# JeroendenBoef/GraphPOPE

Measured on AMD Instinct MI355X. Metric: POPE embeddings/sec (nodes x anchors) + SAGE nodes/sec, Flickr 256 anchors, higher is better.
Workload: dtype u64; 1 GPU; configs[1]: flickr-shaped geodesic-stochastic, N=89250 E=899756 F=500, 256 anchors PER GPU (np.random seed 42); inputs resident in HBM (edge_index, x) -> [N, F+K] f32 in HBM on every rank; anchors_total=256, anchors_per_rank=256, parallelism=single GPU

## Files before the change

### graphpope_amd/_lib.py

```python
from __future__ import annotations

import ctypes
import os
from ctypes import c_char_p, c_double, c_float, c_int, c_int32, c_int64, c_size_t, c_uint64, c_void_p, POINTER

_HERE = os.path.dirname(os.path.abspath(__file__))
LIB_PATH = os.path.join(_HERE, "libgraphpope_hip.so")

OK, ERR_INVALID, ERR_HIP, ERR_INDEX, ERR_HOP_OVERFLOW, ERR_WORKSPACE, ERR_NO_DEVICE, ERR_UNSORTED = 0, -1, -2, -3, -4, -5, -6, -7
METRIC = {"distance": 0, "similarity": 1, "euclidean": 2}
KNOB_LIVE_MODE, KNOB_FINALIZE_VARIANT, KNOB_FINALIZE_BLOCKS = 0, 1, 2
KNOB_PAIRWISE_KERNEL, KNOB_COPY_BATCHES, KNOB_FAIL_HOST_REGISTER = 4, 5, 7
KNOB_SAGE_FORWARD_OVERLAP = 14
KNOB_GEMM_TILE16_BUFFERS = 18
KNOB_PREPARE_MERGE = 19
KNOB_STREAMK_XCD = 20
KNOB_FORWARD_WHOLE_TILES = 21
KNOB_LEVEL1_APPLY = 22

SIGNATURES = {
    "pope_last_error": (c_char_p, []),
    "pope_version": (c_char_p, []),
    "pope_require_device": (c_int, [POINTER(c_int32)]),
    "pope_debug_set": (c_int, [c_int32, c_int32]),
    "pope_host_copy_2d": (c_int, [c_void_p, c_int64, c_void_p, c_int64, c_int64, c_int64, c_int32]),
    "pope_copy_2d_to_host": (c_int, [c_void_p, c_int64, c_void_p, c_int64, c_int64, c_int64, c_void_p]),
    "pope_assemble_host_result": (c_int, [c_void_p, c_int64, c_int64, c_void_p, c_int64, c_int64, c_void_p, c_int64, c_int64, c_int32,
                                          c_int32, c_void_p]),
    "pope_assemble_begin": (c_void_p, [c_void_p, c_int64, c_int64, c_void_p, c_int64, c_int64, c_int32, c_int32]),
    "pope_assemble_finish": (c_int, [c_void_p, c_void_p, c_int64, c_int64, c_void_p]),
    "pope_assemble_abort": (None, [c_void_p]),
    "pope_assemble_prepare": (None, [c_int32]),
    "pope_assemble_ring_ready": (c_int32, []),
    "pope_assemble_finish_codes": (c_int, [c_void_p, c_void_p, c_int64, c_int32, c_void_p, c_void_p]),
    "pope_geodesic_hop_codes": (c_int, [c_void_p, c_int32, c_int32, c_int64, c_int32, c_void_p, c_int64, c_void_p, c_void_p]),
    "pope_host_pin": (c_int, [c_void_p, c_size_t]),
    "pope_host_unpin": (c_int, [c_void_p]),
    "pope_copy_to_device": (c_int, [c_void_p, c_void_p, c_size_t, c_void_p]),
    "pope_csr_scratch_bytes": (c_size_t, [c_int64, c_int64]),
    "pope_csr_aux_elems": (c_size_t, [c_int64]),
    "pope_csr_build": (c_int, [c_void_p, c_int64, c_int64, c_void_p, c_void_p, c_void_p, c_void_p, c_void_p, c_size_t,
                               c_int32, c_void_p]),
    "pope_csr_build_canonical": (c_int, [c_void_p, c_int64, c_int64, c_void_p, c_void_p, c_void_p, c_void_p, c_void_p, c_size_t, c_void_p]),
    "pope_pagerank_weights": (c_int, [c_void_p, c_void_p, c_int64, c_void_p, c_void_p]),
    "pope_pagerank_step": (c_int, [c_void_p, c_void_p, c_int64, c_void_p, c_void_p, c_double, c_double, c_void_p, c_void_p]),
    "pope_clustering_scratch_bytes": (c_size_t, [c_int64, c_int64]),
    "pope_clustering_counts": (c_int, [c_void_p, c_void_p, c_void_p, c_void_p, c_void_p, c_void_p, c_int64, c_int64, c_void_p, c_void_p,
                                       c_void_p, c_void_p, c_size_t, c_void_p]),
    "pope_betweenness_scratch_bytes": (c_size_t, [c_int64, c_int64]),
    "pope_betweenness_batch": (c_int, [c_void_p, c_void_p, c_int64, c_void_p, c_void_p, c_int64, c_int64, c_int64, c_int64, c_void_p,
                                       c_void_p, c_void_p, c_void_p, c_void_p, c_void_p, c_size_t, c_void_p]),
    "pope_eigenvector_scratch_bytes": (c_size_t, [c_int64]),
    "pope_eigenvector_iterate": (c_int, [c_void_p, c_void_p, c_int64, c_void_p, c_void_p, c_size_t, c_int32, c_double, c_void_p, c_void_p]),
    "pope_degree_counts": (c_int, [c_void_p, c_void_p, c_void_p, c_int64, c_void_p, c_void_p, c_void_p]),
    "pope_topk_scratch_bytes": (c_size_t, [c_int64, c_int64]),
    "pope_topk_u64": (c_int, [c_void_p, c_int64, c_int64, c_void_p, c_void_p, c_size_t, c_void_p]),
    "pope_topk_max_k": (c_int, []),
    "pope_topk_f64_scratch_bytes": (c_size_t, [c_int64, c_int64]),
    "pope_topk_f64": (c_int, [c_void_p, c_int64, c_int64, c_void_p, c_void_p, c_void_p, c_size_t, c_void_p]),
    "pope_score_keys_host": (c_int, [c_void_p, c_int64, c_void_p]),
    "pope_kmeans_scratch_bytes": (c_size_t, [c_int64, c_int32, c_int32]),
    "pope_column_moments": (c_int, [c_void_p, c_int64, c_int32, c_void_p, c_void_p, c_void_p, c_size_t, c_void_p]),
    "pope_shift_columns": (c_int, [c_void_p, c_void_p, c_int64, c_int32, c_float, c_void_p, c_void_p]),
    "pope_kmeans_plusplus": (c_int, [c_void_p, c_int64, c_int32, c_int32, c_int64, c_void_p, c_int32, c_void_p, c_void_p, c_size_t,
                                     c_void_p]),
    "pope_kmeans_lloyd_step": (c_int, [c_void_p, c_int64, c_int32, c_void_p, c_int32, c_void_p, c_void_p, c_void_p, c_void_p, c_void_p,
                                       c_void_p, c_size_t, c_void_p]),
    "pope_words": (c_int32, [c_int32]),
    "pope_plane_bytes": (c_size_t, [c_int64, c_int32]),
    "pope_bfs_scratch_bytes": (c_size_t, [c_int64, c_int64, c_int32]),
    "pope_geodesic_bfs": (c_int, [c_void_p, c_void_p, c_void_p, c_void_p, c_int64, c_int64, c_void_p, c_int32, c_void_p, c_int32,
                                  c_void_p, c_size_t, POINTER(c_int32), POINTER(c_int32), c_void_p]),
    "pope_geodesic_bfs_begin": (c_int, [c_void_p, c_void_p, c_void_p, c_void_p, c_int64, c_int64, c_void_p, c_int32, c_void_p, c_int32,
                                        c_void_p, c_size_t, c_void_p]),
    "pope_geodesic_bfs_finish": (c_int, [c_void_p, c_void_p, c_void_p, c_void_p, c_int64, c_int64, c_void_p, c_int32, c_void_p, c_int32,
                                         c_void_p, c_size_t, POINTER(c_int32), POINTER(c_int32), c_void_p]),
    "pope_geodesic_finalize": (c_int, [c_void_p, c_int32, c_int64, c_int32, c_void_p, c_int32, c_void_p, c_int64,
                                       c_int32, c_void_p]),
    "pope_geodesic_run_workspace_bytes": (c_size_t, [c_int64, c_int64, c_int32, c_int32]),
    "pope_geodesic_run_planes": (c_void_p, [c_void_p, c_int64, c_int64, c_int32, c_int32]),
    "pope_geodesic_run": (c_int, [c_void_p, c_int64, c_int64, c_void_p, c_int32, c_void_p, c_int32, c_void_p, c_int64,
                                  c_int32, c_void_p, c_size_t, POINTER(c_int32), POINTER(c_int32), c_void_p]),
    "pope_profile_levels": (None, [c_int32]),
    "pope_profile_read": (c_int32, [c_void_p, c_void_p, c_int32]),
    "pope_profile_level1_applies": (c_int32, []),
    "pope_geodesic_finalize_shards": (c_int, [c_void_p, c_int32, c_int64, c_int32, c_int64, c_int32, c_void_p, c_int32,
                                              c_void_p, c_int64, c_void_p]),
    "pope_finalize_kernel_name": (c_int, [c_int64, c_int32, c_int32, c_int32, c_int32, c_char_p, c_size_t]),
    "pope_level_kernel_name": (c_int, [c_int64, c_int32, c_char_p, c_size_t]),
    "pope_column_stats_scratch_bytes": (c_size_t, [c_int32]),
    "pope_geodesic_column_stats": (c_int, [c_void_p, c_int32, c_int64, c_int32, c_void_p, c_void_p, c_void_p, c_size_t, c_void_p]),
    "pope_geodesic_hops": (c_int, [c_void_p, c_int32, c_int64, c_int32, c_void_p, c_void_p]),
    "pope_pairwise_scratch_bytes": (c_size_t, [c_int64, c_int32, c_int32]),
    "pope_pairwise_minmax": (c_int, [c_void_p, c_int64, c_int32, c_void_p, c_int32, c_int32, c_void_p, c_int64,
                                     c_int32, c_void_p, c_size_t, c_void_p]),
    "pope_pairwise_by_id_scratch_bytes": (c_size_t, [c_int64, c_int32, c_int32]),
    "pope_pairwise_features_by_id": (c_int, [c_void_p, c_int32, c_void_p, c_int64, c_int32, c_void_p, c_int32, c_int32, c_void_p, c_int64, c_int32,
                                             c_void_p, c_size_t, c_void_p]),
    "pope_pairwise_features": (c_int, [c_void_p, c_int32, c_void_p, c_int64, c_int32, c_void_p, c_int32, c_int32, c_void_p, c_int64,
                                       c_int32, c_void_p, c_size_t, c_void_p]),
    "pope_pairwise_kernel_name": (c_int, [c_int64, c_int32, c_int32, c_int32, c_int32, c_int32, c_int32, c_char_p, c_size_t]),
    "pope_concat": (c_int, [c_void_p, c_int64, c_int32, c_void_p, c_int64, c_void_p]),
    "sage_conv_scratch_bytes": (c_size_t, [c_int64, c_int64, c_int64, c_int32, c_int32]),
    "sage_conv_forward_scratch_bytes": (c_size_t, [c_int64, c_int32, c_int32]),
    "sage_conv_forward": (c_int, [c_void_p, c_void_p, c_int64, c_int64, c_int64, c_void_p, c_int32, c_void_p,
                                  c_void_p, c_void_p, c_int32, c_void_p, c_void_p, c_void_p, c_size_t, c_void_p, c_void_p]),
    "sage_gather_mean": (c_int, [c_void_p, c_void_p, c_int64, c_int64, c_int64, c_void_p, c_int32, c_void_p, c_void_p]),
    "sage_conv_forward_indexed": (c_int, [c_void_p, c_void_p, c_void_p, c_int64, c_int64, c_int64, c_void_p, c_int64, c_int32,
                                          c_void_p, c_void_p, c_void_p, c_int32, c_void_p, c_void_p, c_void_p, c_void_p, c_size_t,
                                          c_void_p, c_void_p]),
    "sage_conv_forward_stats": (c_int, [c_void_p, c_void_p, c_int64, c_int64, c_int64, c_void_p, c_int32, c_void_p,
                                        c_void_p, c_void_p, c_int32, c_void_p, c_void_p, c_void_p, c_size_t, c_void_p, c_void_p, c_void_p, c_int32,
                                        c_void_p, c_void_p]),
    "sage_conv_forward_indexed_stats": (c_int, [c_void_p, c_void_p, c_void_p, c_int64, c_int64, c_int64, c_void_p, c_int64, c_int32,
                                                c_void_p, c_void_p, c_void_p, c_int32, c_void_p, c_void_p, c_void_p, c_void_p, c_size_t,
                                                c_void_p, c_void_p, c_void_p, c_int32, c_void_p, c_void_p]),
    "sage_conv_backward": (c_int, [c_void_p, c_void_p, c_int64, c_int64, c_int64, c_void_p, c_void_p, c_int32,
                                   c_void_p, c_void_p, c_int32, c_void_p, c_void_p, c_void_p, c_void_p, c_void_p,
                                   c_void_p, c_size_t, c_void_p, c_void_p]),
    "sage_forward_kernel_name": (c_int, [c_int64, c_int32, c_int32, c_int32, c_char_p, c_size_t]),
    "sage_backward_kernel_name": (c_int, [c_int64, c_int64, c_int32, c_int32, c_int32, c_int32, c_int32, c_char_p, c_size_t]),
    "sage_set_deterministic": (c_int32, [c_int32]),
    "sage_get_deterministic": (c_int32, []),
    "sage_scatter_mean_det_scratch_bytes": (c_size_t, [c_int64, c_int64, c_int64]),
    "sage_scatter_mean_det": (c_int, [c_void_p, c_void_p, c_int64, c_int64, c_int64, c_void_p, c_int32, c_void_p, c_void_p, c_size_t,
                                      c_void_p, c_void_p]),
    "sage_conv_forward_indexed_scratch_bytes": (c_size_t, [c_int64, c_int32, c_int32]),
    "sage_conv_backward_indexed_scratch_bytes": (c_size_t, [c_int64, c_int64, c_int64, c_int32, c_int32]),
    "sage_conv_backward_indexed": (c_int, [c_void_p, c_void_p, c_void_p, c_int64, c_int64, c_int64, c_void_p, c_int64, c_void_p, c_int32, c_void_p,
                                           c_void_p, c_int32, c_void_p, c_void_p, c_void_p, c_void_p, c_void_p, c_size_t, c_void_p, c_void_p]),
    "sage_bn_scratch_bytes": (c_size_t, [c_int32]),
    "sage_bn_relu_dropout_forward": (c_int, [c_void_p, c_int64, c_int32, c_void_p, c_void_p, c_void_p, c_void_p, c_void_p, c_float, c_float,
                                             c_int32, c_float, c_uint64, c_void_p, c_void_p, c_void_p, c_void_p, c_size_t,
                                             c_void_p, c_void_p, c_void_p]),
    "sage_bn_relu_dropout_forward_stats": (c_int, [c_void_p, c_int64, c_int32, c_void_p, c_void_p, c_void_p, c_void_p, c_void_p, c_float, c_float,
                                                   c_int32, c_float, c_uint64, c_void_p, c_void_p, c_void_p, c_void_p, c_size_t,
                                                   c_void_p, c_void_p, c_void_p, c_void_p, c_int32, c_int32, c_void_p]),
    "sage_bn_relu_dropout_backward": (c_int, [c_void_p, c_void_p, c_int64, c_int32, c_void_p, c_void_p, c_void_p, c_void_p,
                                              c_int32, c_float, c_uint64, c_void_p, c_void_p, c_void_p, c_void_p, c_size_t,
                                              c_void_p, c_void_p, c_void_p]),
    "sage_bn_relu_dropout_backward_bias": (c_int, [c_void_p, c_void_p, c_int64, c_int32, c_void_p, c_void_p, c_void_p, c_void_p,
                                                   c_int32, c_float, c_uint64, c_void_p, c_void_p, c_void_p, c_void_p, c_size_t,
                                                   c_void_p, c_void_p, c_void_p, c_void_p]),
    "sage_cross_entropy_forward": (c_int, [c_void_p, c_void_p, c_int64, c_int32, c_int64, c_void_p, c_void_p, c_void_p, c_void_p,
                                           c_void_p, c_int32, c_void_p]),
    "sage_cross_entropy_backward": (c_int, [c_void_p, c_int64, c_int32, c_void_p, c_void_p, c_void_p, c_void_p]),
    "sage_eval_metrics": (c_int, [c_void_p, c_void_p, c_int64, c_int32, c_int64, c_void_p, c_void_p, c_void_p]),
    "sage_adam_step": (c_int, [c_int32, c_void_p, c_void_p, c_void_p, c_void_p, c_void_p, c_double, c_double, c_double, c_double,
                               c_double, c_int64, c_void_p, c_void_p]),
    "sage_adam_step_loss": (c_int, [c_int32, c_void_p, c_void_p, c_void_p, c_void_p, c_void_p, c_double, c_double, c_double, c_double,
                                    c_double, c_int64, c_void_p, c_void_p, c_int64, c_void_p, c_void_p]),
    "sage_grad_norm_partials": (c_size_t, [c_int32, c_void_p]),
    "sage_grad_sqnorm": (c_int, [c_int32, c_void_p, c_void_p, c_void_p, c_size_t, c_void_p]),
    "sage_adam_step_clip": (c_int, [c_int32, c_void_p, c_void_p, c_void_p, c_void_p, c_void_p, c_double, c_double, c_double, c_double,
                                    c_double, c_int64, c_void_p, c_double, c_void_p, c_size_t, c_void_p, c_void_p, c_int64, c_void_p, c_void_p]),
    "sage_advance_counters": (c_int, [c_void_p, c_void_p, c_int32, c_void_p]),
    "sage_copy_segments": (c_int, [c_int32, c_void_p, c_void_p, c_void_p, c_void_p]),
    "sage_sample_batch_device": (c_int, [c_void_p, c_void_p, c_int64, c_void_p, c_int64, c_void_p, c_int32, c_uint64, c_void_p,
                                         c_void_p, c_void_p, c_void_p, c_void_p, c_void_p, c_size_t, c_void_p]),
    "sage_sample_epoch_batch_device": (c_int, [c_void_p, c_void_p, c_int64, c_void_p, c_void_p, c_int64, c_void_p, c_void_p, c_void_p, c_int32, c_uint64,
                                                c_void_p, c_void_p, c_void_p, c_void_p, c_void_p, c_void_p, c_size_t, c_void_p]),
    "sage_sample_scratch_bytes": (c_size_t, [c_int64, c_int64, c_int64]),
    "sage_sample_batch": (c_int, [c_void_p, c_void_p, c_int64, c_void_p, c_int64, c_void_p, c_int32, c_uint64, c_void_p, c_void_p,
                                  c_void_p, c_void_p, c_void_p, c_void_p, c_size_t, c_void_p]),
    "sage_sample_hop": (c_int, [c_void_p, c_void_p, c_int64, c_void_p, c_int64, c_int32, c_uint64, c_int32, c_void_p,
                                c_void_p, c_int64, c_void_p, POINTER(c_int64), POINTER(c_int64), c_void_p, c_size_t, c_void_p]),
    "pope_n2v_walks": (c_int, [c_void_p, c_void_p, c_int64, c_void_p, c_int64, c_int64, c_int32, c_uint64, c_int64, c_void_p, c_void_p,
                               c_void_p]),
    "pope_n2v_windows": (c_int, [c_void_p, c_int64, c_int32, c_int32, c_void_p, c_void_p]),
    "pope_n2v_loss_grad": (c_int, [c_void_p, c_int64, c_int32, c_void_p, c_int64, c_int32, c_int32, c_int32, c_double, c_void_p, c_void_p,
                                   c_void_p, c_void_p]),
    "pope_n2v_sparse_adam": (c_int, [c_void_p, c_void_p, c_void_p, c_void_p, c_void_p, c_int64, c_int32, c_double, c_double, c_double,
                                     c_double, c_int64, c_void_p]),
}


class PopeError(RuntimeError):

    def __init__(self, code: int, message: str):
        super().__init__(f"libgraphpope_hip error {code}: {message}")
        self.code = code


_lib = None


def load() -> ctypes.CDLL:
    global _lib
    if _lib is None:
        if not os.path.exists(LIB_PATH):
            raise ImportError(
                f"{LIB_PATH} is missing: build it with `make -C graphpope_amd/csrc` "
                "(or `python -c 'import __graft_entry__ as g; g.build()'`). graphpope_amd has no CPU fallback.")
        lib = ctypes.CDLL(LIB_PATH)
        for name, (res, args) in SIGNATURES.items():
            fn = getattr(lib, name)
            fn.restype = res
            fn.argtypes = args
        _lib = lib
    return _lib


def check(code: int) -> None:
    if code != OK:
        raise PopeError(code, load().pope_last_error().decode())


def ptr(t) -> c_void_p:
    return c_void_p(0) if t is None else c_void_p(t.data_ptr())


class _NoGuard:
    def __enter__(self):
        return self

    def __exit__(self, *exc):
        return False


_NO_GUARD = _NoGuard()


def on_device(dev):
    import torch
    idx = dev.index if dev.index is not None else torch.cuda.current_device()
    return _NO_GUARD if idx == torch.cuda.current_device() else torch.cuda.device(idx)
```

### graphpope_amd/csrc/epilogue.hip

```cpp
#include "common.h"

namespace pope {

constexpr int BN_MAX_PARTS = 256;

__device__ __forceinline__ unsigned fmix32(unsigned h) {
    h ^= h >> 16;
    h *= 0x85ebca6bu;
    h ^= h >> 13;
    h *= 0xc2b2ae35u;
    h ^= h >> 16;
    return h;
}

__device__ __forceinline__ bool keep_element(unsigned long long seed, unsigned long long idx, unsigned threshold) {
    unsigned h = fmix32((unsigned)idx ^ (unsigned)seed);
    h = fmix32(h ^ ((unsigned)(idx >> 32) * 0x9e3779b1u) ^ (unsigned)(seed >> 32));
    return (h >> 8) >= threshold;
}

template <int VEC> struct Pack { float v[VEC]; };

template <int VEC>
__device__ __forceinline__ Pack<VEC> load_pack(const float *p) {
    Pack<VEC> r;
    if constexpr (VEC == 4) {
        const float4 t = *reinterpret_cast<const float4 *>(p);
        r.v[0] = t.x; r.v[1] = t.y; r.v[2] = t.z; r.v[3] = t.w;
    } else {
        r.v[0] = p[0];
    }
    return r;
}

template <int VEC>
__device__ __forceinline__ void store_pack(float *p, const Pack<VEC> &r) {
    if constexpr (VEC == 4) *reinterpret_cast<float4 *>(p) = make_float4(r.v[0], r.v[1], r.v[2], r.v[3]);
    else p[0] = r.v[0];
}

template <int VEC, bool BWD>
__global__ __launch_bounds__(256) void k_bn_partial(const float *__restrict__ x, const float *__restrict__ dy, int M, int C,
                                                    int rows_per_part, const float *__restrict__ mean,
                                                    const float *__restrict__ rstd, const float *__restrict__ gamma,
                                                    const float *__restrict__ beta, unsigned long long seed,
                                                    unsigned threshold, float inv_keep, double *__restrict__ pa,
                                                    double *__restrict__ pb, const int *__restrict__ m_dev,
                                                    const unsigned long long *__restrict__ seed_dev, double *__restrict__ pc) {
    __shared__ double sh[3][4][64 * VEC];
    const int lane = threadIdx.x & 63, wave = threadIdx.x >> 6;
    const int c0 = (blockIdx.y * 64 + lane) * VEC;
    const bool valid = c0 < C;
    if (m_dev) {
        M = dyn_extent(m_dev, M);
        rows_per_part = (M + (int)gridDim.x - 1) / (int)gridDim.x;
    }
    if (seed_dev) seed += *seed_dev;
    const int r0 = blockIdx.x * rows_per_part, r1 = min(M, r0 + rows_per_part);
    double a[VEC], b[VEC], cc[VEC];
    float mu[VEC], rs[VEC], ga[VEC], be[VEC];
#pragma unroll
    for (int i = 0; i < VEC; ++i) {
        a[i] = b[i] = cc[i] = 0.0;
        mu[i] = rs[i] = ga[i] = be[i] = 0.f;
    }
    if (BWD && valid) {
        const Pack<VEC> m4 = load_pack<VEC>(mean + c0), r4 = load_pack<VEC>(rstd + c0), g4 = load_pack<VEC>(gamma + c0),
                        b4 = load_pack<VEC>(beta + c0);
#pragma unroll
        for (int i = 0; i < VEC; ++i) { mu[i] = m4.v[i]; rs[i] = r4.v[i]; ga[i] = g4.v[i]; be[i] = b4.v[i]; }
    }
    if (valid) {
        auto accumulate = [&](const Pack<VEC> &xv, const Pack<VEC> &gv, size_t off) {
            if constexpr (!BWD) {
#pragma unroll
                for (int i = 0; i < VEC; ++i) {
                    a[i] += (double)xv.v[i];
                    b[i] += (double)xv.v[i] * (double)xv.v[i];
                }
            } else {
#pragma unroll
                for (int i = 0; i < VEC; ++i) {
                    const float xhat = (xv.v[i] - mu[i]) * rs[i];
                    const bool on = xhat * ga[i] + be[i] > 0.f && keep_element(seed, off + i, threshold);
                    const float g = on ? gv.v[i] * inv_keep : 0.f;
                    a[i] += (double)g;
                    b[i] += (double)g * (double)xhat;
                    if (pc) cc[i] += (double)xhat;
                }
            }
        };
        int r = r0 + wave;
        for (; r + 12 < r1; r += 16) {
            Pack<VEC> xv[4], gv[4];
#pragma unroll
            for (int u = 0; u < 4; ++u) {
                const size_t off = (size_t)(r + 4 * u) * C + c0;
                xv[u] = load_pack<VEC>(x + off);
                if constexpr (BWD) gv[u] = load_pack<VEC>(dy + off);
                else gv[u] = xv[u];
            }
#pragma unroll
            for (int u = 0; u < 4; ++u) accumulate(xv[u], gv[u], (size_t)(r + 4 * u) * C + c0);
        }
        for (; r < r1; r += 4) {
            const size_t off = (size_t)r * C + c0;
            const Pack<VEC> xv = load_pack<VEC>(x + off);
            Pack<VEC> gv = xv;
            if constexpr (BWD) gv = load_pack<VEC>(dy + off);
            accumulate(xv, gv, off);
        }
    }
#pragma unroll
    for (int i = 0; i < VEC; ++i) {
        sh[0][wave][lane * VEC + i] = a[i];
        sh[1][wave][lane * VEC + i] = b[i];
        sh[2][wave][lane * VEC + i] = cc[i];
    }
    __syncthreads();
    if (wave == 0 && valid) {
#pragma unroll
        for (int i = 0; i < VEC; ++i) {
            const int j = lane * VEC + i;
            pa[(size_t)blockIdx.x * C + c0 + i] = sh[0][0][j] + sh[0][1][j] + sh[0][2][j] + sh[0][3][j];
            pb[(size_t)blockIdx.x * C + c0 + i] = sh[1][0][j] + sh[1][1][j] + sh[1][2][j] + sh[1][3][j];
            if (BWD && pc) pc[(size_t)blockIdx.x * C + c0 + i] = sh[2][0][j] + sh[2][1][j] + sh[2][2][j] + sh[2][3][j];
        }
    }
}

template <bool THIRD = false>
__device__ __forceinline__ void fold_parts(const double *__restrict__ pa, const double *__restrict__ pb, int parts, int C, int c,
                                           double &s, double &q, const double *__restrict__ pc = nullptr, double *t = nullptr) {
    __shared__ double red[3][16][17];
    const int cl = threadIdx.x & 15, grp = threadIdx.x >> 4;
    double a = 0.0, b = 0.0, d = 0.0;
    if (c < C)
#pragma unroll 4
        for (int p = grp; p < parts; p += 16) {
            a += pa[(size_t)p * C + c];
            b += pb[(size_t)p * C + c];
            if constexpr (THIRD) d += pc[(size_t)p * C + c];
        }
    red[0][grp][cl] = a;
    red[1][grp][cl] = b;
    red[2][grp][cl] = d;
    __syncthreads();
    s = q = 0.0;
    double tt = 0.0;
    if (grp == 0)
#pragma unroll
        for (int g = 0; g < 16; ++g) {
            s += red[0][g][cl];
            q += red[1][g][cl];
            tt += red[2][g][cl];
        }
    if (t) *t = tt;
}

__global__ __launch_bounds__(256) void k_bn_final(const double *__restrict__ pa, const double *__restrict__ pb, int parts, int M, int C, int training,
                           float momentum, float eps, float *__restrict__ running_mean, float *__restrict__ running_var,
                           float *__restrict__ mean, float *__restrict__ rstd, long long *num_batches_tracked,
                           const int *__restrict__ m_dev, int rows_per_part) {
    M = dyn_extent(m_dev, M);
    if (rows_per_part > 0) parts = min(parts, (M + rows_per_part - 1) / rows_per_part);
    if (training && num_batches_tracked && blockIdx.x == 0 && threadIdx.x == 0) *num_batches_tracked += 1;
    const int c = blockIdx.x * 16 + (threadIdx.x & 15);
    const bool owner = (threadIdx.x >> 4) == 0 && c < C;
    if (!training) {
        if (owner) {
            mean[c] = running_mean[c];
            rstd[c] = (float)(1.0 / sqrt((double)running_var[c] + (double)eps));
        }
        return;
    }
    double s, q;
    fold_parts(pa, pb, parts, C, c, s, q);
    if (!owner) return;
    const double mu = s / M;
    double var = q / M - mu * mu;
    if (var < 0.0) var = 0.0;
    mean[c] = (float)mu;
    rstd[c] = (float)(1.0 / sqrt(var + (double)eps));
    if (running_mean) {
        const double unbiased = M > 1 ? var * ((double)M / (double)(M - 1)) : var;
        running_mean[c] = (float)((1.0 - (double)momentum) * (double)running_mean[c] + (double)momentum * mu);
        running_var[c] = (float)((1.0 - (double)momentum) * (double)running_var[c] + (double)momentum * unbiased);
    }
}

__global__ __launch_bounds__(256) void k_bn_bwd_final(const double *__restrict__ pa, const double *__restrict__ pb, int parts, int M, int C,
                               int training, float *__restrict__ dgamma, float *__restrict__ dbeta, float *__restrict__ c1,
                               float *__restrict__ c2, const int *__restrict__ m_dev, const double *__restrict__ pc,
                               const float *__restrict__ gamma, const float *__restrict__ rstd, float *__restrict__ dx_colsum) {
    M = dyn_extent(m_dev, M);
    const int c = blockIdx.x * 16 + (threadIdx.x & 15);
    double s, q, t = 0.0;
    if (pc) fold_parts<true>(pa, pb, parts, C, c, s, q, pc, &t);
    else fold_parts<false>(pa, pb, parts, C, c, s, q);
    if ((threadIdx.x >> 4) != 0 || c >= C) return;
    if (dbeta) dbeta[c] = (float)s;
    if (dgamma) dgamma[c] = (float)q;
    const double k1 = training ? s / M : 0.0, k2 = training ? q / M : 0.0;
    c1[c] = (float)k1;
    c2[c] = (float)k2;
    if (dx_colsum) dx_colsum[c] = (float)((double)gamma[c] * (double)rstd[c] * (s - (double)M * (double)(float)k1 - (double)(float)k2 * t));
}

template <int VEC, bool BWD>
__global__ __launch_bounds__(256) void k_bn_apply(const float *__restrict__ x, const float *__restrict__ dy, size_t total, int C,
                                                  const float *__restrict__ mean, const float *__restrict__ rstd,
                                                  const float *__restrict__ gamma, const float *__restrict__ beta,
                                                  const float *__restrict__ c1, const float *__restrict__ c2,
                                                  unsigned long long seed, unsigned threshold, float inv_keep,
                                                  float *__restrict__ out, const int *__restrict__ m_dev,
                                                  const unsigned long long *__restrict__ seed_dev) {
    if (m_dev) total = (size_t)dyn_extent(m_dev, (int)(total / C)) * C;
    if (seed_dev) seed += *seed_dev;
    const size_t stride = (size_t)gridDim.x * blockDim.x * VEC;
    for (size_t off = ((size_t)blockIdx.x * blockDim.x + threadIdx.x) * VEC; off < total; off += stride) {
        const int c0 = (int)(off % C);
        const Pack<VEC> xv = load_pack<VEC>(x + off);
        Pack<VEC> gv, r;
        if constexpr (BWD) gv = load_pack<VEC>(dy + off);
        const Pack<VEC> mu = load_pack<VEC>(mean + c0), rs = load_pack<VEC>(rstd + c0), ga = load_pack<VEC>(gamma + c0),
                        be = load_pack<VEC>(beta + c0);
        Pack<VEC> k1, k2;
        if constexpr (BWD) { k1 = load_pack<VEC>(c1 + c0); k2 = load_pack<VEC>(c2 + c0); }
#pragma unroll
        for (int i = 0; i < VEC; ++i) {
            const float xhat = (xv.v[i] - mu.v[i]) * rs.v[i];
            const float z = xhat * ga.v[i] + be.v[i];
            const bool on = z > 0.f && keep_element(seed, off + i, threshold);
            if constexpr (!BWD) {
                r.v[i] = on ? z * inv_keep : 0.f;
            } else {
                const float g = on ? gv.v[i] * inv_keep : 0.f;
                r.v[i] = ga.v[i] * rs.v[i] * (g - k1.v[i] - xhat * k2.v[i]);
            }
        }
        store_pack<VEC>(out + off, r);
    }
}

struct BnPlan {
    int parts, rows_per_part, vec;
    double *pa, *pb, *pc;
    float *c1, *c2;
};

static size_t bn_scratch(int C) { return 3 * (size_t)BN_MAX_PARTS * C * sizeof(double) + 2 * align_up((size_t)C * sizeof(float), 256); }

static BnPlan bn_plan(int64_t M, int C, void *scratch, const void *p0, const void *p1, const void *p2, const void *p3,
                      const void *p4, const void *p5, const void *p6) {
    BnPlan p;
    p.parts = (int)((M + 15) / 16);
    if (p.parts > BN_MAX_PARTS) p.parts = BN_MAX_PARTS;
    if (p.parts < 1) p.parts = 1;
    p.rows_per_part = (int)((M + p.parts - 1) / p.parts);
    const bool aligned = (((uintptr_t)p0 | (uintptr_t)p1 | (uintptr_t)p2 | (uintptr_t)p3 | (uintptr_t)p4 | (uintptr_t)p5 |
                           (uintptr_t)p6) & 15) == 0;
    p.vec = (C % 4 == 0 && aligned) ? 4 : 1;
    p.pa = (double *)scratch;
    p.pb = p.pa + (size_t)BN_MAX_PARTS * C;
    p.pc = p.pb + (size_t)BN_MAX_PARTS * C;
    p.c1 = (float *)(p.pc + (size_t)BN_MAX_PARTS * C);
    p.c2 = (float *)((char *)p.c1 + align_up((size_t)C * sizeof(float), 256));
    return p;
}

static unsigned drop_threshold(float p) {
    if (!(p > 0.f)) return 0u;
    if (p >= 1.f) return 1u << 24;
    return (unsigned)((double)p * 16777216.0);
}

}

using namespace pope;

extern "C" size_t sage_bn_scratch_bytes(int32_t C) { return C <= 0 ? 0 : bn_scratch(C); }

static int bn_forward_impl(const float *x, int64_t M, int32_t C, const float *gamma, const float *beta,
                           float *running_mean, float *running_var, int64_t *num_batches_tracked, float momentum, float eps,
                           int32_t training, float p, uint64_t seed, float *y, float *save_mean,
                           float *save_rstd, void *scratch, size_t scratch_bytes, const int32_t *rows_dev,
                           const uint64_t *seed_dev_, const double *ext_pa, const double *ext_pb, int ext_parts, int ext_rows_per_part,
                           hipStream_t stream) {
    POPE_REQUIRE(x && gamma && beta && y && save_mean && save_rstd && scratch, "sage_bn_relu_dropout_forward: null pointer");
    POPE_REQUIRE(M > 0 && M < INT32_MAX && C > 0 && (size_t)M * C < ((size_t)1 << 40), "sage_bn_relu_dropout_forward: bad size");
    POPE_REQUIRE(training || (running_mean && running_var), "sage_bn_relu_dropout_forward: eval mode needs running statistics");
    POPE_REQUIRE((running_mean == nullptr) == (running_var == nullptr), "sage_bn_relu_dropout_forward: running_mean/var go together");
    POPE_REQUIRE(p >= 0.f && p <= 1.f && eps > 0.f, "sage_bn_relu_dropout_forward: need 0 <= p <= 1, eps > 0");
    if (scratch_bytes < bn_scratch(C)) {
        set_error("sage_bn_relu_dropout_forward: scratch %zu < %zu bytes", scratch_bytes, bn_scratch(C));
        return POPE_ERR_WORKSPACE;
    }
    const BnPlan pl = bn_plan(M, C, scratch, x, y, nullptr, gamma, beta, save_mean, save_rstd);
    const unsigned long long *seed_dev = (const unsigned long long *)seed_dev_;
    const bool external = training && ext_pa && ext_pb && ext_parts > 0 && ext_rows_per_part > 0;
    if (training && !external) {
        const dim3 grid(pl.parts, (C + 64 * pl.vec - 1) / (64 * pl.vec));
        if (pl.vec == 4)
            hipLaunchKernelGGL((k_bn_partial<4, false>), grid, dim3(256), 0, stream, x, nullptr, (int)M, C, pl.rows_per_part,
                               nullptr, nullptr, nullptr, nullptr, 0ull, 0u, 1.f, pl.pa, pl.pb, rows_dev, nullptr, nullptr);
        else
            hipLaunchKernelGGL((k_bn_partial<1, false>), grid, dim3(256), 0, stream, x, nullptr, (int)M, C, pl.rows_per_part,
                               nullptr, nullptr, nullptr, nullptr, 0ull, 0u, 1.f, pl.pa, pl.pb, rows_dev, nullptr, nullptr);
    }
    hipLaunchKernelGGL(k_bn_final, dim3((C + 15) / 16), dim3(256), 0, stream, external ? ext_pa : pl.pa, external ? ext_pb : pl.pb,
                       external ? ext_parts : pl.parts, (int)M, C, training, momentum, eps, running_mean, running_var, save_mean, save_rstd,
                       (long long *)num_batches_tracked, rows_dev, external ? ext_rows_per_part : 0);
    const unsigned thr = training ? drop_threshold(p) : 0u;
    const float inv_keep = (training && p > 0.f && p < 1.f) ? (float)(1.0 / (1.0 - (double)p)) : 1.f;
    const size_t total = (size_t)M * C;
    const unsigned blocks = capped_grid(total / pl.vec, 256);
    if (pl.vec == 4)
        hipLaunchKernelGGL((k_bn_apply<4, false>), dim3(blocks), dim3(256), 0, stream, x, nullptr, total, C, save_mean, save_rstd,
                           gamma, beta, nullptr, nullptr, (unsigned long long)seed, thr, inv_keep, y, rows_dev, seed_dev);
    else
        hipLaunchKernelGGL((k_bn_apply<1, false>), dim3(blocks), dim3(256), 0, stream, x, nullptr, total, C, save_mean, save_rstd,
                           gamma, beta, nullptr, nullptr, (unsigned long long)seed, thr, inv_keep, y, rows_dev, seed_dev);
    POPE_HIP(hipGetLastError());
    return POPE_OK;
}

extern "C" int sage_bn_relu_dropout_forward(const float *x, int64_t M, int32_t C, const float *gamma, const float *beta,
                                            float *running_mean, float *running_var, int64_t *num_batches_tracked, float momentum, float eps,
                                            int32_t training, float p, uint64_t seed, float *y, float *save_mean,
                                            float *save_rstd, void *scratch, size_t scratch_bytes, const int32_t *rows_dev,
                                            const uint64_t *seed_dev_, void *stream_) {
    clear_error();
    return bn_forward_impl(x, M, C, gamma, beta, running_mean, running_var, num_batches_tracked, momentum, eps, training, p, seed, y, save_mean,
                           save_rstd, scratch, scratch_bytes, rows_dev, seed_dev_, nullptr, nullptr, 0, 0, (hipStream_t)stream_);
}

extern "C" int sage_bn_relu_dropout_forward_stats(const float *x, int64_t M, int32_t C, const float *gamma, const float *beta,
                                                  float *running_mean, float *running_var, int64_t *num_batches_tracked, float momentum, float eps,
                                                  int32_t training, float p, uint64_t seed, float *y, float *save_mean, float *save_rstd,
                                                  void *scratch, size_t scratch_bytes, const int32_t *rows_dev, const uint64_t *seed_dev_,
                                                  const double *pa, const double *pb, int32_t parts, int32_t rows_per_part, void *stream_) {
    clear_error();
    POPE_REQUIRE(pa && pb && parts > 0 && rows_per_part > 0 && (int64_t)parts * rows_per_part >= M, "sage_bn_relu_dropout_forward_stats: the partials do not cover the rows");
    return bn_forward_impl(x, M, C, gamma, beta, running_mean, running_var, num_batches_tracked, momentum, eps, training, p, seed, y, save_mean,
                           save_rstd, scratch, scratch_bytes, rows_dev, seed_dev_, pa, pb, parts, rows_per_part, (hipStream_t)stream_);
}

static int bn_backward_impl(const float *x, const float *grad_y, int64_t M, int32_t C, const float *gamma,
                            const float *beta, const float *save_mean, const float *save_rstd,
                            int32_t training, float p, uint64_t seed, float *grad_x, float *grad_gamma,
                            float *grad_beta, void *scratch, size_t scratch_bytes, const int32_t *rows_dev,
                            const uint64_t *seed_dev_, float *grad_x_colsum, hipStream_t stream) {
    POPE_REQUIRE(x && grad_y && gamma && beta && save_mean && save_rstd && grad_x && scratch,
                 "sage_bn_relu_dropout_backward: null pointer");
    POPE_REQUIRE(M > 0 && M < INT32_MAX && C > 0 && (size_t)M * C < ((size_t)1 << 40), "sage_bn_relu_dropout_backward: bad size");
    POPE_REQUIRE(p >= 0.f && p <= 1.f, "sage_bn_relu_dropout_backward: need 0 <= p <= 1");
    if (scratch_bytes < bn_scratch(C)) {
        set_error("sage_bn_relu_dropout_backward: scratch %zu < %zu bytes", scratch_bytes, bn_scratch(C));
        return POPE_ERR_WORKSPACE;
    }
    const BnPlan pl = bn_plan(M, C, scratch, x, grad_y, grad_x, gamma, beta, save_mean, save_rstd);
    const unsigned long long *seed_dev = (const unsigned long long *)seed_dev_;
    const unsigned thr = training ? drop_threshold(p) : 0u;
    const float inv_keep = (training && p > 0.f && p < 1.f) ? (float)(1.0 / (1.0 - (double)p)) : 1.f;
    const dim3 grid(pl.parts, (C + 64 * pl.vec - 1) / (64 * pl.vec));
    if (pl.vec == 4)
        hipLaunchKernelGGL((k_bn_partial<4, true>), grid, dim3(256), 0, stream, x, grad_y, (int)M, C, pl.rows_per_part, save_mean,
                           save_rstd, gamma, beta, (unsigned long long)seed, thr, inv_keep, pl.pa, pl.pb, rows_dev, seed_dev, grad_x_colsum ? pl.pc : nullptr);
    else
        hipLaunchKernelGGL((k_bn_partial<1, true>), grid, dim3(256), 0, stream, x, grad_y, (int)M, C, pl.rows_per_part, save_mean,
                           save_rstd, gamma, beta, (unsigned long long)seed, thr, inv_keep, pl.pa, pl.pb, rows_dev, seed_dev, grad_x_colsum ? pl.pc : nullptr);
    hipLaunchKernelGGL(k_bn_bwd_final, dim3((C + 15) / 16), dim3(256), 0, stream, pl.pa, pl.pb, pl.parts, (int)M, C, training,
                       grad_gamma, grad_beta, pl.c1, pl.c2, rows_dev, grad_x_colsum ? pl.pc : nullptr, gamma, save_rstd, grad_x_colsum);
    const size_t total = (size_t)M * C;
    const unsigned blocks = capped_grid(total / pl.vec, 256);
    if (pl.vec == 4)
        hipLaunchKernelGGL((k_bn_apply<4, true>), dim3(blocks), dim3(256), 0, stream, x, grad_y, total, C, save_mean, save_rstd,
                           gamma, beta, pl.c1, pl.c2, (unsigned long long)seed, thr, inv_keep, grad_x, rows_dev, seed_dev);
    else
        hipLaunchKernelGGL((k_bn_apply<1, true>), dim3(blocks), dim3(256), 0, stream, x, grad_y, total, C, save_mean, save_rstd,
                           gamma, beta, pl.c1, pl.c2, (unsigned long long)seed, thr, inv_keep, grad_x, rows_dev, seed_dev);
    POPE_HIP(hipGetLastError());
    return POPE_OK;
}

extern "C" int sage_bn_relu_dropout_backward(const float *x, const float *grad_y, int64_t M, int32_t C, const float *gamma,
                                             const float *beta, const float *save_mean, const float *save_rstd,
                                             int32_t training, float p, uint64_t seed, float *grad_x, float *grad_gamma,
                                             float *grad_beta, void *scratch, size_t scratch_bytes, const int32_t *rows_dev,
                                             const uint64_t *seed_dev_, void *stream_) {
    clear_error();
    return bn_backward_impl(x, grad_y, M, C, gamma, beta, save_mean, save_rstd, training, p, seed, grad_x, grad_gamma, grad_beta, scratch,
                            scratch_bytes, rows_dev, seed_dev_, nullptr, (hipStream_t)stream_);
}

extern "C" int sage_bn_relu_dropout_backward_bias(const float *x, const float *grad_y, int64_t M, int32_t C, const float *gamma,
                                                  const float *beta, const float *save_mean, const float *save_rstd,
                                                  int32_t training, float p, uint64_t seed, float *grad_x, float *grad_gamma,
                                                  float *grad_beta, void *scratch, size_t scratch_bytes, const int32_t *rows_dev,
                                                  const uint64_t *seed_dev_, float *grad_x_colsum, void *stream_) {
    clear_error();
    POPE_REQUIRE(grad_x_colsum, "sage_bn_relu_dropout_backward_bias: null pointer");
    return bn_backward_impl(x, grad_y, M, C, gamma, beta, save_mean, save_rstd, training, p, seed, grad_x, grad_gamma, grad_beta, scratch,
                            scratch_bytes, rows_dev, seed_dev_, grad_x_colsum, (hipStream_t)stream_);
}

namespace pope {
__global__ void k_xent_final(const float *__restrict__ row_loss, int N, float *__restrict__ loss, float *__restrict__ inv_count);
}

namespace pope {

constexpr int ADAM_MAX_TENSORS = 24;
constexpr int ADAM_CHUNK = 4096;

struct AdamTable {
    float *p[ADAM_MAX_TENSORS];
    const float *g[ADAM_MAX_TENSORS];
    float *m[ADAM_MAX_TENSORS];
    float *v[ADAM_MAX_TENSORS];
    long long n[ADAM_MAX_TENSORS];
    int first_block[ADAM_MAX_TENSORS + 1];
    int count;
};

constexpr int CLIP_MAX_PARTS = 256;
constexpr int NORM_MAX_TENSORS = 128;

struct NormTable {
    const float *g[NORM_MAX_TENSORS];
    long long n[NORM_MAX_TENSORS];
    int first_chunk[NORM_MAX_TENSORS + 1];
    int count;
};

__device__ __forceinline__ double block_sum_f64(double s) {
    __shared__ double wsum[4];
#pragma unroll
    for (int off = 32; off > 0; off >>= 1) s += __shfl_down(s, off, 64);
    if ((threadIdx.x & 63) == 0) wsum[threadIdx.x >> 6] = s;
    __syncthreads();
    return ((wsum[0] + wsum[1]) + wsum[2]) + wsum[3];
}

__global__ __launch_bounds__(256) void k_grad_sqnorm(NormTable t, double *__restrict__ parts, int accumulate) {
    const int chunks = t.first_chunk[t.count];
    double s = 0.0;
    int k = 0;
    for (int c = (int)blockIdx.x; c < chunks; c += (int)gridDim.x) {
        while (k + 1 < t.count && c >= t.first_chunk[k + 1]) ++k;
        const long long base = (long long)(c - t.first_chunk[k]) * ADAM_CHUNK;
        const long long end = min(t.n[k], base + ADAM_CHUNK);
        const float *__restrict__ g = t.g[k];
        long long i = base + threadIdx.x;
        if ((reinterpret_cast<uintptr_t>(g) & 15) == 0) {
            const long long end4 = base + ((end - base) & ~3ll);
            for (long long q = base + 4ll * threadIdx.x; q < end4; q += 4ll * blockDim.x) {
                const float4 g4 = *reinterpret_cast<const float4 *>(g + q);
                s += (double)g4.x * (double)g4.x;
                s += (double)g4.y * (double)g4.y;
                s += (double)g4.z * (double)g4.z;
                s += (double)g4.w * (double)g4.w;
            }
            i = end4 + threadIdx.x;
        }
        for (; i < end; i += blockDim.x) s += (double)g[i] * (double)g[i];
    }
    s = block_sum_f64(s);
    if (threadIdx.x == 0) parts[blockIdx.x] = accumulate ? parts[blockIdx.x] + s : s;
}

__device__ __forceinline__ void xent_final_block(const float *__restrict__ row_loss, int N, float *__restrict__ loss,
                                                 float *__restrict__ inv_count) {
    __shared__ double ssum[256];
    __shared__ int scnt[256];
    double s = 0.0;
    int n = 0;
    for (int base = 0; base < N; base += 8 * 256) {
        float v[8];
#pragma unroll
        for (int u = 0; u < 8; ++u) {
            const float t = row_loss[min(base + (int)threadIdx.x + 256 * u, N - 1)];
            v[u] = base + (int)threadIdx.x + 256 * u < N ? t : -1.f;
        }
#pragma unroll
        for (int u = 0; u < 8; ++u)
            if (v[u] >= 0.f) { s += (double)v[u]; ++n; }
    }
    ssum[threadIdx.x] = s;
    scnt[threadIdx.x] = n;
    __syncthreads();
    for (int off = 128; off > 0; off >>= 1) {
        if ((int)threadIdx.x < off) { ssum[threadIdx.x] += ssum[threadIdx.x + off]; scnt[threadIdx.x] += scnt[threadIdx.x + off]; }
        __syncthreads();
    }
    if (threadIdx.x == 0) {
        *loss = scnt[0] > 0 ? (float)(ssum[0] / scnt[0]) : __builtin_nanf("");
        *inv_count = scnt[0] > 0 ? 1.f / (float)scnt[0] : 0.f;
    }
}

template <bool CLIP>
__global__ __launch_bounds__(256) void k_adam(AdamTable t, float step_size, float one_minus_b1, float beta2, float one_minus_b2,
                                              float eps, float weight_decay, float inv_bc2_sqrt, const long long *__restrict__ step_dev,
                                              double lr, double beta1_d, double beta2_d, const float *__restrict__ xent_rows, int xent_n,
                                              float *__restrict__ xent_out, const double *__restrict__ parts, int n_parts, float max_norm,
                                              float *__restrict__ norm_out) {
    if ((int)blockIdx.x == t.first_block[t.count]) {
        xent_final_block(xent_rows, xent_n, xent_out, xent_out + 1);
        return;
    }
    float coef = 1.f;
    if constexpr (CLIP) {
        const float total = (float)sqrt(block_sum_f64((int)threadIdx.x < n_parts ? parts[threadIdx.x] : 0.0));
        const float c = max_norm / (total + 1e-6f);
        coef = c > 1.f ? 1.f : c;
        if (blockIdx.x == 0 && threadIdx.x == 0 && norm_out) {
            norm_out[0] = total;
            norm_out[1] = coef;
        }
    }
    if (step_dev) {
        const double step = (double)*step_dev;
        step_size = (float)(lr / (1.0 - pow(beta1_d, step)));
        inv_bc2_sqrt = (float)(1.0 / sqrt(1.0 - pow(beta2_d, step)));
    }
    int k = 0;
    while (k + 1 < t.count && (int)blockIdx.x >= t.first_block[k + 1]) ++k;
    const long long base = (long long)((int)blockIdx.x - t.first_block[k]) * ADAM_CHUNK;
    const long long end = min(t.n[k], base + ADAM_CHUNK);
    float *__restrict__ p = t.p[k];
    const float *__restrict__ g = t.g[k];
    float *__restrict__ m = t.m[k];
    float *__restrict__ v = t.v[k];
    auto update = [&](float &pi, float gi, float &mi, float &vi) {
        if constexpr (CLIP) gi *= coef;
        if (weight_decay != 0.f) gi += weight_decay * pi;
        mi = mi + (gi - mi) * one_minus_b1;
        vi = beta2 * vi + one_minus_b2 * gi * gi;
        pi = pi - step_size * (mi / (sqrtf(vi) * inv_bc2_sqrt + eps));
    };
    long long i = base + threadIdx.x;
    if (((reinterpret_cast<uintptr_t>(p) | reinterpret_cast<uintptr_t>(g) | reinterpret_cast<uintptr_t>(m) |
          reinterpret_cast<uintptr_t>(v)) & 15) == 0) {
        const long long end4 = base + ((end - base) & ~3ll);
        for (long long q = base + 4ll * threadIdx.x; q < end4; q += 4ll * blockDim.x) {
            float4 p4 = *reinterpret_cast<float4 *>(p + q), m4 = *reinterpret_cast<float4 *>(m + q), v4 = *reinterpret_cast<float4 *>(v + q);
            const float4 g4 = *reinterpret_cast<const float4 *>(g + q);
            update(p4.x, g4.x, m4.x, v4.x);
            update(p4.y, g4.y, m4.y, v4.y);
            update(p4.z, g4.z, m4.z, v4.z);
            update(p4.w, g4.w, m4.w, v4.w);
            *reinterpret_cast<float4 *>(m + q) = m4;
            *reinterpret_cast<float4 *>(v + q) = v4;
            *reinterpret_cast<float4 *>(p + q) = p4;
        }
        i = end4 + threadIdx.x;
    }
    for (; i < end; i += blockDim.x) {
        float pi = p[i], mi = m[i], vi = v[i];
        update(pi, g[i], mi, vi);
        m[i] = mi;
        v[i] = vi;
        p[i] = pi;
    }
}

}

static int64_t grad_norm_parts(int32_t n_tensors, const int64_t *numel) {
    if (n_tensors < 0 || (n_tensors > 0 && !numel)) return -1;
    int64_t chunks = 0;
    for (int t = 0; t < n_tensors; ++t) {
        if (numel[t] < 0) return -1;
        chunks += (numel[t] + ADAM_CHUNK - 1) / ADAM_CHUNK;
    }
    return chunks < 1 ? 1 : chunks > CLIP_MAX_PARTS ? CLIP_MAX_PARTS : chunks;
}

static int adam_step_impl(int32_t n_tensors, float *const *params, const float *const *grads, float *const *exp_avg,
                          float *const *exp_avg_sq, const int64_t *numel, double lr, double beta1, double beta2, double eps,
                          double weight_decay, int64_t step, const int64_t *step_dev, const float *xent_rows, int64_t xent_n, float *xent_out,
                          hipStream_t stream, const double *clip_parts = nullptr, int n_parts = 0, float max_norm = 0.f,
                          float *norm_out = nullptr) {
    POPE_REQUIRE(n_tensors >= 0 && (n_tensors == 0 || (params && grads && exp_avg && exp_avg_sq && numel)), "sage_adam_step: null pointer");
    if (step_dev) step = 1;
    POPE_REQUIRE(step >= 1 && lr >= 0.0 && beta1 >= 0.0 && beta1 < 1.0 && beta2 >= 0.0 && beta2 < 1.0 && eps >= 0.0,
                 "sage_adam_step: need step >= 1, lr >= 0, 0 <= beta < 1, eps >= 0");
    const double bc1 = 1.0 - pow(beta1, (double)step), bc2 = 1.0 - pow(beta2, (double)step);
    const float step_size = (float)(lr / bc1), inv_bc2_sqrt = (float)(1.0 / sqrt(bc2));
    for (int t0 = 0; t0 < n_tensors; t0 += ADAM_MAX_TENSORS) {
        AdamTable tab;
        tab.count = 0;
        int blocks = 0;
        for (int t = t0; t < n_tensors && tab.count < ADAM_MAX_TENSORS; ++t) {
            POPE_REQUIRE(numel[t] >= 0 && (numel[t] == 0 || (params[t] && grads[t] && exp_avg[t] && exp_avg_sq[t])),
                         "sage_adam_step: tensor %d has a null pointer", t);
            if (numel[t] == 0) continue;
            const int c = tab.count++;
            tab.p[c] = params[t]; tab.g[c] = grads[t]; tab.m[c] = exp_avg[t]; tab.v[c] = exp_avg_sq[t]; tab.n[c] = numel[t];
            tab.first_block[c] = blocks;
            blocks += (int)((numel[t] + ADAM_CHUNK - 1) / ADAM_CHUNK);
        }
        if (tab.count == 0) continue;
        tab.first_block[tab.count] = blocks;
        const bool with_loss = xent_rows != nullptr;
        hipLaunchKernelGGL(clip_parts ? k_adam<true> : k_adam<false>, dim3(blocks + (with_loss ? 1 : 0)), dim3(256), 0, stream, tab, step_size,
                           (float)(1.0 - beta1), (float)beta2, (float)(1.0 - beta2), (float)eps, (float)weight_decay, inv_bc2_sqrt,
                           (const long long *)step_dev, lr, beta1, beta2, xent_rows, (int)xent_n, xent_out, clip_parts, n_parts, max_norm, norm_out);
        xent_rows = nullptr;
    }
    if (xent_rows)
        hipLaunchKernelGGL(k_xent_final, dim3(1), dim3(256), 0, stream, xent_rows, (int)xent_n, xent_out, xent_out + 1);
    POPE_HIP(hipGetLastError());
    return POPE_OK;
}

extern "C" int sage_adam_step(int32_t n_tensors, float *const *params, const float *const *grads, float *const *exp_avg,
                              float *const *exp_avg_sq, const int64_t *numel, double lr, double beta1, double beta2, double eps,
                              double weight_decay, int64_t step, const int64_t *step_dev, void *stream_) {
    clear_error();
    return adam_step_impl(n_tensors, params, grads, exp_avg, exp_avg_sq, numel, lr, beta1, beta2, eps, weight_decay, step, step_dev, nullptr, 0,
                          nullptr, (hipStream_t)stream_);
}

extern "C" int sage_adam_step_loss(int32_t n_tensors, float *const *params, const float *const *grads, float *const *exp_avg,
                                   float *const *exp_avg_sq, const int64_t *numel, double lr, double beta1, double beta2, double eps,
                                   double weight_decay, int64_t step, const int64_t *step_dev, const float *xent_rows, int64_t xent_n,
                                   float *loss_out, void *stream_) {
    clear_error();
    POPE_REQUIRE(xent_rows && loss_out && xent_n > 0 && xent_n < INT32_MAX, "sage_adam_step_loss: null pointer or bad row count");
    return adam_step_impl(n_tensors, params, grads, exp_avg, exp_avg_sq, numel, lr, beta1, beta2, eps, weight_decay, step, step_dev, xent_rows,
                          xent_n, loss_out, (hipStream_t)stream_);
}

extern "C" size_t sage_grad_norm_partials(int32_t n_tensors, const int64_t *numel) {
    const int64_t parts = grad_norm_parts(n_tensors, numel);
    return parts < 0 ? 0 : (size_t)parts;
}

extern "C" int sage_grad_sqnorm(int32_t n_tensors, const float *const *grads, const int64_t *numel, double *partials,
                                size_t partials_len, void *stream_) {
    clear_error();
    const int64_t parts = grad_norm_parts(n_tensors, numel);
    POPE_REQUIRE(parts > 0 && (n_tensors == 0 || grads), "sage_grad_sqnorm: null pointer or negative size");
    POPE_REQUIRE(partials && partials_len >= (size_t)parts, "sage_grad_sqnorm: the workspace holds %zu doubles, sage_grad_norm_partials asks for %lld",
                 partials ? partials_len : (size_t)0, (long long)parts);
    int64_t all_chunks = 0;
    for (int t = 0; t < n_tensors; ++t) {
        POPE_REQUIRE(numel[t] == 0 || grads[t], "sage_grad_sqnorm: tensor %d has a null pointer", t);
        all_chunks += (numel[t] + ADAM_CHUNK - 1) / ADAM_CHUNK;
    }
    POPE_REQUIRE(all_chunks <= INT32_MAX, "sage_grad_sqnorm: too many elements");
    hipStream_t stream = (hipStream_t)stream_;
    int launches = 0;
    for (int t0 = 0; t0 < n_tensors || launches == 0; t0 += NORM_MAX_TENSORS) {
        NormTable tab;
        tab.count = 0;
        int chunks = 0;
        for (int t = t0; t < n_tensors && t < t0 + NORM_MAX_TENSORS; ++t) {
            if (numel[t] == 0) continue;
            const int c = tab.count++;
            tab.g[c] = grads[t]; tab.n[c] = numel[t];
            tab.first_chunk[c] = chunks;
            chunks += (int)((numel[t] + ADAM_CHUNK - 1) / ADAM_CHUNK);
        }
        tab.first_chunk[tab.count] = chunks;
// ... 388 lines not shown
```

### graphpope_amd/csrc/sage.hip

```cpp
#include <cstring>
#include <mutex>

#include "gemm_streamk_tn.h"
#include "gemm_tile16.h"
#include "side_copy.h"

namespace pope {

__device__ __forceinline__ long long src_row(int j, const long long *__restrict__ n_id) { return n_id ? n_id[j] : (long long)j; }

template <bool VEC>
__global__ __launch_bounds__(256) void k_gather_mean(const int *__restrict__ rowptr, const int *__restrict__ col,
                                                     int n_dst, const float *__restrict__ x, int C,
                                                     float *__restrict__ agg, const long long *__restrict__ n_id,
                                                     float *__restrict__ x_dst, const int *__restrict__ n_dst_dev) {
    const int lane = threadIdx.x & 63;
    const int wave = (blockIdx.x * blockDim.x + threadIdx.x) >> 6;
    const int nwaves = (gridDim.x * blockDim.x) >> 6;
    n_dst = dyn_extent(n_dst_dev, n_dst);
    for (int i = wave; i < n_dst; i += nwaves) {
        const int beg = rowptr[i], end = rowptr[i + 1];
        const float inv = end > beg ? 1.0f / (float)(end - beg) : 0.0f;
        if (VEC) {
            const int C4 = C >> 2;
            for (int q = lane; q < C4; q += 64) {
                float4 s = make_float4(0.f, 0.f, 0.f, 0.f);
                int p = beg;
                for (; p + 3 < end; p += 4) {
                    const long long j0 = src_row(col[p], n_id), j1 = src_row(col[p + 1], n_id), j2 = src_row(col[p + 2], n_id), j3 = src_row(col[p + 3], n_id);
                    const float4 a = reinterpret_cast<const float4 *>(x + (size_t)j0 * C)[q];
                    const float4 b = reinterpret_cast<const float4 *>(x + (size_t)j1 * C)[q];
                    const float4 c = reinterpret_cast<const float4 *>(x + (size_t)j2 * C)[q];
                    const float4 d = reinterpret_cast<const float4 *>(x + (size_t)j3 * C)[q];
                    s.x += a.x; s.y += a.y; s.z += a.z; s.w += a.w;
                    s.x += b.x; s.y += b.y; s.z += b.z; s.w += b.w;
                    s.x += c.x; s.y += c.y; s.z += c.z; s.w += c.w;
                    s.x += d.x; s.y += d.y; s.z += d.z; s.w += d.w;
                }
                for (; p < end; ++p) {
                    const float4 a = reinterpret_cast<const float4 *>(x + (size_t)src_row(col[p], n_id) * C)[q];
                    s.x += a.x; s.y += a.y; s.z += a.z; s.w += a.w;
                }
                s.x *= inv; s.y *= inv; s.z *= inv; s.w *= inv;
                reinterpret_cast<float4 *>(agg + (size_t)i * C)[q] = s;
                if (x_dst) reinterpret_cast<float4 *>(x_dst + (size_t)i * C)[q] = reinterpret_cast<const float4 *>(x + (size_t)n_id[i] * C)[q];
            }
        } else {
            for (int c = lane; c < C; c += 64) {
                float s = 0.f;
                for (int p = beg; p < end; ++p) s += x[(size_t)src_row(col[p], n_id) * C + c];
                agg[(size_t)i * C + c] = s * inv;
                if (x_dst) x_dst[(size_t)i * C + c] = x[(size_t)n_id[i] * C + c];
            }
        }
    }
}

__device__ __forceinline__ void scatter_mean_block(const int *__restrict__ rowptr, const int *__restrict__ col, int n_dst,
                                                   const float *__restrict__ gagg, int C, float *__restrict__ gx,
                                                   const int *__restrict__ n_dst_dev, const int block, const int nblocks) {
    const int lane = threadIdx.x & 63;
    const int wave = (block * blockDim.x + threadIdx.x) >> 6;
    const int nwaves = (nblocks * blockDim.x) >> 6;
    const int slabs = (C + 255) / 256;
    n_dst = dyn_extent(n_dst_dev, n_dst);
    for (int w = wave; w < n_dst * slabs; w += nwaves) {
        const int i = w / slabs, c0 = (w - i * slabs) * 256;
        const int beg = rowptr[i], end = rowptr[i + 1];
        if (end == beg) continue;
        const float inv = 1.0f / (float)(end - beg);
        float g[4];
#pragma unroll
        for (int k = 0; k < 4; ++k) {
            const int c = c0 + k * 64 + lane;
            g[k] = c < C ? gagg[(size_t)i * C + c] * inv : 0.f;
        }
        for (int p0 = beg; p0 < end; p0 += 64) {
            const int mine = p0 + lane < end ? col[p0 + lane] : 0;
            const int cnt = min(64, end - p0);
            for (int p = 0; p < cnt; ++p) {
                float *row = gx + (size_t)__shfl(mine, p) * C;
#pragma unroll
                for (int k = 0; k < 4; ++k) {
                    const int c = c0 + k * 64 + lane;
                    if (c < C) atomicAdd(&row[c], g[k]);
                }
            }
        }
    }
}

__global__ __launch_bounds__(256) void k_scatter_mean(const int *__restrict__ rowptr, const int *__restrict__ col,
                                                      int n_dst, const float *__restrict__ gagg, int C,
                                                      float *__restrict__ gx, const int *__restrict__ n_dst_dev) {
    scatter_mean_block(rowptr, col, n_dst, gagg, C, gx, n_dst_dev, blockIdx.x, gridDim.x);
}

__device__ __forceinline__ void zero_rows_block(float *__restrict__ x, int C, int r0, int r1, int b, int nb) {
    if (r1 <= r0) return;
    const size_t n = (size_t)(r1 - r0) * C;
    const size_t stride = (size_t)nb * blockDim.x;
    float *base = x + (size_t)r0 * C;
    const size_t i = (size_t)b * blockDim.x + threadIdx.x;
    if ((reinterpret_cast<uintptr_t>(base) & 15) == 0) {
        const size_t n4 = n >> 2;
        for (size_t q = i; q < n4; q += stride) reinterpret_cast<float4 *>(base)[q] = make_float4(0.f, 0.f, 0.f, 0.f);
        for (size_t q = (n4 << 2) + i; q < n; q += stride) base[q] = 0.f;
    } else {
        for (size_t q = i; q < n; q += stride) base[q] = 0.f;
    }
}

__global__ __launch_bounds__(256) void k_zero_rows(float *__restrict__ x, int C, int r0, int r1, const int *__restrict__ r0_dev,
                                                   const int *__restrict__ r1_dev) {
    zero_rows_block(x, C, dyn_extent(r0_dev, r0), dyn_extent(r1_dev, r1), blockIdx.x, gridDim.x);
}

int g_sage_deterministic = 0;

constexpr int DET_SCAN_THREADS = 1024, DET_SCAN_ITEMS = 8, DET_AHEAD = 8;

__global__ __launch_bounds__(256) void k_det_clear(int *__restrict__ start, int n_src, const int *__restrict__ n_src_dev) {
    n_src = dyn_extent(n_src_dev, n_src);
    for (int j = blockIdx.x * blockDim.x + threadIdx.x; j <= n_src; j += gridDim.x * blockDim.x) start[j] = 0;
}

template <bool FILL>
__global__ __launch_bounds__(256) void k_det_index(const int *__restrict__ rowptr, const int *__restrict__ col, int n_dst, int n_src, int nnz,
                                                   int *__restrict__ start, int *__restrict__ list, const int *__restrict__ n_dst_dev,
                                                   const int *__restrict__ n_src_dev) {
    const int lane = threadIdx.x & 63;
    const int wave = (blockIdx.x * blockDim.x + threadIdx.x) >> 6, nwaves = (gridDim.x * blockDim.x) >> 6;
    n_dst = dyn_extent(n_dst_dev, n_dst);
    n_src = dyn_extent(n_src_dev, n_src);
    for (int i = wave; i < n_dst; i += nwaves) {
        const int beg = max(rowptr[i], 0), end = min(rowptr[i + 1], nnz);
        for (int p = beg + lane; p < end; p += 64) {
            const int j = col[p];
            if ((unsigned)j >= (unsigned)n_src) continue;
            const int at = atomicAdd(&start[j], 1);
            if (FILL && at >= 0 && at < nnz) list[at] = i;
        }
    }
}

__global__ __launch_bounds__(DET_SCAN_THREADS) void k_det_scan(int *__restrict__ start, int n_src, const int *__restrict__ n_src_dev) {
    __shared__ int s_wave[DET_SCAN_THREADS / 64];
    __shared__ int s_carry;
    const int lane = threadIdx.x & 63, wib = threadIdx.x >> 6;
    n_src = dyn_extent(n_src_dev, n_src);
    if (threadIdx.x == 0) s_carry = 0;
    __syncthreads();
    for (int base = 0; base < n_src; base += DET_SCAN_THREADS * DET_SCAN_ITEMS) {
        const int at = base + threadIdx.x * DET_SCAN_ITEMS;
        int v[DET_SCAN_ITEMS], sum = 0;
#pragma unroll
        for (int k = 0; k < DET_SCAN_ITEMS; ++k) {
            v[k] = at + k < n_src ? start[at + k] : 0;
            sum += v[k];
        }
        int incl = sum;
#pragma unroll
        for (int off = 1; off < 64; off <<= 1) {
            const int o = __shfl_up(incl, off);
            if (lane >= off) incl += o;
        }
        if (lane == 63) s_wave[wib] = incl;
        __syncthreads();
        int run = s_carry + incl - sum;
        for (int w = 0; w < wib; ++w) run += s_wave[w];
#pragma unroll
        for (int k = 0; k < DET_SCAN_ITEMS; ++k) {
            if (at + k < n_src) start[at + k] = run;
            run += v[k];
        }
        __syncthreads();
        if (threadIdx.x == DET_SCAN_THREADS - 1) s_carry = run;
        __syncthreads();
    }
}

__device__ __forceinline__ int wave_sort_ascending(int v, const int lane) {
#pragma unroll
    for (int k = 2; k <= 64; k <<= 1) {
#pragma unroll
        for (int j = k >> 1; j > 0; j >>= 1) {
            const int o = __shfl_xor(v, j);
            v = (((lane & j) == 0) == ((lane & k) == 0)) ? min(v, o) : max(v, o);
        }
    }
    return v;
}

#pragma clang fp contract(off)
template <bool VEC>
__device__ __forceinline__ void det_add_rows(const int ids, const int cnt, const int *__restrict__ rowptr, const float *__restrict__ gagg,
                                             const int C, const int c0, const int lane, float (&acc)[4]) {
    float inv = 0.f;
    if (lane < cnt) inv = __fdiv_rn(1.0f, (float)(rowptr[ids + 1] - rowptr[ids]));
    for (int t0 = 0; t0 < cnt; t0 += DET_AHEAD) {
        float r[DET_AHEAD][4], iv[DET_AHEAD];
#pragma unroll
        for (int u = 0; u < DET_AHEAD; ++u) {
            const int t = min(t0 + u, cnt - 1);
            const float *row = gagg + (size_t)__shfl(ids, t) * C;
            iv[u] = __shfl(inv, t);
            if (VEC) {
                const int c = c0 + 4 * lane;
                const float4 q = c < C ? *reinterpret_cast<const float4 *>(row + c) : make_float4(0.f, 0.f, 0.f, 0.f);
                r[u][0] = q.x; r[u][1] = q.y; r[u][2] = q.z; r[u][3] = q.w;
            } else {
#pragma unroll
                for (int k = 0; k < 4; ++k) {
                    const int c = c0 + k * 64 + lane;
                    r[u][k] = c < C ? row[c] : 0.f;
                }
            }
        }
#pragma unroll
        for (int u = 0; u < DET_AHEAD; ++u) {
            if (t0 + u < cnt) {
#pragma unroll
                for (int k = 0; k < 4; ++k) {
                    const float prod = r[u][k] * iv[u];
                    acc[k] = acc[k] + prod;
                }
            }
        }
    }
}
#pragma clang fp contract(fast)

template <bool VEC>
__device__ __forceinline__ void det_row_begin(const float *gx, const int j, const bool keep, const int C, const int c0, const int lane,
                                              float (&acc)[4]) {
#pragma unroll
    for (int k = 0; k < 4; ++k) acc[k] = 0.f;
    if (!keep) return;
    const float *row = gx + (size_t)j * C;
    if (VEC) {
        const int c = c0 + 4 * lane;
        if (c < C) {
            const float4 q = *reinterpret_cast<const float4 *>(row + c);
            acc[0] = q.x; acc[1] = q.y; acc[2] = q.z; acc[3] = q.w;
        }
    } else {
#pragma unroll
        for (int k = 0; k < 4; ++k) {
            const int c = c0 + k * 64 + lane;
            if (c < C) acc[k] = row[c];
        }
    }
}

template <bool VEC>
__device__ __forceinline__ void det_row_end(float *gx, const int j, const int C, const int c0, const int lane, const float (&acc)[4]) {
    float *row = gx + (size_t)j * C;
    if (VEC) {
        const int c = c0 + 4 * lane;
        if (c < C) *reinterpret_cast<float4 *>(row + c) = make_float4(acc[0], acc[1], acc[2], acc[3]);
    } else {
#pragma unroll
        for (int k = 0; k < 4; ++k) {
            const int c = c0 + k * 64 + lane;
            if (c < C) row[c] = acc[k];
        }
    }
}

template <bool VEC>
__global__ __launch_bounds__(256) void k_scatter_sum_det(const int *__restrict__ rowptr, const int *__restrict__ start, const int *__restrict__ list,
                                                         int *sorted, int n_dst, int n_src, int nnz, const float *__restrict__ gagg, int C,
                                                         float *gx, const int *__restrict__ n_dst_dev, const int *__restrict__ n_src_dev) {
    const int lane = threadIdx.x & 63;
    const int wave = (blockIdx.x * blockDim.x + threadIdx.x) >> 6, nwaves = (gridDim.x * blockDim.x) >> 6;
    const int slabs = (C + 255) / 256;
    n_dst = dyn_extent(n_dst_dev, n_dst);
    n_src = dyn_extent(n_src_dev, n_src);
    const long long items = (long long)n_src * slabs;
    for (long long w = wave; w < items; w += nwaves) {
        const int j = (int)(w / slabs), slab = (int)(w - (long long)j * slabs);
        const int beg = min(max(j ? start[j - 1] : 0, 0), nnz), end = min(max(start[j], beg), nnz);
        const int len = end - beg;
        const bool keep = j < n_dst;
        if (len == 0 && keep) continue;
        float acc[4];
        if (len <= 64) {
            int ids = lane < len ? list[beg + lane] : 0x7fffffff;
            ids = wave_sort_ascending(ids, lane);
            if ((unsigned)ids >= (unsigned)n_dst) ids = 0;
            det_row_begin<VEC>(gx, j, keep, C, slab * 256, lane, acc);
            det_add_rows<VEC>(ids, len, rowptr, gagg, C, slab * 256, lane, acc);
            det_row_end<VEC>(gx, j, C, slab * 256, lane, acc);
            continue;
        }
        if (slab != 0) continue;
        for (int e0 = 0; e0 < len; e0 += 64) {
            const int e = e0 + lane;
            const int mine = e < len ? list[beg + e] : 0x7fffffff;
            int rank = 0;
            for (int m0 = 0; m0 < len; m0 += 64) {
                const int theirs = m0 + lane < len ? list[beg + m0 + lane] : 0x7fffffff;
                const int cnt = min(64, len - m0);
                for (int t = 0; t < cnt; ++t) {
                    const int o = __shfl(theirs, t);
                    rank += (o < mine || (o == mine && m0 + t < e)) ? 1 : 0;
                }
            }
            if (e < len) sorted[beg + rank] = mine;
        }
        __threadfence();
        for (int s = 0; s < slabs; ++s) {
            det_row_begin<VEC>(gx, j, keep, C, s * 256, lane, acc);
            for (int p0 = 0; p0 < len; p0 += 64) {
                const int cnt = min(64, len - p0);
                int ids = lane < cnt ? sorted[beg + p0 + lane] : 0;
                if ((unsigned)ids >= (unsigned)n_dst) ids = 0;
                det_add_rows<VEC>(ids, cnt, rowptr, gagg, C, s * 256, lane, acc);
            }
            det_row_end<VEC>(gx, j, C, s * 256, lane, acc);
        }
    }
}

constexpr int COLSUM_SPLITS = 256;

template <bool VEC>
__device__ __forceinline__ void colsum_partial_block(const float *__restrict__ g, int rows, int C, float *__restrict__ part, int bx, int by, int gy) {
    constexpr int W = VEC ? 4 : 1;
    __shared__ float red[4][64 * W];
    const int lane = threadIdx.x & 63, wave = threadIdx.x >> 6;
    const int c = (bx * 64 + lane) * W;
    const int per = (rows + gy - 1) / gy;
    const int r0 = by * per, r1 = min(rows, r0 + per);
    float s[W];
#pragma unroll
    for (int k = 0; k < W; ++k) s[k] = 0.f;
    if (c < C) {
        int i = r0 + wave;
        for (; i + 12 < r1; i += 16) {
            if constexpr (VEC) {
                float4 v[4];
#pragma unroll
                for (int u = 0; u < 4; ++u) v[u] = *reinterpret_cast<const float4 *>(g + (size_t)(i + 4 * u) * C + c);
#pragma unroll
                for (int u = 0; u < 4; ++u) { s[0] += v[u].x; s[1] += v[u].y; s[2] += v[u].z; s[3] += v[u].w; }
            } else {
                float v[4];
#pragma unroll
                for (int u = 0; u < 4; ++u) v[u] = g[(size_t)(i + 4 * u) * C + c];
#pragma unroll
                for (int u = 0; u < 4; ++u) s[0] += v[u];
            }
        }
        for (; i < r1; i += 4) {
            if constexpr (VEC) {
                const float4 v = *reinterpret_cast<const float4 *>(g + (size_t)i * C + c);
                s[0] += v.x; s[1] += v.y; s[2] += v.z; s[3] += v.w;
            } else {
                s[0] += g[(size_t)i * C + c];
// ... 504 lines not shown
                }
                float4 v[4][3];
#pragma unroll
                for (int t = 0; t < 4; ++t) {
                    const float4 *r = reinterpret_cast<const float4 *>(g.x + (size_t)row[t] * C);
#pragma unroll
                    for (int k = 0; k < 3; ++k) v[t][k] = r[ok[k] ? q[k] : 0];
                }
#pragma unroll
                for (int t = 0; t < 4; ++t)
#pragma unroll
                    for (int k = 0; k < 3; ++k) {
                        s[k].x += v[t][k].x * w[t]; s[k].y += v[t][k].y * w[t]; s[k].z += v[t][k].z * w[t]; s[k].w += v[t][k].w * w[t];
                    }
            }
#pragma unroll
            for (int k = 0; k < 3; ++k) {
                if (!ok[k]) continue;
                s[k].x *= inv; s[k].y *= inv; s[k].z *= inv; s[k].w *= inv;
                reinterpret_cast<float4 *>(g.agg + (size_t)i * C)[q[k]] = s[k];
            }
            if (g.x_dst) {
                const float4 *own = reinterpret_cast<const float4 *>(g.x + (size_t)own0 * C);
                float4 *dst = reinterpret_cast<float4 *>(g.x_dst + (size_t)i * C);
                const float4 o0 = own[ok[0] ? q[0] : 0], o1 = own[ok[1] ? q[1] : 0], o2 = own[ok[2] ? q[2] : 0];
                if (ok[0]) dst[q[0]] = o0;
                if (ok[1]) dst[q[1]] = o1;
                if (ok[2]) dst[q[2]] = o2;
            }
        }
        b0 = b1; e0 = e1; id0 = id1; own0 = own1;
        b1 = b2; e1 = e2; c1 = c2;
        b2 = b3; e2 = e3;
    }
}

template <int RB>
__global__ __launch_bounds__(T16_THREADS, 4) void k_gather_beside_gemm(T16Args a, GatherArgs g, int gemm_blocks) {
    extern __shared__ __attribute__((aligned(16))) char smem[];
    if ((int)blockIdx.x < gemm_blocks) t16_block_loop<RB>(a, smem, (int)blockIdx.x, gemm_blocks);
    else gather_role(g, (int)blockIdx.x - gemm_blocks, (int)gridDim.x - gemm_blocks);
}

template <int RB>
static int launch_gather_beside_gemm(const T16Args &a, const GatherArgs &g, int gemm_blocks, int gather_blocks, hipStream_t stream) {
    static LdsOptIn opt_in;
    if (!opt_in.done()) {
        POPE_HIP(hipFuncSetAttribute((const void *)k_gather_beside_gemm<RB>, hipFuncAttributeMaxDynamicSharedMemorySize, T16Shape<RB>::LDS_BYTES));
        opt_in.mark();
    }
    hipLaunchKernelGGL((k_gather_beside_gemm<RB>), dim3((unsigned)(gemm_blocks + gather_blocks)), dim3(T16_THREADS), T16Shape<RB>::LDS_BYTES, stream, a, g,
                       gemm_blocks);
    return POPE_OK;
}

static int forward_overlapped(const int32_t *rowptr, const int32_t *col, int64_t n_dst, const float *x, int32_t c_in, const long long *n_id,
                              float *x_dst, float *agg, const float *w_l, const float *b_l, const float *w_r, int32_t c_out, float *out,
                              const int32_t *dims, int rb, int cus, hipStream_t stream, BnStatsOut *stats) {
    T16Plan first, second;
    int rc;
    if ((rc = t16_fill(x, w_r, c_in, nullptr, nullptr, 0, c_in, c_in, (int)n_dst, c_out, b_l, out, c_out, dims, rb, cus, &first))) return rc;
    if ((rc = t16_fill(agg, w_l, c_in, nullptr, nullptr, 0, c_in, c_in, (int)n_dst, c_out, nullptr, out, c_out, dims, rb, cus, &second))) return rc;
    first.a.rows = n_id;
    second.a.accumulate = 1;
    stats_take(stats, second);
    const int gemm_blocks = first.a.tiles_n == 2 ? std::min(first.grid, (cus + 15) / 16 * 16) : std::min(first.grid, cus);
    const int gather_blocks = cus;
    const GatherArgs g{rowptr, col, (int)n_dst, x, c_in, agg, n_id, x_dst, dims};
    switch (rb) {
    case 3: rc = launch_gather_beside_gemm<3>(first.a, g, gemm_blocks, gather_blocks, stream); break;
    case 4: rc = launch_gather_beside_gemm<4>(first.a, g, gemm_blocks, gather_blocks, stream); break;
    default: rc = launch_gather_beside_gemm<5>(first.a, g, gemm_blocks, gather_blocks, stream); break;
    }
    if (rc) return rc;
    POPE_HIP(hipGetLastError());
    return t16_launch(second, stream);
}

static bool streamk_tn_shape_ok(int64_t depth, int32_t M, int32_t Nb) {
    if ((M & 3) || (Nb & 3) || M < 4 || Nb < 4 || depth <= 0) return false;
    const long long tiles = 2ll * ((M + SK_TM - 1) / SK_TM) * ((Nb + SK_TN - 1) / SK_TN);
    return tiles * ((depth + SK_GK - 1) / SK_GK) >= 4ll * SK_MAX_GRID;
}

static int streamk_tn_grid(int cus, int64_t depth, int M, int Nb) {
    return streamk_grid(cus, 2ll * ((M + SK_TM - 1) / SK_TM) * ((Nb + SK_TN - 1) / SK_TN) * ((depth + SK_GK - 1) / SK_GK));
}

static int gemm_streamk_tn(const float *G, const float *B0, const float *B1, int64_t depth, int M, int Nb, float *C0, float *C1,
                           void *slab, int grid, bool xcd, hipStream_t stream, const int *depth_dev, float *cs_part, float *cs_out,
                           const long long *rows1) {
    int rc;
    SkTnArgs a;
    a.G = G; a.ldg = M; a.B[0] = B0; a.B[1] = B1; a.ldb = Nb; a.C[0] = C0; a.C[1] = C1; a.ldc = Nb;
    a.M = M; a.Nb = Nb; a.depth = (int)depth; a.slab = (float *)slab;
    a.tiles_m = (M + SK_TM - 1) / SK_TM; a.tiles_nb = (Nb + SK_TN - 1) / SK_TN; a.S = (int)((depth + SK_GK - 1) / SK_GK);
    a.depth_dev = depth_dev;
    a.rows1 = rows1;
    a.cs_part = cs_part; a.cs_out = cs_out; a.cs_splits = COLSUM_SPLITS; a.cs_C = M;
    const unsigned fix_blocks = 2u * a.tiles_m * a.tiles_nb + (cs_part ? (unsigned)(M + 15) / 16 : 0u);
    a.xcd = xcd;
    static LdsOptIn opt_in;
    if (!opt_in.done()) {
        POPE_HIP(hipFuncSetAttribute((const void *)k_gemm_streamk_tn<SK_GK>, hipFuncAttributeMaxDynamicSharedMemorySize, SkStage<SK_GK>::LDS_BYTES));
        opt_in.mark();
    }
    if ((rc = sk_zero_page(&a.zero))) return rc;
    hipLaunchKernelGGL(k_gemm_streamk_tn<SK_GK>, dim3((unsigned)grid), dim3(SKL_THREADS), SkStage<SK_GK>::LDS_BYTES, stream, a);
    hipLaunchKernelGGL(k_streamk_tn_fixup<SK_GK>, dim3(fix_blocks, SK_TN_FIX_PARTS), dim3(256), 0, stream, a, grid);
    POPE_HIP(hipGetLastError());
    return POPE_OK;
}

enum BwdStep : unsigned char {
    BWD_DUAL, BWD_SCATTER_AND_FINALS, BWD_FINALS, BWD_COLSUM_PARTIAL, BWD_STREAMK, BWD_GATHER_ROWS, BWD_W_TWIN, BWD_COLSUM_FINAL,
    BWD_ZERO_ROWS, BWD_X_TWIN, BWD_SCATTER_MEAN, BWD_DET_SUM
};
struct BwdAligned { bool grad_out, agg, x, x_tmp, w_l, w_r, grad_agg, grad_x; };
struct BwdPlan {
    BwdStep steps[8];
    int n_steps;
    void add(BwdStep s) { steps[n_steps++] = s; }
    int sk_grid;
    bool xcd;
    int splits;
    GemmTile w_tile; GemmLayouts w_layouts;
    bool colsum_vec;
    bool zero_rows;
    GemmTile x_tile; GemmLayouts x_layouts;
    bool det_vec;
};

static BwdPlan backward_plan(int64_t n_dst, int64_t n_src, int32_t c_in, int32_t c_out, bool has_edges, bool need_grad_x, bool need_grad_b,
                             bool indexed, const BwdAligned &al, int cus, size_t slab_bytes) {
    BwdPlan p{};
    p.splits = weight_grad_splits(n_dst, c_in, c_out);
    p.colsum_vec = (c_out & 3) == 0 && al.grad_out;
    p.sk_grid = streamk_tn_grid(cus, n_dst, c_out, c_in);
    const bool streamk = streamk_tn_shape_ok(n_dst, c_out, c_in) && al.grad_out && al.agg && al.x && n_dst < INT32_MAX && slab_bytes >= sk_slab_bytes(p.sk_grid);
    if (streamk) {
        const int tiles_m = (c_out + SK_TM - 1) / SK_TM, tiles_nb = (c_in + SK_TN - 1) / SK_TN;
        const long long S = (n_dst + SK_GK - 1) / SK_GK;
        p.xcd = g_streamk_xcd && p.sk_grid % 8 == 0 && (p.sk_grid / 8) % tiles_m == 0 && p.sk_grid / tiles_m <= 2ll * tiles_nb * S;
    }
    const bool gather_rows = !streamk && indexed;
    const bool x_al = gather_rows ? al.x_tmp : al.x;
    const int M = (int)n_dst;
    const Layout g = pick_layout(al.grad_out, c_out, 1, M, c_out), gt = pick_layout(al.grad_out, 1, c_out, c_out, M);
    const Layout wr_t = pick_layout(al.w_r, 1, c_in, c_in, c_out), wl_t = pick_layout(al.w_l, 1, c_in, c_in, c_out);
    const Layout agg_t = pick_layout(al.agg, 1, c_in, c_in, M), xd_t = pick_layout(x_al, 1, c_in, c_in, M);
    const bool dual = !streamk && need_grad_x && p.splits > 1 && need_grad_b && p.colsum_vec && g == LAYOUT_KC_VEC && wr_t == LAYOUT_OC_VEC &&
                      wl_t == LAYOUT_OC_VEC && gt == LAYOUT_OC_VEC && agg_t == LAYOUT_OC_VEC && xd_t == LAYOUT_OC_VEC &&
                      tiles(M, c_in, 64, 128) * 2 < 384 && tiles(c_out, c_in, 64, 128) * p.splits * 2 < 384;
    const bool det_sum = g_sage_deterministic && need_grad_x;
    const bool scatter = need_grad_x && has_edges && !det_sum;
    p.zero_rows = need_grad_x && n_src > n_dst && !det_sum;
    p.det_vec = (c_in & 3) == 0 && al.grad_agg && al.grad_x;
    if (dual) {
        p.add(BWD_DUAL);
        p.add(scatter ? BWD_SCATTER_AND_FINALS : BWD_FINALS);
        if (det_sum) p.add(BWD_DET_SUM);
        return p;
    }
    if (streamk) {
        if (need_grad_b) p.add(BWD_COLSUM_PARTIAL);
        p.add(BWD_STREAMK);
    } else {
        if (gather_rows) p.add(BWD_GATHER_ROWS);
        p.w_tile = gemm_tile_for(c_out, c_in, p.splits, 2);
        p.w_layouts = gemm_layouts(gt, agg_t, false, LAYOUT_GENERIC, LAYOUT_GENERIC, true, xd_t);
        p.add(BWD_W_TWIN);
        if (need_grad_b) {
            p.add(BWD_COLSUM_PARTIAL);
            p.add(BWD_COLSUM_FINAL);
        }
    }
    if (need_grad_x) {
        if (p.zero_rows) p.add(BWD_ZERO_ROWS);
        p.x_tile = gemm_tile_for(M, c_in, 1, 2);
        p.x_layouts = gemm_layouts(g, wr_t, false, LAYOUT_GENERIC, LAYOUT_GENERIC, true, wl_t);
        p.add(BWD_X_TWIN);
        if (scatter) p.add(BWD_SCATTER_MEAN);
        if (det_sum) p.add(BWD_DET_SUM);
    }
    return p;
}

}

using namespace pope;

#ifdef POPE_STAMP
extern "C" int pope_debug_read_t16_trace(unsigned long long *host, int count) {
    return (int)hipMemcpyFromSymbol(host, HIP_SYMBOL(g_t16_trace), (size_t)count * sizeof(unsigned long long));
}
extern "C" int pope_debug_read_gemm_stamps(unsigned long long *host, int count) {
    return (int)hipMemcpyFromSymbol(host, HIP_SYMBOL(g_gemm_stamps), (size_t)count * sizeof(unsigned long long));
}
#endif

__global__ __launch_bounds__(256) void k_gather_rows(const float *__restrict__ x, const long long *__restrict__ rows, int n, int C,
                                                     float *__restrict__ dst, const int *__restrict__ n_dev) {
    const int lane = threadIdx.x & 63;
    const int wave = (blockIdx.x * blockDim.x + threadIdx.x) >> 6, nwaves = (gridDim.x * blockDim.x) >> 6;
    n = dyn_extent(n_dev, n);
    for (int i = wave; i < n; i += nwaves) {
        const float *src = x + (size_t)rows[i] * C;
        float *d = dst + (size_t)i * C;
        if ((C & 3) == 0 && ((reinterpret_cast<uintptr_t>(x) | reinterpret_cast<uintptr_t>(dst)) & 15) == 0) {
            for (int q = lane; q < (C >> 2); q += 64) reinterpret_cast<float4 *>(d)[q] = reinterpret_cast<const float4 *>(src)[q];
        } else {
            for (int c = lane; c < C; c += 64) d[c] = src[c];
        }
    }
}

static size_t rows_matrix_bytes(int64_t n_dst, int32_t c_in) { return align_up((size_t)n_dst * c_in * sizeof(float), 256); }

struct BwdScratch {
    size_t grad_agg, slab, slab_bytes, colsum, core;
    size_t det_start, det_list, det_sorted, rows, total;
};

static BwdScratch backward_scratch(int64_t n_src, int64_t n_dst, int64_t nnz, int32_t c_in, int32_t c_out, bool deterministic, bool indexed) {
    BwdScratch s{};
    size_t at = 0;
    auto take = [&at](size_t bytes) { const size_t was = at; at += align_up(bytes, 256); return was; };
    if (n_dst > 0 && c_in > 0 && c_out > 0) {
        s.grad_agg = take((size_t)n_dst * c_in * sizeof(float));
        s.slab_bytes = 2 * (size_t)weight_grad_splits(n_dst, c_in, c_out) * c_out * c_in * sizeof(float);
        if (streamk_tn_shape_ok(n_dst, c_out, c_in) && s.slab_bytes < sk_slab_bytes(SK_MAX_GRID)) s.slab_bytes = sk_slab_bytes(SK_MAX_GRID);
        s.slab_bytes = align_up(s.slab_bytes, 256);
        s.slab = take(s.slab_bytes);
        s.colsum = take((size_t)COLSUM_SPLITS * c_out * sizeof(float));
        s.core = at;
    }
    if (deterministic && n_src > 0 && n_dst >= 0 && n_dst <= n_src && nnz >= 0 && n_src < INT32_MAX && nnz < INT32_MAX) {
        s.det_start = take((size_t)(n_src + 1) * sizeof(int));
        s.det_list = take((size_t)(nnz > 0 ? nnz : 1) * sizeof(int));
        s.det_sorted = take((size_t)(nnz > 0 ? nnz : 1) * sizeof(int));
    }
    if (indexed && s.core) s.rows = take(rows_matrix_bytes(n_dst, c_in));
    s.total = at;
    return s;
}

template <typename T>
static T *scratch_at(void *scratch, size_t offset) { return reinterpret_cast<T *>(static_cast<char *>(scratch) + offset); }

extern "C" size_t sage_scatter_mean_det_scratch_bytes(int64_t n_src, int64_t n_dst, int64_t nnz) {
    return backward_scratch(n_src, n_dst, nnz, 0, 0, true, false).total;
}

extern "C" int32_t sage_set_deterministic(int32_t on) {
    const int32_t was = g_sage_deterministic;
    g_sage_deterministic = on != 0;
    return was;
}

extern "C" int32_t sage_get_deterministic(void) { return g_sage_deterministic; }

extern "C" size_t sage_conv_scratch_bytes(int64_t n_src, int64_t n_dst, int64_t nnz, int32_t c_in, int32_t c_out) {
    const BwdScratch s = backward_scratch(n_src, n_dst, nnz, c_in, c_out, g_sage_deterministic, false);
    return s.core ? s.total : 0;
}

extern "C" size_t sage_conv_forward_scratch_bytes(int64_t n_dst, int32_t c_in, int32_t c_out) {
    if (n_dst <= 0 || c_in <= 0 || c_out <= 0) return 0;
    return streamk_shape_ok(n_dst, c_in, c_in, c_out) ? sk_slab_bytes(SK_MAX_GRID) : 0;
}

extern "C" size_t sage_conv_forward_indexed_scratch_bytes(int64_t n_dst, int32_t c_in, int32_t c_out) {
    if (n_dst <= 0 || c_in <= 0 || c_out <= 0) return 0;
    return align_up(sage_conv_forward_scratch_bytes(n_dst, c_in, c_out), 256) + rows_matrix_bytes(n_dst, c_in);
}

extern "C" size_t sage_conv_backward_indexed_scratch_bytes(int64_t n_src, int64_t n_dst, int64_t nnz, int32_t c_in, int32_t c_out) {
    const BwdScratch s = backward_scratch(n_src, n_dst, nnz, c_in, c_out, g_sage_deterministic, true);
    return s.core ? s.total : 0;
}

static void enqueue_gather_mean(const int32_t *rowptr, const int32_t *col, int64_t n_dst, const float *x_src, int32_t c_in,
                                float *agg, hipStream_t stream, const int64_t *n_id = nullptr, float *x_dst = nullptr,
                                const int32_t *n_dst_dev = nullptr) {
    dim3 grid(capped_grid((size_t)n_dst * 64, 256));
    if ((c_in & 3) == 0 && aligned16(x_src) && aligned16(agg) && (!x_dst || aligned16(x_dst)))
        hipLaunchKernelGGL(k_gather_mean<true>, grid, dim3(256), 0, stream, rowptr, col, (int)n_dst, x_src, c_in, agg,
                           (const long long *)n_id, x_dst, n_dst_dev);
    else
        hipLaunchKernelGGL(k_gather_mean<false>, grid, dim3(256), 0, stream, rowptr, col, (int)n_dst, x_src, c_in, agg,
                           (const long long *)n_id, x_dst, n_dst_dev);
}

extern "C" int sage_gather_mean(const int32_t *rowptr, const int32_t *col, int64_t n_src, int64_t n_dst, int64_t nnz,
                                const float *x_src, int32_t c_in, float *agg, void *stream_) {
    clear_error();
    POPE_REQUIRE(rowptr && (col || nnz == 0) && x_src && agg, "sage_gather_mean: null pointer");
    POPE_REQUIRE(n_dst > 0 && n_src > 0 && n_src < INT32_MAX && nnz >= 0 && nnz < INT32_MAX && c_in > 0, "sage_gather_mean: bad size");
    enqueue_gather_mean(rowptr, col, n_dst, x_src, c_in, agg, (hipStream_t)stream_);
    POPE_HIP(hipGetLastError());
    return POPE_OK;
}

static int conv_forward_run(const int32_t *rowptr, const int32_t *col, const int64_t *n_id, int64_t n_dst, const float *x, int64_t x_rows,
                            int32_t c_in, const float *w_l, const float *b_l, const float *w_r, int32_t c_out, float *agg, float *x_dst,
                            float *out, void *scratch, size_t scratch_bytes, const int32_t *dims, BnStatsOut *stats, hipStream_t stream) {
    int cus = 0, rc;
    if ((rc = device_cu_count(&cus))) return rc;
    const size_t rows_at = align_up(sage_conv_forward_scratch_bytes(n_dst, c_in, c_out), 256);
    float *const x_dst_tail = scratch ? (float *)((char *)scratch + rows_at) : nullptr;
    const float *own = !n_id ? x : x_dst ? x_dst : x_dst_tail;
    const FwdAligned al{aligned16(x), aligned16(agg), aligned16(own), !x_dst || aligned16(x_dst), aligned16(w_l), aligned16(w_r)};
    const FwdPlan plan = forward_plan(n_dst, c_in, c_out, x_rows, cus, al, !scratch ? 0 : n_id && !x_dst ? rows_at : scratch_bytes);
    if (plan.path == FWD_OVERLAPPED)
        return forward_overlapped(rowptr, col, n_dst, x, c_in, (const long long *)n_id, x_dst, agg, w_l, b_l, w_r, c_out, out, dims, plan.rb, cus,
                                  stream, stats);
    if (n_id && !x_dst) {
        if (!scratch || scratch_bytes < rows_at + rows_matrix_bytes(n_dst, c_in)) {
            set_error("sage_conv_forward_indexed: without x_dst the scratch must hold sage_conv_forward_indexed_scratch_bytes (%zu), got %zu",
                      rows_at + rows_matrix_bytes(n_dst, c_in), scratch_bytes);
            return POPE_ERR_WORKSPACE;
        }
        x_dst = x_dst_tail;
    }
    enqueue_gather_mean(rowptr, col, n_dst, x, c_in, agg, stream, n_id, x_dst, dims);
    switch (plan.path) {
    case FWD_TILE16:
        return gemm_tile16(agg, w_l, c_in, own, w_r, c_in, c_in, c_in, (int)n_dst, c_out, b_l, out, c_out, plan.rb, cus, stream, dims, stats);
    case FWD_STREAMK:
        return gemm_streamk(agg, w_l, c_in, own, w_r, c_in, c_in, c_in, (int)n_dst, c_out, b_l, out, c_out, scratch, cus, stream, dims);
    default: {
        GemmArgs p = gemm_problem(Operand{agg, c_in, 1}, Operand{w_l, c_in, 1}, c_in, (int)n_dst, c_out, out, c_out);
        p.A1 = Operand{own, c_in, 1}; p.B1 = Operand{w_r, c_in, 1}; p.K1 = c_in;
        p.bias = b_l;
        p.m_dev = dims;
        return launch_gemm(p, plan.tile, gemm_layouts(p), stream);
    }
    }
}

static int conv_forward_impl(const int32_t *rowptr, const int32_t *col, int64_t n_src, int64_t n_dst, int64_t nnz,
                             const float *x_src, int32_t c_in, const float *w_l, const float *b_l, const float *w_r,
                             int32_t c_out, float *agg, float *out, void *scratch, size_t scratch_bytes, const int32_t *dims,
                             BnStatsOut *stats, hipStream_t stream) {
    POPE_REQUIRE(rowptr && (col || nnz == 0) && x_src && w_l && w_r && agg && out, "sage_conv_forward: null pointer");
    POPE_REQUIRE(n_dst > 0 && n_dst <= n_src && n_src < INT32_MAX && nnz >= 0 && nnz < INT32_MAX && c_in > 0 && c_out > 0,
                 "sage_conv_forward: bad size (destinations must be the first n_dst sources)");
    return conv_forward_run(rowptr, col, nullptr, n_dst, x_src, n_src, c_in, w_l, b_l, w_r, c_out, agg, nullptr, out, scratch, scratch_bytes, dims,
                            stats, stream);
}

static int conv_forward_indexed_impl(const int32_t *rowptr, const int32_t *col, const int64_t *n_id, int64_t n_src, int64_t n_dst,
                                     int64_t nnz, const float *feats, int64_t n_rows, int32_t c_in, const float *w_l,
                                     const float *b_l, const float *w_r, int32_t c_out, float *agg, float *x_dst, float *out,
                                     void *scratch, size_t scratch_bytes, const int32_t *dims, BnStatsOut *stats, hipStream_t stream) {
    POPE_REQUIRE(rowptr && (col || nnz == 0) && n_id && feats && w_l && w_r && agg && out, "sage_conv_forward_indexed: null pointer");
    POPE_REQUIRE(n_dst > 0 && n_dst <= n_src && n_src < INT32_MAX && n_rows > 0 && nnz >= 0 && nnz < INT32_MAX && c_in > 0 && c_out > 0,
                 "sage_conv_forward_indexed: bad size (destinations must be the first n_dst entries of n_id)");
    return conv_forward_run(rowptr, col, n_id, n_dst, feats, n_rows, c_in, w_l, b_l, w_r, c_out, agg, x_dst, out, scratch, scratch_bytes, dims,
                            stats, stream);
}

extern "C" int sage_forward_kernel_name(int64_t n_dst, int32_t c_in, int32_t c_out, int32_t cu_count, char *name, size_t cap) {
    clear_error();
    POPE_REQUIRE(name && cap > 0 && n_dst > 0 && n_dst < INT32_MAX && c_in > 0 && c_out > 0 && cu_count > 0, "sage_forward_kernel_name: bad argument");
    const FwdPlan p = forward_plan(n_dst, c_in, c_out, n_dst, cu_count, FwdAligned{true, true, true, true, true, true},
                                   sage_conv_forward_scratch_bytes(n_dst, c_in, c_out));
    switch (p.path) {
    case FWD_OVERLAPPED: snprintf(name, cap, "k_gather_beside_gemm<%d>+k_gemm_tile16<%d, %d>", p.rb, p.rb, t16_buffers()); break;
    case FWD_TILE16:     snprintf(name, cap, "k_gemm_tile16<%d, %d>", p.rb, t16_buffers()); break;
    case FWD_STREAMK:    snprintf(name, cap, "k_gemm_streamk_ld<%d>", SK_GK); break;
    default:             snprintf(name, cap, "k_gemm<%d, %d>", p.tile.tm, p.tile.tn); break;
    }
    return POPE_OK;
}

extern "C" int sage_conv_forward(const int32_t *rowptr, const int32_t *col, int64_t n_src, int64_t n_dst, int64_t nnz,
                                 const float *x_src, int32_t c_in, const float *w_l, const float *b_l, const float *w_r,
                                 int32_t c_out, float *agg, float *out, void *scratch, size_t scratch_bytes, const int32_t *dims,
                                 void *stream_) {
    clear_error();
    return conv_forward_impl(rowptr, col, n_src, n_dst, nnz, x_src, c_in, w_l, b_l, w_r, c_out, agg, out, scratch, scratch_bytes, dims, nullptr,
                             (hipStream_t)stream_);
}

extern "C" int sage_conv_forward_indexed(const int32_t *rowptr, const int32_t *col, const int64_t *n_id, int64_t n_src, int64_t n_dst,
                                         int64_t nnz, const float *feats, int64_t n_rows, int32_t c_in, const float *w_l,
                                         const float *b_l, const float *w_r, int32_t c_out, float *agg, float *x_dst, float *out,
                                         void *scratch, size_t scratch_bytes, const int32_t *dims, void *stream_) {
    clear_error();
    return conv_forward_indexed_impl(rowptr, col, n_id, n_src, n_dst, nnz, feats, n_rows, c_in, w_l, b_l, w_r, c_out, agg, x_dst, out, scratch,
                                     scratch_bytes, dims, nullptr, (hipStream_t)stream_);
}

extern "C" int sage_conv_forward_stats(const int32_t *rowptr, const int32_t *col, int64_t n_src, int64_t n_dst, int64_t nnz,
                                       const float *x_src, int32_t c_in, const float *w_l, const float *b_l, const float *w_r,
                                       int32_t c_out, float *agg, float *out, void *scratch, size_t scratch_bytes, const int32_t *dims,
                                       double *bn_pa, double *bn_pb, int32_t bn_parts_cap, int32_t *bn_info, void *stream_) {
    clear_error();
    POPE_REQUIRE(bn_pa && bn_pb && bn_info && bn_parts_cap > 0, "sage_conv_forward_stats: null pointer");
    BnStatsOut st{bn_pa, bn_pb, bn_parts_cap};
    return stats_report(conv_forward_impl(rowptr, col, n_src, n_dst, nnz, x_src, c_in, w_l, b_l, w_r, c_out, agg, out, scratch, scratch_bytes, dims, &st,
                                          (hipStream_t)stream_), st, bn_info);
}

extern "C" int sage_conv_forward_indexed_stats(const int32_t *rowptr, const int32_t *col, const int64_t *n_id, int64_t n_src, int64_t n_dst,
                                               int64_t nnz, const float *feats, int64_t n_rows, int32_t c_in, const float *w_l,
                                               const float *b_l, const float *w_r, int32_t c_out, float *agg, float *x_dst, float *out,
                                               void *scratch, size_t scratch_bytes, const int32_t *dims, double *bn_pa, double *bn_pb,
                                               int32_t bn_parts_cap, int32_t *bn_info, void *stream_) {
    clear_error();
    POPE_REQUIRE(bn_pa && bn_pb && bn_info && bn_parts_cap > 0, "sage_conv_forward_indexed_stats: null pointer");
    BnStatsOut st{bn_pa, bn_pb, bn_parts_cap};
    return stats_report(conv_forward_indexed_impl(rowptr, col, n_id, n_src, n_dst, nnz, feats, n_rows, c_in, w_l, b_l, w_r, c_out, agg, x_dst, out,
                                                  scratch, scratch_bytes, dims, &st, (hipStream_t)stream_), st, bn_info);
}

static void enqueue_scatter_sum_det(const int32_t *rowptr, const int32_t *col, int64_t n_src, int64_t n_dst, int64_t nnz, const float *gagg,
                                    int32_t c, float *grad_x, bool vec, void *scratch, const BwdScratch &lay, const int32_t *dims,
                                    hipStream_t stream) {
    int *start = scratch_at<int>(scratch, lay.det_start), *list = scratch_at<int>(scratch, lay.det_list);
    int *sorted = scratch_at<int>(scratch, lay.det_sorted);
    const int32_t *n_dst_dev = dims, *n_src_dev = dims ? dims + 1 : nullptr;
    hipLaunchKernelGGL(k_det_clear, dim3(capped_grid((size_t)n_src + 1, 256)), dim3(256), 0, stream, start, (int)n_src, n_src_dev);
    if (nnz > 0 && n_dst > 0) {
        const dim3 rows(capped_grid((size_t)n_dst * 64, 256));
        hipLaunchKernelGGL(k_det_index<false>, rows, dim3(256), 0, stream, rowptr, col, (int)n_dst, (int)n_src, (int)nnz, start, list, n_dst_dev, n_src_dev);
        hipLaunchKernelGGL(k_det_scan, dim3(1), dim3(DET_SCAN_THREADS), 0, stream, start, (int)n_src, n_src_dev);
        hipLaunchKernelGGL(k_det_index<true>, rows, dim3(256), 0, stream, rowptr, col, (int)n_dst, (int)n_src, (int)nnz, start, list, n_dst_dev, n_src_dev);
    }
    const dim3 grid(capped_grid((size_t)n_src * ((c + 255) / 256) * 64, 256));
    if (vec)
        hipLaunchKernelGGL(k_scatter_sum_det<true>, grid, dim3(256), 0, stream, rowptr, start, list, sorted, (int)n_dst, (int)n_src, (int)nnz, gagg, c,
                           grad_x, n_dst_dev, n_src_dev);
    else
        hipLaunchKernelGGL(k_scatter_sum_det<false>, grid, dim3(256), 0, stream, rowptr, start, list, sorted, (int)n_dst, (int)n_src, (int)nnz, gagg, c,
                           grad_x, n_dst_dev, n_src_dev);
}

extern "C" int sage_scatter_mean_det(const int32_t *rowptr, const int32_t *col, int64_t n_src, int64_t n_dst, int64_t nnz, const float *grad_agg,
                                     int32_t c, float *grad_x, void *scratch, size_t scratch_bytes, const int32_t *dims, void *stream_) {
    clear_error();
    POPE_REQUIRE(n_src >= 0 && n_dst >= 0 && n_dst <= n_src && n_src < INT32_MAX && nnz >= 0 && nnz < INT32_MAX && c > 0,
                 "sage_scatter_mean_det: bad size (destinations must be the first n_dst sources)");
    if (n_src == 0) return POPE_OK;
    POPE_REQUIRE(rowptr && (col || nnz == 0) && grad_agg && grad_x && scratch, "sage_scatter_mean_det: null pointer");
    const BwdScratch lay = backward_scratch(n_src, n_dst, nnz, 0, 0, true, false);
    POPE_REQUIRE(scratch_bytes >= lay.total, "sage_scatter_mean_det: scratch %zu < %zu bytes", scratch_bytes, lay.total);
    if (nnz == 0 && n_src == n_dst) return POPE_OK;
    enqueue_scatter_sum_det(rowptr, col, n_src, n_dst, nnz, grad_agg, c, grad_x, (c & 3) == 0 && aligned16(grad_agg) && aligned16(grad_x), scratch,
                            lay, dims, (hipStream_t)stream_);
    POPE_HIP(hipGetLastError());
    return POPE_OK;
}

static int launch_gemm_dual(GemmArgs px, GemmArgs pw, const DualAux &aux, hipStream_t stream) {
    gemm_set_grid(px, 64, 64);
    gemm_set_grid(pw, 64, 64);
    const size_t lds = tile_lds_bytes<64, 64>();
    static LdsOptIn opt_in;
    if (!opt_in.done()) {
        POPE_HIP(hipFuncSetAttribute((const void *)k_gemm_dual<64, 64, 2, 2>, hipFuncAttributeMaxDynamicSharedMemorySize, (int)lds));
        opt_in.mark();
    }
    const int blocks = px.gx * px.gy * px.gz + pw.gx * pw.gy * pw.gz + aux.zero_blocks + aux.cs_gx * aux.cs_gy;
    hipLaunchKernelGGL((k_gemm_dual<64, 64, 2, 2>), dim3(blocks), dim3(256), lds, stream, px, pw, aux);
    return POPE_OK;
}

static int conv_backward_impl(const int32_t *rowptr, const int32_t *col, int64_t n_src, int64_t n_dst, int64_t nnz, const float *x_src,
                              const long long *x_rows, const float *agg, int32_t c_in, const float *w_l, const float *w_r, int32_t c_out,
                              const float *grad_out, float *grad_x, float *grad_w_l, float *grad_b_l, float *grad_w_r, void *scratch,
                              const BwdScratch &lay, const int32_t *dims, hipStream_t stream) {
    float *const gagg = scratch_at<float>(scratch, lay.grad_agg), *const slab = scratch_at<float>(scratch, lay.slab);
    float *const colsum = scratch_at<float>(scratch, lay.colsum), *const x_tmp = x_rows ? scratch_at<float>(scratch, lay.rows) : nullptr;
    const int32_t *n_dst_dev = dims, *n_src_dev = dims ? dims + 1 : nullptr;
    int cus = 0, rc = POPE_OK;
    if (streamk_tn_shape_ok(n_dst, c_out, c_in) && (rc = device_cu_count(&cus))) return rc;
    const BwdAligned al{aligned16(grad_out), aligned16(agg), aligned16(x_src), aligned16(x_tmp), aligned16(w_l), aligned16(w_r), aligned16(gagg),
                        aligned16(grad_x)};
    const BwdPlan plan = backward_plan(n_dst, n_src, c_in, c_out, nnz > 0, grad_x != nullptr, grad_b_l != nullptr, x_rows != nullptr, al, cus,
                                       lay.slab_bytes);

    GemmArgs pw = gemm_problem(Operand{grad_out, 1, c_out}, Operand{agg, 1, c_in}, (int)n_dst, c_out, c_in, grad_w_l, c_in);
    pw.twin.B = Operand{x_src, 1, c_in}; pw.twin.C = grad_w_r; pw.gz = plan.splits; pw.slab = slab; pw.k0_dev = n_dst_dev;
    GemmArgs px = gemm_problem(Operand{grad_out, c_out, 1}, Operand{w_r, 1, c_in}, c_out, (int)n_dst, c_in, grad_x, c_in);
    px.twin.B = Operand{w_l, 1, c_in}; px.twin.C = gagg; px.m_dev = n_dst_dev;
    const int reduce_blocks = (int)capped_grid((size_t)c_out * c_in * 2, 256), finals_blocks = reduce_blocks + (c_out + 15) / 16;
    const BwdFinals fin{slab, plan.splits, (size_t)c_out * c_in, c_in, grad_w_l, grad_w_r, (long long)c_in, reduce_blocks, colsum, COLSUM_SPLITS, c_out, grad_b_l};
    const dim3 scatter_grid(capped_grid((size_t)n_dst * ((c_in + 255) / 256) * 64, 256));

    for (int s = 0; s < plan.n_steps && !rc; ++s) {
        switch (plan.steps[s]) {
        case BWD_DUAL: {
            DualAux aux;
            aux.zero_x = plan.zero_rows ? grad_x : nullptr;
            aux.zero_C = c_in; aux.zero_r0 = (int)n_dst; aux.zero_r1 = (int)n_src; aux.zero_r0_dev = n_dst_dev; aux.zero_r1_dev = n_src_dev;
            aux.zero_blocks = aux.zero_x ? (int)capped_grid((size_t)n_src * c_in / 4 / 8 + 1, 256, 256) : 0;
            aux.cs_g = grad_out; aux.cs_rows = (int)n_dst; aux.cs_C = c_out; aux.cs_part = colsum; aux.cs_rows_dev = n_dst_dev;
            const dim3 cs = colsum_partial_grid(c_out, true);
            aux.cs_gx = (int)cs.x; aux.cs_gy = (int)cs.y;
            rc = launch_gemm_dual(px, pw, aux, stream);
            break;
        }
        case BWD_SCATTER_AND_FINALS:
            hipLaunchKernelGGL(k_scatter_and_finals, dim3(finals_blocks + scatter_grid.x), dim3(256), 0, stream, rowptr, col, (int)n_dst, gagg, c_in,
                               grad_x, n_dst_dev, fin, finals_blocks);
            break;
        case BWD_FINALS:         hipLaunchKernelGGL(k_bwd_finals, dim3(finals_blocks), dim3(256), 0, stream, fin); break;
        case BWD_COLSUM_PARTIAL: enqueue_colsum_partial(grad_out, (int)n_dst, c_out, colsum, n_dst_dev, plan.colsum_vec, stream); break;
        case BWD_STREAMK:
            rc = gemm_streamk_tn(grad_out, agg, x_src, n_dst, c_out, c_in, grad_w_l, grad_w_r, slab, plan.sk_grid, plan.xcd, stream, n_dst_dev,
                                 grad_b_l ? colsum : nullptr, grad_b_l, x_rows);
            break;
        case BWD_GATHER_ROWS:
            hipLaunchKernelGGL(k_gather_rows, dim3(capped_grid((size_t)n_dst * 64, 256)), dim3(256), 0, stream, x_src, x_rows, (int)n_dst, c_in, x_tmp,
                               n_dst_dev);
            pw.twin.B.p = x_tmp;
            break;
        case BWD_W_TWIN:       rc = launch_gemm(pw, plan.w_tile, plan.w_layouts, stream); break;
        case BWD_COLSUM_FINAL: hipLaunchKernelGGL(k_colsum_final, dim3((c_out + 15) / 16), dim3(256), 0, stream, colsum, COLSUM_SPLITS, c_out, grad_b_l); break;
        case BWD_ZERO_ROWS:
            hipLaunchKernelGGL(k_zero_rows, dim3(capped_grid((size_t)(n_src - (dims ? 0 : n_dst)) * c_in / 4 + 1, 256)), dim3(256), 0, stream, grad_x, c_in,
                               (int)n_dst, (int)n_src, n_dst_dev, n_src_dev);
            break;
        case BWD_X_TWIN:       rc = launch_gemm(px, plan.x_tile, plan.x_layouts, stream); break;
        case BWD_SCATTER_MEAN: hipLaunchKernelGGL(k_scatter_mean, scatter_grid, dim3(256), 0, stream, rowptr, col, (int)n_dst, gagg, c_in, grad_x, n_dst_dev); break;
        case BWD_DET_SUM:      enqueue_scatter_sum_det(rowptr, col, n_src, n_dst, nnz, gagg, c_in, grad_x, plan.det_vec, scratch, lay, dims, stream); break;
        }
    }
    if (rc) return rc;
    POPE_HIP(hipGetLastError());
    return POPE_OK;
}

extern "C" int sage_backward_kernel_name(int64_t n_dst, int64_t n_src, int32_t c_in, int32_t c_out, int32_t need_grad_x, int32_t need_grad_b,
                                         int32_t cu_count, char *name, size_t cap) {
    clear_error();
    POPE_REQUIRE(name && cap > 0 && n_dst > 0 && n_dst <= n_src && n_src < INT32_MAX && c_in > 0 && c_out > 0 && cu_count > 0,
                 "sage_backward_kernel_name: bad argument");
    const BwdPlan p = backward_plan(n_dst, n_src, c_in, c_out, true, need_grad_x != 0, need_grad_b != 0, false,
                                    BwdAligned{true, true, true, true, true, true, true, true}, cu_count,
                                    backward_scratch(n_src, n_dst, 0, c_in, c_out, g_sage_deterministic, false).slab_bytes);
    char buf[384];
    int n = 0;
    auto add = [&](const char *fmt, auto... args) {
        if (n < (int)sizeof buf) n += snprintf(buf + n, sizeof buf - n, "%s", n ? "+" : "");
        if (n < (int)sizeof buf) n += snprintf(buf + n, sizeof buf - n, fmt, args...);
    };
    auto add_gemm = [&](GemmTile t, GemmLayouts l, int splits) {
        const int wm = t.tm == 128 ? 4 : 2, wn = t.tm == 128 ? 1 : 2;
        if (splits > 1) add("k_gemm<%d, %d, %d, %d, %d, %d>[splits=%d]+k_slab_reduce", t.tm, t.tn, wm, wn, (int)l.a, (int)l.b, splits);
        else add("k_gemm<%d, %d, %d, %d, %d, %d>", t.tm, t.tn, wm, wn, (int)l.a, (int)l.b);
    };
    for (int s = 0; s < p.n_steps; ++s) {
        switch (p.steps[s]) {
        case BWD_DUAL:               add("k_gemm_dual<64, 64, 2, 2>[splits=%d]", p.splits); break;
        case BWD_SCATTER_AND_FINALS: add("%s", "k_scatter_and_finals"); break;
        case BWD_FINALS:             add("%s", "k_bwd_finals"); break;
        case BWD_COLSUM_PARTIAL:     add("k_colsum_partial<%s>", p.colsum_vec ? "true" : "false"); break;
        case BWD_STREAMK:            add("k_gemm_streamk_tn<%d>%s+k_streamk_tn_fixup<%d>", SK_GK, p.xcd ? "[xcd]" : "", SK_GK); break;
        case BWD_GATHER_ROWS:        break;
        case BWD_W_TWIN:             add_gemm(p.w_tile, p.w_layouts, p.splits); break;
        case BWD_COLSUM_FINAL:       add("%s", "k_colsum_final"); break;
        case BWD_ZERO_ROWS:          add("%s", "k_zero_rows"); break;
        case BWD_X_TWIN:             add_gemm(p.x_tile, p.x_layouts, 1); break;
        case BWD_SCATTER_MEAN:       add("%s", "k_scatter_mean"); break;
        case BWD_DET_SUM:
            add("k_det_clear+k_det_index<false>+k_det_scan+k_det_index<true>+k_scatter_sum_det<%s>", p.det_vec ? "true" : "false");
            break;
        }
    }
    POPE_REQUIRE((size_t)n < cap && n < (int)sizeof buf, "sage_backward_kernel_name: %d characters do not fit name[%zu]", n, cap);
    memcpy(name, buf, (size_t)n + 1);
    return POPE_OK;
}

extern "C" int sage_conv_backward(const int32_t *rowptr, const int32_t *col, int64_t n_src, int64_t n_dst, int64_t nnz,
                                  const float *x_src, const float *agg, int32_t c_in, const float *w_l, const float *w_r,
                                  int32_t c_out, const float *grad_out, float *grad_x, float *grad_w_l, float *grad_b_l,
                                  float *grad_w_r, void *scratch, size_t scratch_bytes, const int32_t *dims, void *stream_) {
    clear_error();
    POPE_REQUIRE(rowptr && (col || nnz == 0) && x_src && agg && w_l && w_r && grad_out && grad_w_l && grad_w_r && scratch,
                 "sage_conv_backward: null pointer");
    POPE_REQUIRE(n_dst > 0 && n_dst <= n_src && n_src < INT32_MAX && nnz >= 0 && c_in > 0 && c_out > 0, "sage_conv_backward: bad size");
    const BwdScratch lay = backward_scratch(n_src, n_dst, nnz, c_in, c_out, g_sage_deterministic, false);
    if (scratch_bytes < lay.total) {
        set_error("sage_conv_backward: scratch %zu < %zu bytes", scratch_bytes, lay.total);
        return POPE_ERR_WORKSPACE;
    }
    return conv_backward_impl(rowptr, col, n_src, n_dst, nnz, x_src, nullptr, agg, c_in, w_l, w_r, c_out, grad_out, grad_x, grad_w_l, grad_b_l,
                              grad_w_r, scratch, lay, dims, (hipStream_t)stream_);
}

extern "C" int sage_conv_backward_indexed(const int32_t *rowptr, const int32_t *col, const int64_t *n_id, int64_t n_src, int64_t n_dst,
                                          int64_t nnz, const float *feats, int64_t n_rows, const float *agg, int32_t c_in, const float *w_l,
                                          const float *w_r, int32_t c_out, const float *grad_out, float *grad_w_l, float *grad_b_l,
                                          float *grad_w_r, void *scratch, size_t scratch_bytes, const int32_t *dims, void *stream_) {
    clear_error();
    POPE_REQUIRE(rowptr && (col || nnz == 0) && n_id && feats && agg && w_l && w_r && grad_out && grad_w_l && grad_w_r && scratch,
                 "sage_conv_backward_indexed: null pointer");
    POPE_REQUIRE(n_dst > 0 && n_dst <= n_src && n_src < INT32_MAX && n_rows > 0 && nnz >= 0 && c_in > 0 && c_out > 0,
                 "sage_conv_backward_indexed: bad size");
    const BwdScratch lay = backward_scratch(n_src, n_dst, nnz, c_in, c_out, g_sage_deterministic, true);
    if (scratch_bytes < lay.total) {
        set_error("sage_conv_backward_indexed: scratch %zu < %zu bytes", scratch_bytes, lay.total);
        return POPE_ERR_WORKSPACE;
    }
    return conv_backward_impl(rowptr, col, n_src, n_dst, nnz, feats, (const long long *)n_id, agg, c_in, w_l, w_r, c_out, grad_out, nullptr, grad_w_l,
                              grad_b_l, grad_w_r, scratch, lay, dims, (hipStream_t)stream_);
}
```

### graphpope_amd/sage.py

```python
from __future__ import annotations

import ctypes
import math
from typing import NamedTuple

import numpy as np
import torch
import torch.nn.functional as F
from torch import nn

from . import _lib
from ._lib import check, on_device, ptr


def _stream():
    return ctypes.c_void_p(torch.cuda.current_stream().cuda_stream)


def set_deterministic(on: bool) -> bool:
    return bool(_lib.load().sage_set_deterministic(1 if on else 0))


def is_deterministic() -> bool:
    return bool(_lib.load().sage_get_deterministic())


class deterministic:

    def __init__(self, on: bool = True):
        self.on = bool(on)

    def __enter__(self):
        self.was = set_deterministic(self.on)
        return self

    def __exit__(self, *exc):
        set_deterministic(self.was)
        return False


class SampledAdj:

    def __init__(self, rowptr: torch.Tensor, col: torch.Tensor, n_src: int, dims: torch.Tensor | None = None):
        self.rowptr = rowptr.to(torch.int32).contiguous()
        self.col = col.to(torch.int32).contiguous()
        self.n_dst = int(rowptr.numel() - 1)
        self.n_src = int(n_src)
        if dims is not None:
            assert dims.is_cuda and dims.dtype == torch.int32 and dims.numel() >= 3 and dims.is_contiguous()
        self.dims = dims

    def size(self, dim: int) -> int:
        return (self.n_dst, self.n_src)[dim]

    def to(self, device):
        return SampledAdj(self.rowptr.to(device), self.col.to(device), self.n_src, None if self.dims is None else self.dims.to(device))

    def device_extents(self) -> "SampledAdj":
        if self.dims is not None:
            return self
        dims = torch.tensor([self.n_dst, self.n_src, int(self.col.numel()), 0], dtype=torch.int32, device=self.rowptr.device)
        return SampledAdj(self.rowptr, self.col, self.n_src, dims)


def _forward_scratch(lib, n_dst, c_in, c_out, dev):
    nbytes = lib.sage_conv_forward_scratch_bytes(n_dst, c_in, c_out)
    if nbytes == 0:
        return None, 0
    return torch.empty(nbytes, dtype=torch.uint8, device=dev), nbytes


def _stats_buffers(n_dst, c_out, dev):
    return torch.empty((2, (n_dst + 15) // 16, c_out), dtype=torch.float64, device=dev), (ctypes.c_int32 * 2)(0, 0)


class IndexedFeatures:

    def __init__(self, feats: torch.Tensor, n_id: torch.Tensor):
        assert feats.dim() == 2 and feats.dtype == torch.float32 and feats.is_contiguous() and not feats.requires_grad
        assert n_id.dtype == torch.int64 and n_id.dim() == 1 and n_id.device == feats.device
        self.feats, self.n_id = feats, n_id.contiguous()

    def materialize(self) -> torch.Tensor:
        return self.feats.index_select(0, self.n_id)


def _conv_forward(lib, x, w_l, b_l, w_r, adj, want_stats):
    indexed = isinstance(x, IndexedFeatures)
    feats = x.feats if indexed else x
    if not feats.is_cuda:
        raise RuntimeError("SAGEConv runs on the GPU only (no CPU fallback)")
    if not (feats.is_contiguous() and w_l.is_contiguous() and w_r.is_contiguous()):
        feats, w_l, w_r = feats.contiguous(), w_l.contiguous(), w_r.contiguous()
    rowptr, col, n_dst, dev = adj.rowptr, adj.col, adj.size(0), feats.device
    c_in, c_out = feats.shape[1], w_l.shape[0]
    agg = torch.empty((n_dst, c_in), dtype=torch.float32, device=dev)
    x_dst = torch.empty((n_dst, c_in), dtype=torch.float32, device=dev) if indexed else None
    out = torch.empty((n_dst, c_out), dtype=torch.float32, device=dev)
    with on_device(dev):
        scratch, nbytes = _forward_scratch(lib, n_dst, c_in, c_out, dev)
        if indexed:
            plain, with_stats = lib.sage_conv_forward_indexed, lib.sage_conv_forward_indexed_stats
            args = (ptr(rowptr), ptr(col), ptr(x.n_id), x.n_id.numel(), n_dst, col.numel(), ptr(feats), feats.shape[0], c_in, ptr(w_l),
                    ptr(b_l), ptr(w_r), c_out, ptr(agg), ptr(x_dst), ptr(out), ptr(scratch), nbytes, ptr(adj.dims))
        else:
            plain, with_stats = lib.sage_conv_forward, lib.sage_conv_forward_stats
            args = (ptr(rowptr), ptr(col), feats.shape[0], n_dst, col.numel(), ptr(feats), c_in, ptr(w_l), ptr(b_l), ptr(w_r), c_out,
                    ptr(agg), ptr(out), ptr(scratch), nbytes, ptr(adj.dims))
        stats = None
        if want_stats:
            partials, info = _stats_buffers(n_dst, c_out, dev)
            check(with_stats(*args, ptr(partials[0]), ptr(partials[1]), partials.shape[1], info, _stream()))
            if info[0] > 0:
                stats = (partials, int(info[0]), int(info[1]))
        else:
            check(plain(*args, _stream()))
    return out, (x_dst if indexed else feats, agg, w_l, w_r), stats


def _conv_backward(lib, rows, agg, w_l, w_r, adj, grad_out, need_x, need_b):
    (n_src, c_in), n_dst, c_out, dev = rows.shape, agg.shape[0], w_l.shape[0], rows.device
    rowptr, col = adj.rowptr, adj.col
    grad_out = grad_out.contiguous()
    grad_x = torch.empty_like(rows) if need_x else None
    grad_w_l, grad_w_r = torch.empty_like(w_l), torch.empty_like(w_r)
    grad_b = torch.empty(c_out, dtype=torch.float32, device=dev) if need_b else None
    with on_device(dev):
        scratch = torch.empty(max(lib.sage_conv_scratch_bytes(n_src, n_dst, col.numel(), c_in, c_out), 16), dtype=torch.uint8, device=dev)
        check(lib.sage_conv_backward(ptr(rowptr), ptr(col), n_src, n_dst, col.numel(), ptr(rows), ptr(agg), c_in, ptr(w_l), ptr(w_r),
                                     c_out, ptr(grad_out), ptr(grad_x), ptr(grad_w_l), ptr(grad_b), ptr(grad_w_r), ptr(scratch),
                                     scratch.numel(), ptr(adj.dims), _stream()))
    return grad_x, grad_w_l, grad_b, grad_w_r


class _Tail(NamedTuple):
    running_mean: torch.Tensor | None
    running_var: torch.Tensor | None
    num_batches_tracked: torch.Tensor | None
    momentum: float
    eps: float
    batch_stats: bool
    p: float
    seed: int
    rows: torch.Tensor | None
    seed_dev: torch.Tensor | None


def _bn_forward(lib, x, gamma, beta, t: _Tail, stats=None):
    if not x.is_cuda:
        raise RuntimeError("the fused BatchNorm/ReLU/dropout epilogue runs on the GPU only (no CPU fallback)")
    (m, c), dev = x.shape, x.device
    y = torch.empty_like(x)
    mean = torch.empty(c, dtype=torch.float32, device=dev)
    rstd = torch.empty(c, dtype=torch.float32, device=dev)
    with on_device(dev):
        scratch = torch.empty(lib.sage_bn_scratch_bytes(c), dtype=torch.uint8, device=dev)
        args = (ptr(x), m, c, ptr(gamma), ptr(beta), ptr(t.running_mean), ptr(t.running_var), ptr(t.num_batches_tracked), t.momentum, t.eps,
                int(t.batch_stats), t.p, t.seed, ptr(y), ptr(mean), ptr(rstd), ptr(scratch), scratch.numel(), ptr(t.rows), ptr(t.seed_dev))
        if stats is None:
            check(lib.sage_bn_relu_dropout_forward(*args, _stream()))
        else:
            partials, tiles, rows_per_tile = stats
            check(lib.sage_bn_relu_dropout_forward_stats(*args, ptr(partials[0]), ptr(partials[1]), tiles, rows_per_tile, _stream()))
    return y, mean, rstd


def _bn_backward(lib, x, gamma, beta, mean, rstd, t: _Tail, grad_y, sum_columns):
    (m, c), dev = x.shape, x.device
    grad_y = grad_y.contiguous()
    grad_x = torch.empty_like(x)
    grad_gamma = torch.empty_like(gamma)
    grad_beta = torch.empty_like(beta)
    with on_device(dev):
        scratch = torch.empty(lib.sage_bn_scratch_bytes(c), dtype=torch.uint8, device=dev)
        args = (ptr(x), ptr(grad_y), m, c, ptr(gamma), ptr(beta), ptr(mean), ptr(rstd), int(t.batch_stats), t.p, t.seed, ptr(grad_x),
                ptr(grad_gamma), ptr(grad_beta), ptr(scratch), scratch.numel(), ptr(t.rows), ptr(t.seed_dev))
        colsum = None
        if sum_columns:
            colsum = torch.empty(c, dtype=torch.float32, device=dev)
            check(lib.sage_bn_relu_dropout_backward_bias(*args, ptr(colsum), _stream()))
        else:
            check(lib.sage_bn_relu_dropout_backward(*args, _stream()))
    return grad_x, grad_gamma, grad_beta, colsum


class _SageConvFn(torch.autograd.Function):

    @staticmethod
    def forward(ctx, x, w_l, b_l, w_r, adj):
        out, kept, _ = _conv_forward(_lib.load(), x, w_l, b_l, w_r, adj, False)
        ctx.save_for_backward(*kept)
        ctx.adj, ctx.has_bias = adj, b_l is not None
        return out

    @staticmethod
    def backward(ctx, grad_out):
        grad_x, grad_w_l, grad_b, grad_w_r = _conv_backward(_lib.load(), *ctx.saved_tensors, ctx.adj, grad_out, ctx.needs_input_grad[0],
                                                            ctx.has_bias)
        return grad_x, grad_w_l, grad_b, grad_w_r, None


class _Linear(nn.Module):

    def __init__(self, c_in, c_out, bias):
        super().__init__()
        self.weight = nn.Parameter(torch.empty(c_out, c_in))
        self.bias = nn.Parameter(torch.empty(c_out)) if bias else None
        self.reset_parameters()

    def reset_parameters(self):
        nn.init.kaiming_uniform_(self.weight, a=math.sqrt(5))
        if self.bias is not None:
            bound = 1 / math.sqrt(self.weight.shape[1])
            nn.init.uniform_(self.bias, -bound, bound)


class SAGEConv(nn.Module):

    def __init__(self, in_channels: int, out_channels: int):
        super().__init__()
        self.in_channels, self.out_channels = in_channels, out_channels
        self.lin_l = _Linear(in_channels, out_channels, bias=True)
        self.lin_r = _Linear(in_channels, out_channels, bias=False)

    def forward(self, x, adj_t: SampledAdj):
        return _SageConvFn.apply(_source_rows(x), self.lin_l.weight, self.lin_l.bias, self.lin_r.weight, adj_t)


def _source_rows(x):
    return x[0] if isinstance(x, (tuple, list)) else x


class _BnReluDropoutFn(torch.autograd.Function):

    @staticmethod
    def forward(ctx, x, gamma, beta, tail, w_l=None, b_l=None, w_r=None, adj=None):
        lib = _lib.load()
        if adj is None:
            h, kept, stats = x.contiguous(), (), None
        else:
            h, kept, stats = _conv_forward(lib, x, w_l, b_l, w_r, adj, tail.batch_stats)
        y, mean, rstd = _bn_forward(lib, h, gamma, beta, tail, stats)
        ctx.save_for_backward(h, gamma, beta, mean, rstd, *kept)
        ctx.tail, ctx.adj, ctx.has_bias = tail, adj, b_l is not None
        ctx.bias_from_tail = stats is not None
        return y

    @staticmethod
    def backward(ctx, grad_y):
        lib = _lib.load()
        h, gamma, beta, mean, rstd, *kept = ctx.saved_tensors
        grad_h, grad_gamma, grad_beta, colsum = _bn_backward(lib, h, gamma, beta, mean, rstd, ctx.tail, grad_y, ctx.bias_from_tail)
        if ctx.adj is None:
            return grad_h, grad_gamma, grad_beta, None
        given_b = colsum if ctx.has_bias else None
        grad_x, grad_w_l, grad_b, grad_w_r = _conv_backward(lib, *kept, ctx.adj, grad_h, ctx.needs_input_grad[0],
                                                            ctx.has_bias and given_b is None)
        return grad_x, grad_gamma, grad_beta, None, grad_w_l, (given_b if given_b is not None else grad_b), grad_w_r, None


def _tail_of(bn: nn.BatchNorm1d, p: float, training: bool, seed, rows, seed_dev) -> _Tail:
    if bn.weight is None or bn.momentum is None:
        raise NotImplementedError("fused epilogue: affine BatchNorm1d with a fixed momentum only (the reference's default)")
    use_batch_stats = training or bn.running_mean is None
    nbt = bn.num_batches_tracked if (training and bn.track_running_stats and bn.num_batches_tracked is not None) else None
    if nbt is not None and not (nbt.is_cuda and nbt.dtype == torch.int64):
        nbt.add_(1)
        nbt = None
    if seed is None:
        seed = int(torch.randint(0, 2 ** 62, (1,)).item()) if (training and p > 0 and seed_dev is None) else 0
    rm = bn.running_mean if bn.track_running_stats else None
    rv = bn.running_var if bn.track_running_stats else None
    return _Tail(rm, rv, nbt, float(bn.momentum), float(bn.eps), use_batch_stats, float(p) if training else 0.0, int(seed), rows, seed_dev)


def bn_relu_dropout(x: torch.Tensor, bn: nn.BatchNorm1d, p: float, training: bool, seed: int | None = None,
                    rows: torch.Tensor | None = None, seed_dev: torch.Tensor | None = None) -> torch.Tensor:
    return _BnReluDropoutFn.apply(x, bn.weight, bn.bias, _tail_of(bn, p, training, seed, rows, seed_dev))


def conv_bn_relu_dropout(conv: SAGEConv, bn: nn.BatchNorm1d, x, adj_t: SampledAdj, p: float, training: bool, seed: int | None = None,
                         rows: torch.Tensor | None = None, seed_dev: torch.Tensor | None = None) -> torch.Tensor:
    return _BnReluDropoutFn.apply(_source_rows(x), bn.weight, bn.bias, _tail_of(bn, p, training, seed, rows, seed_dev),
                                  conv.lin_l.weight, conv.lin_l.bias, conv.lin_r.weight, adj_t)


_BAD_LABEL = {}


def bad_label_flag(device) -> torch.Tensor:
    dev = torch.device(device)
    key = (dev.type, dev.index if dev.index is not None else torch.cuda.current_device())
    if key not in _BAD_LABEL:
        _BAD_LABEL[key] = torch.zeros(1, dtype=torch.int32, device=dev)
    return _BAD_LABEL[key]


class _CrossEntropyFn(torch.autograd.Function):
    @staticmethod
    def forward(ctx, logits, target, ignore_index, unit_upstream=False, loss_in=None):
        lib = _lib.load()
        if not logits.is_cuda:
            raise RuntimeError("cross_entropy runs on the GPU only (no CPU fallback)")
        logits = logits.contiguous()
        n, c = logits.shape
        dev = logits.device
        out = torch.empty(2, dtype=torch.float32, device=dev)
        grad = torch.empty_like(logits)
        rows = torch.empty(n, dtype=torch.float32, device=dev)
        with on_device(dev):
            check(lib.sage_cross_entropy_forward(ptr(logits), ptr(target), n, c, ignore_index, ptr(out), ptr(grad),
                                                 ctypes.c_void_p(out.data_ptr() + 4), ptr(rows), ptr(bad_label_flag(dev)),
                                                 (2 if loss_in is not None else 1) if unit_upstream else 0, _stream()))
        if unit_upstream and loss_in is not None:
            loss_in.fold_loss(rows, out)
        ctx.save_for_backward(grad, out)
        ctx.unit_upstream = bool(unit_upstream)
        return out[0]

    @staticmethod
    def backward(ctx, grad_loss):
        lib = _lib.load()
        grad, out = ctx.saved_tensors
        if ctx.unit_upstream:
            return grad, None, None, None, None
        n, c = grad.shape
        grad_loss = grad_loss.contiguous()
        res = torch.empty_like(grad)
        with on_device(grad.device):
            check(lib.sage_cross_entropy_backward(ptr(grad), n, c, ptr(grad_loss), ctypes.c_void_p(out.data_ptr() + 4), ptr(res),
                                                  _stream()))
        return res, None, None, None, None


def cross_entropy(logits: torch.Tensor, target: torch.Tensor, ignore_index: int = -100, unit_upstream: bool = False, loss_in=None) -> torch.Tensor:
    if target.dtype != torch.int64 or target.dim() != 1 or logits.dim() != 2 or target.shape[0] != logits.shape[0]:
        raise ValueError("cross_entropy: logits [N, C] float32 and int64 labels [N] expected")
    if loss_in is not None and not unit_upstream:
        raise ValueError("cross_entropy: loss_in needs unit_upstream=True (a step that owns its backward() and step() calls)")
    return _CrossEntropyFn.apply(logits, target.contiguous(), int(ignore_index), bool(unit_upstream), loss_in)


class EvalMetrics:

    def __init__(self, device, acc: torch.Tensor | None = None):
        self.device = torch.device(device)
        if acc is None:
            acc = torch.zeros(3, dtype=torch.int64, device=self.device)
        assert acc.is_cuda and acc.dtype == torch.int64 and acc.numel() == 3 and acc.is_contiguous() and acc.data_ptr() % 8 == 0
        self.acc = acc

    def reset(self) -> None:
        self.acc.zero_()

    def update(self, logits: torch.Tensor, y: torch.Tensor, ignore_index: int = -100) -> None:
        if not logits.is_cuda:
            raise RuntimeError("EvalMetrics runs on the GPU only (no CPU fallback)")
        if logits.dim() != 2 or logits.dtype != torch.float32 or y.dtype != torch.int64 or y.dim() != 1 or y.shape[0] != logits.shape[0]:
            raise ValueError("EvalMetrics.update: logits [M, C] float32 and int64 labels [M] expected")
        logits, y = logits.detach().contiguous(), y.contiguous()
        with on_device(logits.device):
            check(_lib.load().sage_eval_metrics(ptr(logits), ptr(y), logits.shape[0], logits.shape[1], int(ignore_index), ptr(self.acc),
                                                ptr(bad_label_flag(logits.device)), _stream()))

    def read(self):
        words = self.acc.cpu().numpy()
        loss_sum, correct, rows = float(words[:1].view(np.float64)[0]), int(words[1]), int(words[2])
        if rows == 0:
            return float("nan"), float("nan"), 0
        return loss_sum / rows, correct / rows, rows


class SAGE(nn.Module):

    def __init__(self, in_channels: int, out_channels: int, hidden_channels: int, num_layers: int, dropout: float = 0.5):
        super().__init__()
        self.dropout = dropout
        self.convs = nn.ModuleList()
        self.convs.append(SAGEConv(in_channels, hidden_channels))
        for _ in range(num_layers - 2):
            self.convs.append(SAGEConv(hidden_channels, hidden_channels))
        self.convs.append(SAGEConv(hidden_channels, out_channels))
        self.bns = nn.ModuleList()
        for _ in range(num_layers - 1):
            self.bns.append(nn.BatchNorm1d(hidden_channels))
        self.dropout_seed_dev = None

    def forward(self, x, adjs):
        for i, adj_t in enumerate(adjs):
            x = x if isinstance(x, IndexedFeatures) else (x, x[:adj_t.size(0)])
            if i == len(adjs) - 1:
                x = self.convs[i](x, adj_t)
                continue
            rows = None if adj_t.dims is None else adj_t.dims[0:1]
            if self.dropout_seed_dev is not None:
                x = conv_bn_relu_dropout(self.convs[i], self.bns[i], x, adj_t, self.dropout, self.training,
                                         seed=0x9E3779B97F4A7C15 * (i + 1) % (1 << 63), rows=rows, seed_dev=self.dropout_seed_dev)
            else:
                x = conv_bn_relu_dropout(self.convs[i], self.bns[i], x, adj_t, self.dropout, self.training, rows=rows)
        return x


def sample_batch(rowptr: np.ndarray, col: np.ndarray, seeds: np.ndarray, sizes=(25, 10), rng=None):
    rng = rng or np.random.default_rng(0)
    n_id = np.asarray(seeds, dtype=np.int64)
    adjs = []
    for size in sizes:
        local = {int(g): i for i, g in enumerate(n_id)}
        ids = list(n_id)
        rp = [0]
        cols = []
        for g in n_id:
            nbr = col[rowptr[g]:rowptr[g + 1]]
            if nbr.size > size:
                nbr = rng.choice(nbr, size, replace=False)
            for u in nbr:
                u = int(u)
                j = local.get(u)
                if j is None:
                    j = len(ids)
                    local[u] = j
                    ids.append(u)
                cols.append(j)
            rp.append(len(cols))
        adjs.append(SampledAdj(torch.tensor(rp, dtype=torch.int32), torch.tensor(cols, dtype=torch.int32), len(ids)))
        n_id = np.asarray(ids, dtype=np.int64)
    return n_id, adjs[::-1]
```

### include/graphpope_hip.h

```cpp
#ifndef GRAPHPOPE_HIP_H
#define GRAPHPOPE_HIP_H

#include <stddef.h>
#include <stdint.h>

#ifdef __cplusplus
extern "C" {
#endif

#define POPE_OK                 0
#define POPE_ERR_INVALID       -1
#define POPE_ERR_HIP           -2
#define POPE_ERR_INDEX         -3
#define POPE_ERR_HOP_OVERFLOW  -4
#define POPE_ERR_WORKSPACE     -5
#define POPE_ERR_NO_DEVICE     -6
#define POPE_ERR_UNSORTED      -7

const char *pope_last_error(void);

const char *pope_version(void);

int pope_require_device(int32_t *cu_count_host);

#define POPE_KNOB_LIVE_MODE         0
#define POPE_KNOB_FINALIZE_VARIANT  1
#define POPE_KNOB_FINALIZE_BLOCKS   2
#define POPE_KNOB_PAIRWISE_KERNEL   4
#define POPE_KNOB_COPY_BATCHES      5
#define POPE_KNOB_FAIL_HOST_REGISTER 7
#define POPE_KNOB_SAGE_FORWARD_OVERLAP 14
#define POPE_KNOB_GEMM_TILE16_BUFFERS 18
#define POPE_KNOB_PREPARE_MERGE     19
#define POPE_KNOB_STREAMK_XCD       20
#define POPE_KNOB_FORWARD_WHOLE_TILES 21
#define POPE_KNOB_LEVEL1_APPLY      22
int pope_debug_set(int32_t knob, int32_t value);

size_t pope_csr_scratch_bytes(int64_t N, int64_t E);
size_t pope_csr_aux_elems(int64_t E);

int pope_csr_build(const int64_t *edge_index, int64_t E, int64_t N, int32_t *rowptr, int32_t *col, int32_t *erow,
                   int32_t *aux, void *scratch, size_t scratch_bytes, int32_t defer_check, void *stream);

int pope_csr_build_canonical(const int64_t *edge_index, int64_t E, int64_t N, int32_t *rowptr, int32_t *col, int32_t *erow,
                             int32_t *aux, void *scratch, size_t scratch_bytes, void *stream);

int pope_pagerank_weights(const int32_t *rowptr, const int32_t *col, int64_t N, double *w, void *stream);
int pope_pagerank_step(const int32_t *rowptr_by_target, const int32_t *sources, int64_t N, const double *x, const double *w,
                       double dangling_sum, double alpha, double *x_out, void *stream);

size_t pope_clustering_scratch_bytes(int64_t N, int64_t E);
int pope_clustering_counts(const int32_t *rowptr, const int32_t *col, const int32_t *erow, const int32_t *rowptr_by_target,
                           const int32_t *sources, const int32_t *erow_by_target, int64_t N, int64_t E, int64_t *T, int64_t *dt,
                           int64_t *db, void *scratch, size_t scratch_bytes, void *stream);

size_t pope_betweenness_scratch_bytes(int64_t N, int64_t batch);
int pope_betweenness_batch(const int32_t *rowptr, const int32_t *col, int64_t E_by_source, const int32_t *rowptr_by_target,
                           const int32_t *sources, int64_t E_by_target, int64_t N, int64_t first_source, int64_t num_sources,
                           double *bc, double *sigma_out, double *delta_out, int32_t *dist_out, int32_t *queue_len_out,
                           void *scratch, size_t scratch_bytes, void *stream);

size_t pope_eigenvector_scratch_bytes(int64_t N);
int pope_eigenvector_iterate(const int32_t *rowptr_by_target, const int32_t *sources, int64_t N, double *x, void *scratch,
                             size_t scratch_bytes, int32_t iterations, double tol, void *control,
                             void *stream);

#define POPE_TOPK_MAX_K 4096
int pope_degree_counts(const int32_t *rowptr, const int32_t *col, const int32_t *erow, int64_t N, int64_t *degree, uint64_t *keys,
                       void *stream);
size_t pope_topk_scratch_bytes(int64_t N, int64_t K);
int pope_topk_u64(const uint64_t *keys, int64_t N, int64_t K, uint64_t *out, void *scratch, size_t scratch_bytes,
                  void *stream);
int pope_topk_max_k(void);
size_t pope_topk_f64_scratch_bytes(int64_t N, int64_t K);
int pope_topk_f64(const double *scores, int64_t N, int64_t K, int64_t *nodes_out, double *scores_out, void *scratch,
                  size_t scratch_bytes, void *stream);
int pope_score_keys_host(const double *scores, int64_t n, uint64_t *keys);

size_t pope_kmeans_scratch_bytes(int64_t N, int32_t D, int32_t K);
int pope_column_moments(const float *X, int64_t N, int32_t D, double *sum, double *sumsq, void *scratch, size_t scratch_bytes,
                        void *stream);
int pope_shift_columns(const float *X, const float *shift, int64_t N, int32_t D, float sign, float *out, void *stream);
int pope_kmeans_plusplus(const float *X, int64_t N, int32_t D, int32_t K, int64_t first_id, const double *uniforms_host,
                         int32_t n_trials, int64_t *chosen, void *scratch, size_t scratch_bytes, void *stream);
int pope_kmeans_lloyd_step(const float *X, int64_t N, int32_t D, const float *centers, int32_t K, float *centers_new,
                           int32_t *labels, const int32_t *labels_prev, int32_t *changed, double *shift_total,
                           void *scratch, size_t scratch_bytes, void *stream);


int32_t pope_words(int32_t K);

size_t pope_plane_bytes(int64_t N, int32_t K);
size_t pope_bfs_scratch_bytes(int64_t N, int64_t E, int32_t K);

int pope_geodesic_bfs(const int32_t *rowptr, const int32_t *col, const int32_t *erow, const int32_t *aux,
                      int64_t N, int64_t E,
                      const int64_t *anchors_host, int32_t K, uint64_t *planes, int32_t plane_capacity, void *scratch, size_t scratch_bytes,
                      int32_t *max_hop_host, int32_t *n_hop_bits_host, void *stream);

int pope_geodesic_bfs_begin(const int32_t *rowptr, const int32_t *col, const int32_t *erow, const int32_t *aux,
                            int64_t N, int64_t E, const int64_t *anchors_host, int32_t K, uint64_t *planes,
                            int32_t plane_capacity, void *scratch, size_t scratch_bytes, void *stream);
int pope_geodesic_bfs_finish(const int32_t *rowptr, const int32_t *col, const int32_t *erow, const int32_t *aux,
                             int64_t N, int64_t E, const int64_t *anchors_host, int32_t K, uint64_t *planes,
                             int32_t plane_capacity, void *scratch, size_t scratch_bytes, int32_t *max_hop_host,
                             int32_t *n_hop_bits_host, void *stream);

int pope_geodesic_finalize(const uint64_t *planes, int32_t n_hop_bits, int64_t N, int32_t K_shard,
                           const float *x, int32_t F, float *out, int64_t out_cols, int32_t c0, void *stream);

int pope_geodesic_finalize_shards(const uint64_t *planes, int32_t n_shards, int64_t shard_stride_words, int32_t n_hop_bits,
                                  int64_t N, int32_t K_shard, const float *x, int32_t F, float *out, int64_t out_cols,
                                  void *stream);

int pope_finalize_kernel_name(int64_t N, int32_t K_shard, int32_t F, int32_t has_x, int32_t n_shards, char *name, size_t cap);

int pope_level_kernel_name(int64_t N, int32_t K, char *name, size_t cap);

size_t pope_geodesic_run_workspace_bytes(int64_t N, int64_t E, int32_t K, int32_t plane_capacity);
uint64_t *pope_geodesic_run_planes(void *workspace, int64_t N, int64_t E, int32_t K, int32_t plane_capacity);
int pope_geodesic_run(const int64_t *edge_index, int64_t E, int64_t N, const int64_t *anchors_host, int32_t K,
                      const float *x, int32_t F, float *out, int64_t out_cols, int32_t plane_capacity,
                      void *workspace, size_t workspace_bytes, int32_t *max_hop_host, int32_t *n_hop_bits_host,
                      void *stream);

void pope_profile_levels(int32_t enable);
int32_t pope_profile_read(int32_t *levels_host, float *level_ms_host, int32_t capacity);
int32_t pope_profile_level1_applies(void);

int pope_geodesic_hops(const uint64_t *planes, int32_t n_hop_bits, int64_t N, int32_t K,
                       int32_t *hops, void *stream);

size_t pope_column_stats_scratch_bytes(int32_t K);
int pope_geodesic_column_stats(const uint64_t *planes, int32_t n_hop_bits, int64_t N, int32_t K, int64_t *hop_sum,
                               int64_t *reach, void *scratch, size_t scratch_bytes, void *stream);

#define POPE_METRIC_COSINE_DISTANCE   0
#define POPE_METRIC_COSINE_SIMILARITY 1
#define POPE_METRIC_EUCLIDEAN         2

size_t pope_pairwise_scratch_bytes(int64_t N, int32_t K, int32_t D);

int pope_pairwise_minmax(const float *X, int64_t N, int32_t D, const float *A, int32_t K, int32_t metric,
                         float *out, int64_t out_cols, int32_t c0, void *scratch, size_t scratch_bytes,
                         void *stream);
size_t pope_pairwise_by_id_scratch_bytes(int64_t N, int32_t K, int32_t D);
int pope_pairwise_features_by_id(const float *x, int32_t F, const float *X, int64_t N, int32_t D, const int64_t *anchor_ids, int32_t K,
                                 int32_t metric, float *out, int64_t out_cols, int32_t c0, void *scratch, size_t scratch_bytes,
                                 void *stream);

int pope_pairwise_features(const float *x, int32_t F, const float *X, int64_t N, int32_t D, const float *A, int32_t K,
                           int32_t metric, float *out, int64_t out_cols, int32_t c0, void *scratch, size_t scratch_bytes,
                           void *stream);

int pope_pairwise_kernel_name(int64_t N, int32_t D, int32_t K, int32_t F, int32_t has_x, int32_t by_id, int32_t cu_count, char *name,
                              size_t cap);

int pope_concat(const float *x, int64_t N, int32_t F, float *out, int64_t out_cols, void *stream);

int pope_host_copy_2d(const void *src_host, int64_t src_pitch_bytes, void *dst_host, int64_t dst_pitch_bytes,
                      int64_t row_bytes, int64_t rows, int32_t threads);

int pope_copy_2d_to_host(const void *src, int64_t src_pitch_bytes, void *dst_host, int64_t dst_pitch_bytes,
                         int64_t row_bytes, int64_t rows, void *stream);

int pope_assemble_host_result(const void *x_host, int64_t x_pitch_bytes, int64_t x_row_bytes, const void *emb,
                              int64_t emb_pitch_bytes, int64_t emb_row_bytes, void *out_host, int64_t out_pitch_bytes,
                              int64_t rows, int32_t threads, int32_t chunks, void *stream);

void *pope_assemble_begin(const void *x_host, int64_t x_pitch_bytes, int64_t x_row_bytes, void *out_host, int64_t out_pitch_bytes,
                          int64_t rows, int32_t threads, int32_t chunks);
int pope_assemble_finish(void *handle, const void *emb, int64_t emb_pitch_bytes, int64_t emb_row_bytes, void *stream);
void pope_assemble_abort(void *handle);
void pope_assemble_prepare(int32_t device);
int32_t pope_assemble_ring_ready(void);

int pope_geodesic_hop_codes(const uint64_t *planes, int32_t n_hop_bits, int32_t max_hop, int64_t N, int32_t K, uint8_t *codes,
                            int64_t codes_pitch_bytes, float *lut, void *stream);
int pope_assemble_finish_codes(void *handle, const uint8_t *codes, int64_t codes_pitch_bytes, int32_t K, const float *lut, void *stream);

int pope_host_pin(const void *host, size_t bytes);
int pope_host_unpin(const void *host);
int pope_copy_to_device(const void *src_host, void *dst, size_t bytes, void *stream);

size_t sage_conv_scratch_bytes(int64_t n_src, int64_t n_dst, int64_t nnz, int32_t c_in, int32_t c_out);
size_t sage_conv_forward_scratch_bytes(int64_t n_dst, int32_t c_in, int32_t c_out);

int sage_conv_forward(const int32_t *rowptr, const int32_t *col, int64_t n_src, int64_t n_dst, int64_t nnz,
                      const float *x_src, int32_t c_in, const float *w_l, const float *b_l, const float *w_r,
                      int32_t c_out, float *agg, float *out, void *scratch, size_t scratch_bytes, const int32_t *dims,
                      void *stream);

int sage_gather_mean(const int32_t *rowptr, const int32_t *col, int64_t n_src, int64_t n_dst, int64_t nnz,
                     const float *x_src, int32_t c_in, float *agg, void *stream);

int sage_conv_forward_indexed(const int32_t *rowptr, const int32_t *col, const int64_t *n_id, int64_t n_src, int64_t n_dst,
                              int64_t nnz, const float *feats, int64_t n_rows, int32_t c_in, const float *w_l, const float *b_l,
                              const float *w_r, int32_t c_out, float *agg, float *x_dst, float *out, void *scratch,
                              size_t scratch_bytes, const int32_t *dims, void *stream);
int sage_conv_forward_stats(const int32_t *rowptr, const int32_t *col, int64_t n_src, int64_t n_dst, int64_t nnz, const float *x_src,
                            int32_t c_in, const float *w_l, const float *b_l, const float *w_r, int32_t c_out, float *agg, float *out,
                            void *scratch, size_t scratch_bytes, const int32_t *dims, double *bn_pa, double *bn_pb, int32_t bn_parts_cap,
                            int32_t *bn_info, void *stream);
int sage_conv_forward_indexed_stats(const int32_t *rowptr, const int32_t *col, const int64_t *n_id, int64_t n_src, int64_t n_dst,
                                    int64_t nnz, const float *feats, int64_t n_rows, int32_t c_in, const float *w_l, const float *b_l,
                                    const float *w_r, int32_t c_out, float *agg, float *x_dst, float *out, void *scratch,
                                    size_t scratch_bytes, const int32_t *dims, double *bn_pa, double *bn_pb, int32_t bn_parts_cap,
                                    int32_t *bn_info, void *stream);
int sage_forward_kernel_name(int64_t n_dst, int32_t c_in, int32_t c_out, int32_t cu_count, char *name, size_t cap);
int sage_conv_backward(const int32_t *rowptr, const int32_t *col, int64_t n_src, int64_t n_dst, int64_t nnz,
                       const float *x_src, const float *agg, int32_t c_in, const float *w_l, const float *w_r,
                       int32_t c_out, const float *grad_out, float *grad_x, float *grad_w_l, float *grad_b_l,
                       float *grad_w_r, void *scratch, size_t scratch_bytes, const int32_t *dims, void *stream);
int sage_backward_kernel_name(int64_t n_dst, int64_t n_src, int32_t c_in, int32_t c_out, int32_t need_grad_x, int32_t need_grad_b,
                              int32_t cu_count, char *name, size_t cap);

int32_t sage_set_deterministic(int32_t on);
int32_t sage_get_deterministic(void);
size_t sage_scatter_mean_det_scratch_bytes(int64_t n_src, int64_t n_dst, int64_t nnz);
int sage_scatter_mean_det(const int32_t *rowptr, const int32_t *col, int64_t n_src, int64_t n_dst, int64_t nnz, const float *grad_agg,
                          int32_t c, float *grad_x, void *scratch, size_t scratch_bytes, const int32_t *dims, void *stream);
size_t sage_conv_forward_indexed_scratch_bytes(int64_t n_dst, int32_t c_in, int32_t c_out);
size_t sage_conv_backward_indexed_scratch_bytes(int64_t n_src, int64_t n_dst, int64_t nnz, int32_t c_in, int32_t c_out);
int sage_conv_backward_indexed(const int32_t *rowptr, const int32_t *col, const int64_t *n_id, int64_t n_src, int64_t n_dst,
                               int64_t nnz, const float *feats, int64_t n_rows, const float *agg, int32_t c_in, const float *w_l,
                               const float *w_r, int32_t c_out, const float *grad_out, float *grad_w_l, float *grad_b_l,
                               float *grad_w_r, void *scratch, size_t scratch_bytes, const int32_t *dims, void *stream);

size_t sage_sample_scratch_bytes(int64_t N, int64_t n_targets, int64_t nnz_capacity);
int sage_sample_hop(const int32_t *rowptr, const int32_t *col, int64_t N, const int64_t *targets, int64_t n_targets,
                    int32_t fanout, uint64_t seed, int32_t hop, int32_t *out_rowptr, int32_t *out_col, int64_t nnz_capacity,
                    int64_t *out_n_id, int64_t *nnz_host, int64_t *n_src_host, void *scratch, size_t scratch_bytes,
                    void *stream);

int sage_sample_batch(const int32_t *rowptr, const int32_t *col, int64_t N, const int64_t *seeds, int64_t n_seeds,
                      const int32_t *fanouts_host, int32_t n_hops, uint64_t seed, int32_t *const *out_rowptr,
                      int32_t *const *out_col, int64_t *const *out_n_id, int64_t *nnz_host, int64_t *n_src_host, void *scratch,
                      size_t scratch_bytes, void *stream);

int sage_sample_batch_device(const int32_t *rowptr, const int32_t *col, int64_t N, const int64_t *seeds, int64_t n_seeds,
                             const int32_t *fanouts_host, int32_t n_hops, uint64_t seed, const uint64_t *seed_dev,
                             int32_t *const *out_rowptr, int32_t *const *out_col, int64_t *const *out_n_id, int32_t *dims,
                             void *scratch, size_t scratch_bytes, void *stream);
int sage_sample_epoch_batch_device(const int32_t *rowptr, const int32_t *col, int64_t N, const int64_t *order, const int64_t *first_dev,
                                   int64_t n_seeds, const int64_t *labels, int64_t *y_out, const int32_t *fanouts_host, int32_t n_hops,
                                   uint64_t seed, const uint64_t *seed_dev, int32_t *const *out_rowptr, int32_t *const *out_col,
                                   int64_t *const *out_n_id, int32_t *dims, void *scratch, size_t scratch_bytes, void *stream);

size_t sage_bn_scratch_bytes(int32_t C);
int sage_bn_relu_dropout_forward(const float *x, int64_t M, int32_t C, const float *gamma, const float *beta,
                                 float *running_mean, float *running_var, int64_t *num_batches_tracked, float momentum, float eps, int32_t training,
                                 float p, uint64_t seed, float *y, float *save_mean, float *save_rstd, void *scratch,
                                 size_t scratch_bytes, const int32_t *rows_dev, const uint64_t *seed_dev, void *stream);
int sage_bn_relu_dropout_forward_stats(const float *x, int64_t M, int32_t C, const float *gamma, const float *beta,
                                       float *running_mean, float *running_var, int64_t *num_batches_tracked, float momentum, float eps,
                                       int32_t training, float p, uint64_t seed, float *y, float *save_mean, float *save_rstd, void *scratch,
                                       size_t scratch_bytes, const int32_t *rows_dev, const uint64_t *seed_dev, const double *pa,
                                       const double *pb, int32_t parts, int32_t rows_per_part, void *stream);
int sage_bn_relu_dropout_backward(const float *x, const float *grad_y, int64_t M, int32_t C, const float *gamma,
                                  const float *beta, const float *save_mean, const float *save_rstd, int32_t training,
                                  float p, uint64_t seed, float *grad_x, float *grad_gamma, float *grad_beta, void *scratch,
                                  size_t scratch_bytes, const int32_t *rows_dev, const uint64_t *seed_dev, void *stream);
int sage_bn_relu_dropout_backward_bias(const float *x, const float *grad_y, int64_t M, int32_t C, const float *gamma,
                                       const float *beta, const float *save_mean, const float *save_rstd, int32_t training,
                                       float p, uint64_t seed, float *grad_x, float *grad_gamma, float *grad_beta, void *scratch,
                                       size_t scratch_bytes, const int32_t *rows_dev, const uint64_t *seed_dev, float *grad_x_colsum,
                                       void *stream);

int sage_adam_step(int32_t n_tensors, float *const *params, const float *const *grads, float *const *exp_avg,
                   float *const *exp_avg_sq, const int64_t *numel, double lr, double beta1, double beta2, double eps,
                   double weight_decay, int64_t step, const int64_t *step_dev, void *stream);
int sage_adam_step_loss(int32_t n_tensors, float *const *params, const float *const *grads, float *const *exp_avg,
                        float *const *exp_avg_sq, const int64_t *numel, double lr, double beta1, double beta2, double eps,
                        double weight_decay, int64_t step, const int64_t *step_dev, const float *xent_rows, int64_t xent_n,
                        float *loss_out, void *stream);

size_t sage_grad_norm_partials(int32_t n_tensors, const int64_t *numel);
int sage_grad_sqnorm(int32_t n_tensors, const float *const *grads, const int64_t *numel, double *partials, size_t partials_len,
                     void *stream);
int sage_adam_step_clip(int32_t n_tensors, float *const *params, const float *const *grads, float *const *exp_avg,
                        float *const *exp_avg_sq, const int64_t *numel, double lr, double beta1, double beta2, double eps,
                        double weight_decay, int64_t step, const int64_t *step_dev, double max_norm, const double *partials,
                        size_t n_partials, float *norm_out, const float *xent_rows, int64_t xent_n, float *loss_out, void *stream);

int sage_advance_counters(int64_t *counters, const int64_t *increments_host, int32_t n, void *stream);
int sage_copy_segments(int32_t n, void *const *dst, const void *const *src, const int64_t *bytes, void *stream);

int sage_cross_entropy_forward(const float *logits, const int64_t *target, int64_t N, int32_t C, int64_t ignore_index,
                               float *loss, float *grad_unscaled, float *inv_count, float *row_scratch, int32_t *bad_label,
                               int32_t fused, void *stream);
int sage_cross_entropy_backward(const float *grad_unscaled, int64_t N, int32_t C, const float *grad_loss, const float *inv_count,
                                float *grad_logits, void *stream);

int sage_eval_metrics(const float *logits, const int64_t *target, int64_t M, int32_t C, int64_t ignore_index, void *acc,
                      int32_t *bad_label, void *stream);

int pope_n2v_walks(const int32_t *rowptr, const int32_t *col, int64_t N, const int64_t *starts, int64_t B, int64_t B_neg,
                   int32_t walk_length, uint64_t seed, int64_t first_row, int64_t *pos, int64_t *neg, void *stream);
int pope_n2v_windows(const int64_t *rows, int64_t R, int32_t len, int32_t context, int64_t *windows, void *stream);
int pope_n2v_loss_grad(const float *emb, int64_t N, int32_t D, const int64_t *rows, int64_t R, int32_t len, int32_t context,
                       int32_t negative, double scale, double *loss_acc, float *grad, uint8_t *touched, void *stream);
int pope_n2v_sparse_adam(float *emb, float *grad, uint8_t *touched, float *exp_avg, float *exp_avg_sq, int64_t N, int32_t D,
                         double lr, double beta1, double beta2, double eps, int64_t step, void *stream);

#ifdef __cplusplus
}
#endif
#endif
```

Baseline: 102.8 billion embeddings/s.

## Fuse BN-ReLU-dropout apply into the next SAGE conv's neighbor gather

Splits BN statistics from the apply step and adds a fused path for the last hidden layer. BN+ReLU+dropout is applied on the fly inside a mean-aggregation gather kernel that feeds the final conv GEMM, so the normalized activation tensor is never written and re-read. Backward recomputes through the saved aggregated and own-row inputs. The cost is extra per-element transform work, since each neighbor row is re-normalized and re-hashed every time it is gathered, plus a new dispatch path guarded by a support check.

```diff
diff --git a/graphpope_amd/_lib.py b/graphpope_amd/_lib.py
--- a/graphpope_amd/_lib.py
+++ b/graphpope_amd/_lib.py
@@ -136,6 +136,13 @@
     "sage_bn_relu_dropout_forward_stats": (c_int, [c_void_p, c_int64, c_int32, c_void_p, c_void_p, c_void_p, c_void_p, c_void_p, c_float, c_float,
                                                    c_int32, c_float, c_uint64, c_void_p, c_void_p, c_void_p, c_void_p, c_size_t,
                                                    c_void_p, c_void_p, c_void_p, c_void_p, c_int32, c_int32, c_void_p]),
+    "sage_bn_statistics": (c_int, [c_void_p, c_int64, c_int32, c_void_p, c_void_p, c_void_p, c_float, c_float, c_int32, c_void_p, c_void_p,
+                                   c_void_p, c_size_t, c_void_p, c_void_p, c_void_p, c_int32, c_int32, c_void_p]),
+    "sage_conv_forward_bn_supported": (c_int, [c_int64, c_int32, c_int32, c_void_p, c_void_p, c_void_p, c_void_p]),
+    "sage_conv_forward_bn": (c_int, [c_void_p, c_void_p, c_int64, c_int64, c_int64, c_void_p, c_int32, c_void_p, c_void_p, c_void_p, c_void_p,
+                                     c_int32, c_float, c_uint64, c_void_p, c_void_p, c_void_p, c_void_p, c_int32, c_void_p, c_void_p, c_void_p,
+                                     c_void_p, c_size_t, c_void_p, c_void_p]),
+    "sage_tail_forward_kernel_name": (c_int, [c_int64, c_int32, c_int32, c_int32, c_char_p, c_size_t]),
     "sage_bn_relu_dropout_backward": (c_int, [c_void_p, c_void_p, c_int64, c_int32, c_void_p, c_void_p, c_void_p, c_void_p,
                                               c_int32, c_float, c_uint64, c_void_p, c_void_p, c_void_p, c_void_p, c_size_t,
                                               c_void_p, c_void_p, c_void_p]),
diff --git a/graphpope_amd/csrc/bn_transform.h b/graphpope_amd/csrc/bn_transform.h
--- /dev/null
+++ b/graphpope_amd/csrc/bn_transform.h
@@ -0,0 +1,46 @@
+#pragma once
+#include "common.h"
+
+namespace pope {
+
+__device__ __forceinline__ unsigned fmix32(unsigned h) {
+    h ^= h >> 16;
+    h *= 0x85ebca6bu;
+    h ^= h >> 13;
+    h *= 0xc2b2ae35u;
+    h ^= h >> 16;
+    return h;
+}
+
+__device__ __forceinline__ bool keep_element(unsigned long long seed, unsigned long long idx, unsigned threshold) {
+    unsigned h = fmix32((unsigned)idx ^ (unsigned)seed);
+    h = fmix32(h ^ ((unsigned)(idx >> 32) * 0x9e3779b1u) ^ (unsigned)(seed >> 32));
+    return (h >> 8) >= threshold;
+}
+
+__device__ __forceinline__ bool bn_element_on(float x, float mean, float rstd, float gamma, float beta, unsigned long long seed,
+                                              unsigned long long idx, unsigned threshold, float &xhat, float &z) {
+    xhat = (x - mean) * rstd;
+    z = xhat * gamma + beta;
+    return z > 0.f && keep_element(seed, idx, threshold);
+}
+
+__device__ __forceinline__ float bn_relu_dropout_element(float x, float mean, float rstd, float gamma, float beta, float inv_keep,
+                                                         unsigned long long seed, unsigned long long idx, unsigned threshold) {
+    float xhat, z;
+    return bn_element_on(x, mean, rstd, gamma, beta, seed, idx, threshold, xhat, z) ? __fmul_rn(z, inv_keep) : 0.f;
+}
+
+struct DropoutConsts {
+    unsigned threshold;
+    float inv_keep;
+};
+
+static inline DropoutConsts dropout_consts(int training, float p) {
+    DropoutConsts d;
+    d.threshold = !training || !(p > 0.f) ? 0u : p >= 1.f ? 1u << 24 : (unsigned)((double)p * 16777216.0);
+    d.inv_keep = (training && p > 0.f && p < 1.f) ? (float)(1.0 / (1.0 - (double)p)) : 1.f;
+    return d;
+}
+
+}
diff --git a/graphpope_amd/csrc/epilogue.hip b/graphpope_amd/csrc/epilogue.hip
--- a/graphpope_amd/csrc/epilogue.hip
+++ b/graphpope_amd/csrc/epilogue.hip
@@ -1,23 +1,8 @@
-#include "common.h"
+#include "bn_transform.h"
 
 namespace pope {
 
 constexpr int BN_MAX_PARTS = 256;
-
-__device__ __forceinline__ unsigned fmix32(unsigned h) {
-    h ^= h >> 16;
-    h *= 0x85ebca6bu;
-    h ^= h >> 13;
-    h *= 0xc2b2ae35u;
-    h ^= h >> 16;
-    return h;
-}
-
-__device__ __forceinline__ bool keep_element(unsigned long long seed, unsigned long long idx, unsigned threshold) {
-    unsigned h = fmix32((unsigned)idx ^ (unsigned)seed);
-    h = fmix32(h ^ ((unsigned)(idx >> 32) * 0x9e3779b1u) ^ (unsigned)(seed >> 32));
-    return (h >> 8) >= threshold;
-}
 
 template <int VEC> struct Pack { float v[VEC]; };
 
@@ -229,12 +214,11 @@
         if constexpr (BWD) { k1 = load_pack<VEC>(c1 + c0); k2 = load_pack<VEC>(c2 + c0); }
 #pragma unroll
         for (int i = 0; i < VEC; ++i) {
-            const float xhat = (xv.v[i] - mu.v[i]) * rs.v[i];
-            const float z = xhat * ga.v[i] + be.v[i];
-            const bool on = z > 0.f && keep_element(seed, off + i, threshold);
             if constexpr (!BWD) {
-                r.v[i] = on ? z * inv_keep : 0.f;
+                r.v[i] = bn_relu_dropout_element(xv.v[i], mu.v[i], rs.v[i], ga.v[i], be.v[i], inv_keep, seed, off + i, threshold);
             } else {
+                float xhat, z;
+                const bool on = bn_element_on(xv.v[i], mu.v[i], rs.v[i], ga.v[i], be.v[i], seed, off + i, threshold, xhat, z);
                 const float g = on ? gv.v[i] * inv_keep : 0.f;
                 r.v[i] = ga.v[i] * rs.v[i] * (g - k1.v[i] - xhat * k2.v[i]);
             }
@@ -269,35 +253,26 @@
     return p;
 }
 
-static unsigned drop_threshold(float p) {
-    if (!(p > 0.f)) return 0u;
-    if (p >= 1.f) return 1u << 24;
-    return (unsigned)((double)p * 16777216.0);
-}
-
 }
 
 using namespace pope;
 
 extern "C" size_t sage_bn_scratch_bytes(int32_t C) { return C <= 0 ? 0 : bn_scratch(C); }
 
-static int bn_forward_impl(const float *x, int64_t M, int32_t C, const float *gamma, const float *beta,
-                           float *running_mean, float *running_var, int64_t *num_batches_tracked, float momentum, float eps,
-                           int32_t training, float p, uint64_t seed, float *y, float *save_mean,
-                           float *save_rstd, void *scratch, size_t scratch_bytes, const int32_t *rows_dev,
-                           const uint64_t *seed_dev_, const double *ext_pa, const double *ext_pb, int ext_parts, int ext_rows_per_part,
-                           hipStream_t stream) {
-    POPE_REQUIRE(x && gamma && beta && y && save_mean && save_rstd && scratch, "sage_bn_relu_dropout_forward: null pointer");
-    POPE_REQUIRE(M > 0 && M < INT32_MAX && C > 0 && (size_t)M * C < ((size_t)1 << 40), "sage_bn_relu_dropout_forward: bad size");
-    POPE_REQUIRE(training || (running_mean && running_var), "sage_bn_relu_dropout_forward: eval mode needs running statistics");
-    POPE_REQUIRE((running_mean == nullptr) == (running_var == nullptr), "sage_bn_relu_dropout_forward: running_mean/var go together");
-    POPE_REQUIRE(p >= 0.f && p <= 1.f && eps > 0.f, "sage_bn_relu_dropout_forward: need 0 <= p <= 1, eps > 0");
+static int bn_statistics_impl(const char *who, const float *x, const float *y, int64_t M, int32_t C, const float *gamma, const float *beta,
+                              float *running_mean, float *running_var, int64_t *num_batches_tracked, float momentum, float eps, int32_t training,
+                              float *save_mean, float *save_rstd, void *scratch, size_t scratch_bytes, const int32_t *rows_dev,
+                              const double *ext_pa, const double *ext_pb, int ext_parts, int ext_rows_per_part, BnPlan *plan, hipStream_t stream) {
+    POPE_REQUIRE(x && save_mean && save_rstd && scratch, "%s: null pointer", who);
+    POPE_REQUIRE(M > 0 && M < INT32_MAX && C > 0 && (size_t)M * C < ((size_t)1 << 40), "%s: bad size", who);
+    POPE_REQUIRE(training || (running_mean && running_var), "%s: eval mode needs running statistics", who);
+    POPE_REQUIRE((running_mean == nullptr) == (running_var == nullptr), "%s: running_mean/var go together", who);
+    POPE_REQUIRE(eps > 0.f, "%s: need eps > 0", who);
     if (scratch_bytes < bn_scratch(C)) {
-        set_error("sage_bn_relu_dropout_forward: scratch %zu < %zu bytes", scratch_bytes, bn_scratch(C));
+        set_error("%s: scratch %zu < %zu bytes", who, scratch_bytes, bn_scratch(C));
         return POPE_ERR_WORKSPACE;
     }
     const BnPlan pl = bn_plan(M, C, scratch, x, y, nullptr, gamma, beta, save_mean, save_rstd);
-    const unsigned long long *seed_dev = (const unsigned long long *)seed_dev_;
     const bool external = training && ext_pa && ext_pb && ext_parts > 0 && ext_rows_per_part > 0;
     if (training && !external) {
         const dim3 grid(pl.parts, (C + 64 * pl.vec - 1) / (64 * pl.vec));
@@ -311,18 +286,46 @@
     hipLaunchKernelGGL(k_bn_final, dim3((C + 15) / 16), dim3(256), 0, stream, external ? ext_pa : pl.pa, external ? ext_pb : pl.pb,
                        external ? ext_parts : pl.parts, (int)M, C, training, momentum, eps, running_mean, running_var, save_mean, save_rstd,
                        (long long *)num_batches_tracked, rows_dev, external ? ext_rows_per_part : 0);
-    const unsigned thr = training ? drop_threshold(p) : 0u;
-    const float inv_keep = (training && p > 0.f && p < 1.f) ? (float)(1.0 / (1.0 - (double)p)) : 1.f;
+    if (plan) *plan = pl;
+    POPE_HIP(hipGetLastError());
+    return POPE_OK;
+}
+
+static int bn_forward_impl(const float *x, int64_t M, int32_t C, const float *gamma, const float *beta,
+                           float *running_mean, float *running_var, int64_t *num_batches_tracked, float momentum, float eps,
+                           int32_t training, float p, uint64_t seed, float *y, float *save_mean,
+                           float *save_rstd, void *scratch, size_t scratch_bytes, const int32_t *rows_dev,
+                           const uint64_t *seed_dev_, const double *ext_pa, const double *ext_pb, int ext_parts, int ext_rows_per_part,
+                           hipStream_t stream) {
+    POPE_REQUIRE(gamma && beta && y, "sage_bn_relu_dropout_forward: null pointer");
+    POPE_REQUIRE(p >= 0.f && p <= 1.f, "sage_bn_relu_dropout_forward: need 0 <= p <= 1");
+    BnPlan pl;
+    const int rc = bn_statistics_impl("sage_bn_relu_dropout_forward", x, y, M, C, gamma, beta, running_mean, running_var, num_batches_tracked, momentum,
+                                      eps, training, save_mean, save_rstd, scratch, scratch_bytes, rows_dev, ext_pa, ext_pb, ext_parts,
+                                      ext_rows_per_part, &pl, stream);
+    if (rc) return rc;
+    const unsigned long long *seed_dev = (const unsigned long long *)seed_dev_;
+    const DropoutConsts d = dropout_consts(training, p);
     const size_t total = (size_t)M * C;
     const unsigned blocks = capped_grid(total / pl.vec, 256);
     if (pl.vec == 4)
         hipLaunchKernelGGL((k_bn_apply<4, false>), dim3(blocks), dim3(256), 0, stream, x, nullptr, total, C, save_mean, save_rstd,
-                           gamma, beta, nullptr, nullptr, (unsigned long long)seed, thr, inv_keep, y, rows_dev, seed_dev);
+                           gamma, beta, nullptr, nullptr, (unsigned long long)seed, d.threshold, d.inv_keep, y, rows_dev, seed_dev);
     else
         hipLaunchKernelGGL((k_bn_apply<1, false>), dim3(blocks), dim3(256), 0, stream, x, nullptr, total, C, save_mean, save_rstd,
-                           gamma, beta, nullptr, nullptr, (unsigned long long)seed, thr, inv_keep, y, rows_dev, seed_dev);
+                           gamma, beta, nullptr, nullptr, (unsigned long long)seed, d.threshold, d.inv_keep, y, rows_dev, seed_dev);
     POPE_HIP(hipGetLastError());
     return POPE_OK;
+}
+
+extern "C" int sage_bn_statistics(const float *x, int64_t M, int32_t C, float *running_mean, float *running_var, int64_t *num_batches_tracked,
+                                  float momentum, float eps, int32_t training, float *save_mean, float *save_rstd, void *scratch,
+                                  size_t scratch_bytes, const int32_t *rows_dev, const double *pa, const double *pb, int32_t parts,
+                                  int32_t rows_per_part, void *stream_) {
+    clear_error();
+    POPE_REQUIRE(!pa || (pb && parts > 0 && rows_per_part > 0 && (int64_t)parts * rows_per_part >= M), "sage_bn_statistics: the partials do not cover the rows");
+    return bn_statistics_impl("sage_bn_statistics", x, nullptr, M, C, nullptr, nullptr, running_mean, running_var, num_batches_tracked, momentum, eps,
+                              training, save_mean, save_rstd, scratch, scratch_bytes, rows_dev, pa, pb, parts, rows_per_part, nullptr, (hipStream_t)stream_);
 }
 
 extern "C" int sage_bn_relu_dropout_forward(const float *x, int64_t M, int32_t C, const float *gamma, const float *beta,
@@ -361,8 +364,9 @@
     }
     const BnPlan pl = bn_plan(M, C, scratch, x, grad_y, grad_x, gamma, beta, save_mean, save_rstd);
     const unsigned long long *seed_dev = (const unsigned long long *)seed_dev_;
-    const unsigned thr = training ? drop_threshold(p) : 0u;
-    const float inv_keep = (training && p > 0.f && p < 1.f) ? (float)(1.0 / (1.0 - (double)p)) : 1.f;
+    const DropoutConsts d = dropout_consts(training, p);
+    const unsigned thr = d.threshold;
+    const float inv_keep = d.inv_keep;
     const dim3 grid(pl.parts, (C + 64 * pl.vec - 1) / (64 * pl.vec));
     if (pl.vec == 4)
         hipLaunchKernelGGL((k_bn_partial<4, true>), grid, dim3(256), 0, stream, x, grad_y, (int)M, C, pl.rows_per_part, save_mean,
diff --git a/graphpope_amd/csrc/sage.hip b/graphpope_amd/csrc/sage.hip
--- a/graphpope_amd/csrc/sage.hip
+++ b/graphpope_amd/csrc/sage.hip
@@ -1,6 +1,7 @@
 #include <cstring>
 #include <mutex>
 
+#include "bn_transform.h"
 #include "gemm_streamk_tn.h"
 #include "gemm_tile16.h"
 #include "side_copy.h"
@@ -56,6 +57,60 @@
     }
 }
 
+struct BnRowTransform {
+    const float *mean, *rstd, *gamma, *beta;
+    unsigned long long seed;
+    const unsigned long long *seed_dev;
+    unsigned threshold;
+    float inv_keep;
+};
+
+__global__ __launch_bounds__(256) void k_gather_mean_bn(const int *__restrict__ rowptr, const int *__restrict__ col, int n_dst,
+                                                        const float *__restrict__ h, int C, BnRowTransform t, float *__restrict__ agg,
+                                                        float *__restrict__ x_dst, const int *__restrict__ n_dst_dev) {
+    const int lane = threadIdx.x & 63;
+    const int wave = (blockIdx.x * blockDim.x + threadIdx.x) >> 6;
+    const int nwaves = (gridDim.x * blockDim.x) >> 6;
+    n_dst = dyn_extent(n_dst_dev, n_dst);
+    const unsigned long long seed = t.seed + (t.seed_dev ? *t.seed_dev : 0ull);
+    const int slabs = (C + 63) >> 6;
+    const long long items = (long long)n_dst * slabs;
+    for (long long w = wave; w < items; w += nwaves) {
+        const int i = (int)(w / slabs), c = (int)(w - (long long)i * slabs) * 64 + lane;
+        const bool ok = c < C;
+        const int cc = ok ? c : 0;
+        const float mu = t.mean[cc], rs = t.rstd[cc], ga = t.gamma[cc], be = t.beta[cc];
+        auto element = [&](int j) { return h[(size_t)j * C + cc]; };
+        auto transform = [&](float v, int j) {
+            return bn_relu_dropout_element(v, mu, rs, ga, be, t.inv_keep, seed, (unsigned long long)j * C + cc, t.threshold);
+        };
+        const int beg = rowptr[i], end = rowptr[i + 1];
+        const float inv = end > beg ? 1.0f / (float)(end - beg) : 0.0f;
+        const float own = element(i);
+        float s = 0.f;
+        for (int p0 = beg; p0 < end; p0 += 64) {
+            const int cnt = min(64, end - p0);
+            const int mine = lane < cnt ? col[p0 + lane] : 0;
+            for (int p = 0; p < cnt; p += 8) {
+                int j[8];
+                float v[8];
+#pragma unroll
+                for (int k = 0; k < 8; ++k) {
+                    j[k] = __shfl(mine, min(p + k, cnt - 1));
+                    v[k] = element(j[k]);
+                }
+#pragma unroll
+                for (int k = 0; k < 8; ++k)
+                    if (p + k < cnt) s += transform(v[k], j[k]);
+            }
+        }
+        if (ok) {
+            agg[(size_t)i * C + c] = s * inv;
+            x_dst[(size_t)i * C + c] = transform(own, i);
+        }
+    }
+}
+
 __device__ __forceinline__ void scatter_mean_block(const int *__restrict__ rowptr, const int *__restrict__ col, int n_dst,
                                                    const float *__restrict__ gagg, int C, float *__restrict__ gx,
                                                    const int *__restrict__ n_dst_dev, const int block, const int nblocks) {
@@ -1166,6 +1221,24 @@
     return POPE_OK;
 }
 
+static int forward_one_pass(const FwdPlan &plan, const float *agg, const float *own, int64_t n_dst, int32_t c_in, const float *w_l, const float *b_l,
+                            const float *w_r, int32_t c_out, float *out, void *scratch, const int32_t *dims, int cus, BnStatsOut *stats,
+                            hipStream_t stream) {
+    switch (plan.path) {
+    case FWD_TILE16:
+        return gemm_tile16(agg, w_l, c_in, own, w_r, c_in, c_in, c_in, (int)n_dst, c_out, b_l, out, c_out, plan.rb, cus, stream, dims, stats);
+    case FWD_STREAMK:
+        return gemm_streamk(agg, w_l, c_in, own, w_r, c_in, c_in, c_in, (int)n_dst, c_out, b_l, out, c_out, scratch, cus, stream, dims);
+    default: {
+        GemmArgs p = gemm_problem(Operand{agg, c_in, 1}, Operand{w_l, c_in, 1}, c_in, (int)n_dst, c_out, out, c_out);
+        p.A1 = Operand{own, c_in, 1}; p.B1 = Operand{w_r, c_in, 1}; p.K1 = c_in;
+        p.bias = b_l;
+        p.m_dev = dims;
+        return launch_gemm(p, plan.tile, gemm_layouts(p), stream);
+    }
+    }
+}
+
 static int conv_forward_run(const int32_t *rowptr, const int32_t *col, const int64_t *n_id, int64_t n_dst, const float *x, int64_t x_rows,
                             int32_t c_in, const float *w_l, const float *b_l, const float *w_r, int32_t c_out, float *agg, float *x_dst,
                             float *out, void *scratch, size_t scratch_bytes, const int32_t *dims, BnStatsOut *stats, hipStream_t stream) {
@@ -1188,19 +1261,7 @@
         x_dst = x_dst_tail;
     }
     enqueue_gather_mean(rowptr, col, n_dst, x, c_in, agg, stream, n_id, x_dst, dims);
-    switch (plan.path) {
-    case FWD_TILE16:
-        return gemm_tile16(agg, w_l, c_in, own, w_r, c_in, c_in, c_in, (int)n_dst, c_out, b_l, out, c_out, plan.rb, cus, stream, dims, stats);
-    case FWD_STREAMK:
-        return gemm_streamk(agg, w_l, c_in, own, w_r, c_in, c_in, c_in, (int)n_dst, c_out, b_l, out, c_out, scratch, cus, stream, dims);
-    default: {
-        GemmArgs p = gemm_problem(Operand{agg, c_in, 1}, Operand{w_l, c_in, 1}, c_in, (int)n_dst, c_out, out, c_out);
-        p.A1 = Operand{own, c_in, 1}; p.B1 = Operand{w_r, c_in, 1}; p.K1 = c_in;
-        p.bias = b_l;
-        p.m_dev = dims;
-        return launch_gemm(p, plan.tile, gemm_layouts(p), stream);
-    }
-    }
+    return forward_one_pass(plan, agg, own, n_dst, c_in, w_l, b_l, w_r, c_out, out, scratch, dims, cus, stats, stream);
 }
 
 static int conv_forward_impl(const int32_t *rowptr, const int32_t *col, int64_t n_src, int64_t n_dst, int64_t nnz,
@@ -1278,6 +1339,62 @@
     BnStatsOut st{bn_pa, bn_pb, bn_parts_cap};
     return stats_report(conv_forward_indexed_impl(rowptr, col, n_id, n_src, n_dst, nnz, feats, n_rows, c_in, w_l, b_l, w_r, c_out, agg, x_dst, out,
                                                   scratch, scratch_bytes, dims, &st, (hipStream_t)stream_), st, bn_info);
+}
+
+static bool fused_tail_ok(int64_t n_dst, int32_t c_in, int32_t c_out, int cus, bool aligned) {
+    if ((c_in & 3) || !aligned) return false;
+    const FwdAligned all{true, true, true, true, true, true};
+    return forward_plan(n_dst, c_in, c_out, n_dst, cus, all, sage_conv_forward_scratch_bytes(n_dst, c_in, c_out)).path != FWD_OVERLAPPED;
+}
+
+extern "C" int sage_conv_forward_bn_supported(int64_t n_dst, int32_t c_in, int32_t c_out, const float *gamma, const float *beta, const float *w_l,
+                                              const float *w_r) {
+    clear_error();
+    POPE_REQUIRE(n_dst > 0 && n_dst < INT32_MAX && c_in > 0 && c_out > 0, "sage_conv_forward_bn_supported: bad size");
+    int cus = 0, rc;
+    if ((rc = device_cu_count(&cus))) return rc;
+    return fused_tail_ok(n_dst, c_in, c_out, cus, aligned16(gamma) && aligned16(beta) && aligned16(w_l) && aligned16(w_r)) ? 1 : 0;
+}
+
+extern "C" int sage_conv_forward_bn(const int32_t *rowptr, const int32_t *col, int64_t n_src, int64_t n_dst, int64_t nnz, const float *h,
+                                    int32_t c_in, const float *mean, const float *rstd, const float *gamma, const float *beta, int32_t training,
+                                    float p, uint64_t seed, const uint64_t *seed_dev, const float *w_l, const float *b_l, const float *w_r,
+                                    int32_t c_out, float *agg, float *x_dst, float *out, void *scratch, size_t scratch_bytes, const int32_t *dims,
+                                    void *stream_) {
+    clear_error();
+    hipStream_t stream = (hipStream_t)stream_;
+    POPE_REQUIRE(rowptr && (col || nnz == 0) && h && mean && rstd && gamma && beta && w_l && w_r && agg && x_dst && out, "sage_conv_forward_bn: null pointer");
+    POPE_REQUIRE(n_dst > 0 && n_dst <= n_src && n_src < INT32_MAX && nnz >= 0 && nnz < INT32_MAX && c_in > 0 && c_out > 0,
+                 "sage_conv_forward_bn: bad size (destinations must be the first n_dst sources)");
+    POPE_REQUIRE(p >= 0.f && p <= 1.f, "sage_conv_forward_bn: need 0 <= p <= 1");
+    int cus = 0, rc;
+    if ((rc = device_cu_count(&cus))) return rc;
+    const bool aligned = aligned16(h) && aligned16(mean) && aligned16(rstd) && aligned16(gamma) && aligned16(beta) && aligned16(w_l) && aligned16(w_r) &&
+                         aligned16(agg) && aligned16(x_dst);
+    POPE_REQUIRE(fused_tail_ok(n_dst, c_in, c_out, cus, aligned), "sage_conv_forward_bn: not a layer of this form (sage_conv_forward_bn_supported)");
+    const DropoutConsts d = dropout_consts(training, p);
+    const BnRowTransform t{mean, rstd, gamma, beta, (unsigned long long)seed, (const unsigned long long *)seed_dev, d.threshold, d.inv_keep};
+    hipLaunchKernelGGL(k_gather_mean_bn, dim3(capped_grid((size_t)n_dst * ((c_in + 63) / 64) * 64, 256)), dim3(256), 0, stream, rowptr, col, (int)n_dst, h, c_in, t, agg, x_dst,
+                       dims);
+    POPE_HIP(hipGetLastError());
+    const FwdAligned al{false, true, true, true, true, true};
+    const FwdPlan plan = forward_plan(n_dst, c_in, c_out, n_dst, cus, al, scratch ? scratch_bytes : 0);
+    return forward_one_pass(plan, agg, x_dst, n_dst, c_in, w_l, b_l, w_r, c_out, out, scratch, dims, cus, nullptr, stream);
+}
+
+extern "C" int sage_tail_forward_kernel_name(int64_t n_dst, int32_t c_in, int32_t c_out, int32_t cu_count, char *name, size_t cap) {
+    clear_error();
+    POPE_REQUIRE(name && cap > 0 && n_dst > 0 && n_dst < INT32_MAX && c_in > 0 && c_out > 0 && cu_count > 0, "sage_tail_forward_kernel_name: bad argument");
+    char proj[96], buf[192];
+    const int rc = sage_forward_kernel_name(n_dst, c_in, c_out, cu_count, proj, sizeof proj);
+    if (rc) return rc;
+    int n;
+    if (fused_tail_ok(n_dst, c_in, c_out, cu_count, true)) n = snprintf(buf, sizeof buf, "k_bn_final+k_gather_mean_bn+%s", proj);
+    else if (!strncmp(proj, "k_gather_beside_gemm", 20)) n = snprintf(buf, sizeof buf, "k_bn_final+k_bn_apply<%d, false>+%s", c_in % 4 ? 1 : 4, proj);
+    else n = snprintf(buf, sizeof buf, "k_bn_final+k_bn_apply<%d, false>+k_gather_mean<%s>+%s", c_in % 4 ? 1 : 4, c_in % 4 ? "false" : "true", proj);
+    POPE_REQUIRE((size_t)n < cap && n < (int)sizeof buf, "sage_tail_forward_kernel_name: %d characters do not fit name[%zu]", n, cap);
+    memcpy(name, buf, (size_t)n + 1);
+    return POPE_OK;
 }
 
 static void enqueue_scatter_sum_det(const int32_t *rowptr, const int32_t *col, int64_t n_src, int64_t n_dst, int64_t nnz, const float *gagg,
diff --git a/graphpope_amd/sage.py b/graphpope_amd/sage.py
--- a/graphpope_amd/sage.py
+++ b/graphpope_amd/sage.py
@@ -118,11 +118,11 @@
     return out, (x_dst if indexed else feats, agg, w_l, w_r), stats
 
 
-def _conv_backward(lib, rows, agg, w_l, w_r, adj, grad_out, need_x, need_b):
-    (n_src, c_in), n_dst, c_out, dev = rows.shape, agg.shape[0], w_l.shape[0], rows.device
+def _conv_backward(lib, rows, agg, w_l, w_r, adj, grad_out, need_x, need_b, n_src=None):
+    n_src, c_in, n_dst, c_out, dev = rows.shape[0] if n_src is None else n_src, rows.shape[1], agg.shape[0], w_l.shape[0], rows.device
     rowptr, col = adj.rowptr, adj.col
     grad_out = grad_out.contiguous()
-    grad_x = torch.empty_like(rows) if need_x else None
+    grad_x = torch.empty((n_src, c_in), dtype=torch.float32, device=dev) if need_x else None
     grad_w_l, grad_w_r = torch.empty_like(w_l), torch.empty_like(w_r)
     grad_b = torch.empty(c_out, dtype=torch.float32, device=dev) if need_b else None
     with on_device(dev):
@@ -165,6 +165,43 @@
     return y, mean, rstd
 
 
+def _bn_statistics(lib, x, t: _Tail, stats=None):
+    (m, c), dev = x.shape, x.device
+    mean = torch.empty(c, dtype=torch.float32, device=dev)
+    rstd = torch.empty(c, dtype=torch.float32, device=dev)
+    partials, tiles, rows_per_tile = stats if stats is not None else ((None, None), 0, 0)
+    with on_device(dev):
+        scratch = torch.empty(lib.sage_bn_scratch_bytes(c), dtype=torch.uint8, device=dev)
+        check(lib.sage_bn_statistics(ptr(x), m, c, ptr(t.running_mean), ptr(t.running_var), ptr(t.num_batches_tracked), t.momentum, t.eps,
+                                     int(t.batch_stats), ptr(mean), ptr(rstd), ptr(scratch), scratch.numel(), ptr(t.rows), ptr(partials[0]),
+                                     ptr(partials[1]), tiles, rows_per_tile, _stream()))
+    return mean, rstd
+
+
+def _fused_tail_supported(lib, h_cols, gamma, beta, w_l, w_r, adj) -> bool:
+    tensors = (gamma, beta, w_l, w_r)
+    if not all(t.is_cuda and t.dtype == torch.float32 and t.is_contiguous() for t in tensors) or w_l.shape[1] != h_cols:
+        return False
+    with on_device(w_l.device):
+        rc = lib.sage_conv_forward_bn_supported(adj.size(0), h_cols, w_l.shape[0], ptr(gamma), ptr(beta), ptr(w_l), ptr(w_r))
+    if rc < 0:
+        check(rc)
+    return rc == 1
+
+
+def _conv_forward_bn(lib, h, gamma, beta, mean, rstd, t: _Tail, w_l, b_l, w_r, adj):
+    (n_src, c_in), n_dst, c_out, dev = h.shape, adj.size(0), w_l.shape[0], h.device
+    agg = torch.empty((n_dst, c_in), dtype=torch.float32, device=dev)
+    x_dst = torch.empty((n_dst, c_in), dtype=torch.float32, device=dev)
+    out = torch.empty((n_dst, c_out), dtype=torch.float32, device=dev)
+    with on_device(dev):
+        scratch, nbytes = _forward_scratch(lib, n_dst, c_in, c_out, dev)
+        check(lib.sage_conv_forward_bn(ptr(adj.rowptr), ptr(adj.col), n_src, n_dst, adj.col.numel(), ptr(h), c_in, ptr(mean), ptr(rstd), ptr(gamma),
+                                       ptr(beta), int(t.batch_stats), t.p, t.seed, ptr(t.seed_dev), ptr(w_l), ptr(b_l), ptr(w_r), c_out, ptr(agg),
+                                       ptr(x_dst), ptr(out), ptr(scratch), nbytes, ptr(adj.dims), _stream()))
+    return out, agg, x_dst
+
+
 def _bn_backward(lib, x, gamma, beta, mean, rstd, t: _Tail, grad_y, sum_columns):
     (m, c), dev = x.shape, x.device
     grad_y = grad_y.contiguous()
@@ -234,29 +271,42 @@
 class _BnReluDropoutFn(torch.autograd.Function):
 
     @staticmethod
-    def forward(ctx, x, gamma, beta, tail, w_l=None, b_l=None, w_r=None, adj=None):
+    def forward(ctx, x, gamma, beta, tail, w_l=None, b_l=None, w_r=None, adj=None, next_w_l=None, next_b_l=None, next_w_r=None, next_adj=None):
         lib = _lib.load()
         if adj is None:
             h, kept, stats = x.contiguous(), (), None
         else:
             h, kept, stats = _conv_forward(lib, x, w_l, b_l, w_r, adj, tail.batch_stats)
-        y, mean, rstd = _bn_forward(lib, h, gamma, beta, tail, stats)
-        ctx.save_for_backward(h, gamma, beta, mean, rstd, *kept)
-        ctx.tail, ctx.adj, ctx.has_bias = tail, adj, b_l is not None
+        ctx.tail, ctx.adj, ctx.next_adj, ctx.has_bias, ctx.next_has_bias = tail, adj, next_adj, b_l is not None, next_b_l is not None
         ctx.bias_from_tail = stats is not None
-        return y
-
-    @staticmethod
-    def backward(ctx, grad_y):
+        if next_adj is None:
+            y, mean, rstd = _bn_forward(lib, h, gamma, beta, tail, stats)
+            ctx.save_for_backward(h, gamma, beta, mean, rstd, *kept)
+            return y
+        mean, rstd = _bn_statistics(lib, h, tail, stats)
+        out, agg, x_dst = _conv_forward_bn(lib, h, gamma, beta, mean, rstd, tail, next_w_l, next_b_l, next_w_r, next_adj)
+        ctx.save_for_backward(h, gamma, beta, mean, rstd, *kept, x_dst, agg, next_w_l, next_w_r)
+        return out
+
+    @staticmethod
+    def backward(ctx, grad_out):
         lib = _lib.load()
         h, gamma, beta, mean, rstd, *kept = ctx.saved_tensors
+        next_grads = (None, None, None, None)
+        if ctx.next_adj is None:
+            grad_y = grad_out
+        else:
+            *kept, x_dst, agg, next_w_l, next_w_r = kept
+            grad_y, grad_nw_l, grad_nb, grad_nw_r = _conv_backward(lib, x_dst, agg, next_w_l, next_w_r, ctx.next_adj, grad_out, True,
+                                                                   ctx.next_has_bias, n_src=h.shape[0])
+            next_grads = (grad_nw_l, grad_nb, grad_nw_r, None)
         grad_h, grad_gamma, grad_beta, colsum = _bn_backward(lib, h, gamma, beta, mean, rstd, ctx.tail, grad_y, ctx.bias_from_tail)
         if ctx.adj is None:
-            return grad_h, grad_gamma, grad_beta, None
+            return (grad_h, grad_gamma, grad_beta, None, None, None, None, None) + next_grads
         given_b = colsum if ctx.has_bias else None
         grad_x, grad_w_l, grad_b, grad_w_r = _conv_backward(lib, *kept, ctx.adj, grad_h, ctx.needs_input_grad[0],
                                                             ctx.has_bias and given_b is None)
-        return grad_x, grad_gamma, grad_beta, None, grad_w_l, (given_b if given_b is not None else grad_b), grad_w_r, None
+        return (grad_x, grad_gamma, grad_beta, None, grad_w_l, (given_b if given_b is not None else grad_b), grad_w_r, None) + next_grads
 
 
 def _tail_of(bn: nn.BatchNorm1d, p: float, training: bool, seed, rows, seed_dev) -> _Tail:
@@ -283,6 +333,18 @@
                          rows: torch.Tensor | None = None, seed_dev: torch.Tensor | None = None) -> torch.Tensor:
     return _BnReluDropoutFn.apply(_source_rows(x), bn.weight, bn.bias, _tail_of(bn, p, training, seed, rows, seed_dev),
                                   conv.lin_l.weight, conv.lin_l.bias, conv.lin_r.weight, adj_t)
+
+
+def conv_bn_relu_dropout_conv(conv: SAGEConv, bn: nn.BatchNorm1d, next_conv: SAGEConv, x, adj_t: SampledAdj, next_adj_t: SampledAdj, p: float,
+                              training: bool, seed: int | None = None, rows: torch.Tensor | None = None,
+                              seed_dev: torch.Tensor | None = None) -> torch.Tensor:
+    tail = _tail_of(bn, p, training, seed, rows, seed_dev)
+    nl, nr = next_conv.lin_l, next_conv.lin_r
+    if _fused_tail_supported(_lib.load(), conv.out_channels, bn.weight, bn.bias, nl.weight, nr.weight, next_adj_t):
+        return _BnReluDropoutFn.apply(_source_rows(x), bn.weight, bn.bias, tail, conv.lin_l.weight, conv.lin_l.bias, conv.lin_r.weight, adj_t,
+                                      nl.weight, nl.bias, nr.weight, next_adj_t)
+    y = _BnReluDropoutFn.apply(_source_rows(x), bn.weight, bn.bias, tail, conv.lin_l.weight, conv.lin_l.bias, conv.lin_r.weight, adj_t)
+    return next_conv((y, y[:next_adj_t.size(0)]), next_adj_t)
 
 
 _BAD_LABEL = {}
@@ -387,17 +449,20 @@
         self.dropout_seed_dev = None
 
     def forward(self, x, adjs):
-        for i, adj_t in enumerate(adjs):
-            x = x if isinstance(x, IndexedFeatures) else (x, x[:adj_t.size(0)])
-            if i == len(adjs) - 1:
-                x = self.convs[i](x, adj_t)
-                continue
+        def pair(x, adj_t):
+            return x if isinstance(x, IndexedFeatures) else (x, x[:adj_t.size(0)])
+
+        last = len(adjs) - 1
+        if last == 0:
+            return self.convs[0](pair(x, adjs[0]), adjs[0])
+        for i, adj_t in enumerate(adjs[:last]):
             rows = None if adj_t.dims is None else adj_t.dims[0:1]
-            if self.dropout_seed_dev is not None:
-                x = conv_bn_relu_dropout(self.convs[i], self.bns[i], x, adj_t, self.dropout, self.training,
-                                         seed=0x9E3779B97F4A7C15 * (i + 1) % (1 << 63), rows=rows, seed_dev=self.dropout_seed_dev)
+            seeds = {} if self.dropout_seed_dev is None else {"seed": 0x9E3779B97F4A7C15 * (i + 1) % (1 << 63), "seed_dev": self.dropout_seed_dev}
+            if i < last - 1:
+                x = conv_bn_relu_dropout(self.convs[i], self.bns[i], pair(x, adj_t), adj_t, self.dropout, self.training, rows=rows, **seeds)
             else:
-                x = conv_bn_relu_dropout(self.convs[i], self.bns[i], x, adj_t, self.dropout, self.training, rows=rows)
+                x = conv_bn_relu_dropout_conv(self.convs[i], self.bns[i], self.convs[last], pair(x, adj_t), adj_t, adjs[last], self.dropout,
+                                              self.training, rows=rows, **seeds)
         return x
 
 
diff --git a/include/graphpope_hip.h b/include/graphpope_hip.h
--- a/include/graphpope_hip.h
+++ b/include/graphpope_hip.h
@@ -258,6 +258,16 @@
                                        int32_t training, float p, uint64_t seed, float *y, float *save_mean, float *save_rstd, void *scratch,
                                        size_t scratch_bytes, const int32_t *rows_dev, const uint64_t *seed_dev, const double *pa,
                                        const double *pb, int32_t parts, int32_t rows_per_part, void *stream);
+int sage_bn_statistics(const float *x, int64_t M, int32_t C, float *running_mean, float *running_var, int64_t *num_batches_tracked,
+                       float momentum, float eps, int32_t training, float *save_mean, float *save_rstd, void *scratch, size_t scratch_bytes,
+                       const int32_t *rows_dev, const double *pa, const double *pb, int32_t parts, int32_t rows_per_part, void *stream);
+int sage_conv_forward_bn_supported(int64_t n_dst, int32_t c_in, int32_t c_out, const float *gamma, const float *beta, const float *w_l,
+                                   const float *w_r);
+int sage_conv_forward_bn(const int32_t *rowptr, const int32_t *col, int64_t n_src, int64_t n_dst, int64_t nnz, const float *h, int32_t c_in,
+                         const float *mean, const float *rstd, const float *gamma, const float *beta, int32_t training, float p, uint64_t seed,
+                         const uint64_t *seed_dev, const float *w_l, const float *b_l, const float *w_r, int32_t c_out, float *agg,
+                         float *x_dst, float *out, void *scratch, size_t scratch_bytes, const int32_t *dims, void *stream);
+int sage_tail_forward_kernel_name(int64_t n_dst, int32_t c_in, int32_t c_out, int32_t cu_count, char *name, size_t cap);
 int sage_bn_relu_dropout_backward(const float *x, const float *grad_y, int64_t M, int32_t C, const float *gamma,
                                   const float *beta, const float *save_mean, const float *save_rstd, int32_t training,
                                   float p, uint64_t seed, float *grad_x, float *grad_gamma, float *grad_beta, void *scratch,
```

Measured after the change: 102.7 billion embeddings/s (median of 2 runs). About the same (-0.1%).
